# linhthi/BLISS-GNN

Measured on AMD Instinct MI355X. Metric: steps/sec (train step: sample_blocks + gather + SAGE fwd/bwd + Adam + exp3), reddit-like, higher is better.
Workload: dtype bf16

## Files before the change

bliss_gnn_amd/_engine.py:

```python
import contextlib
import ctypes as C
import os

import numpy as np
import torch

from . import _lib
from .graph import Block, Graph

_CHUNK = 1024
_CAP_ERRS = 1 | 2 | 4 | 8 | 64


def _ptr(t):
    return 0 if t is None else t.data_ptr()


def _stream():
    return torch.cuda.current_stream().cuda_stream


def _up8(n):
    return (int(n) + 7) & ~7


class _LayerWs:

    def __init__(self, dev, cap_s, cap_c):
        self.cap_s, self.cap_c = cap_s, cap_c
        self.seg_ptr = torch.empty(cap_s + 1, dtype=torch.int32, device=dev)
        self.seed_acc = torch.empty(60 * cap_s + 64, dtype=torch.uint8, device=dev)
        self.cand_nid = torch.empty(cap_c, dtype=torch.int32, device=dev)
        self.new_id = torch.empty(cap_c, dtype=torch.int32, device=dev)
        self.p = torch.empty(cap_c, dtype=torch.bfloat16, device=dev)
        self.P = torch.empty(cap_c, dtype=torch.bfloat16, device=dev)
        self.uniforms = torch.empty(cap_c, dtype=torch.float32, device=dev)
        self.src_cnt = None


class LayerEngine:

    def __init__(self, g: Graph):
        if g.device.type != "cuda":
            raise RuntimeError("bliss_gnn_amd samples on the GPU only; move the graph with g.to('cuda') "
                               "(the reference's --data-cpu/--use-uva modes are out of scope)")
        self.g = g
        dev = g.device
        V = g.num_nodes()
        self.V, self.Eg = V, g.num_edges()
        if self.Eg >= 2 ** 31:
            raise RuntimeError("int32 edge positions: graphs with >= 2^31 edges are not supported")
        self.scratch_sets = 2
        self._sets = {}
        self.first_pos = torch.full((V,), -1, dtype=torch.int32, device=dev)
        self.acc_p2 = torch.zeros(V, dtype=torch.int64, device=dev)
        self.c_graph = _lib.Graph(g.indptr.data_ptr(), g.indices.data_ptr(), _ptr(g.eid), V, self.Eg)
        self.flags = torch.zeros(16, dtype=torch.int32, device=dev)
        self.fs_ticket = torch.zeros(1, dtype=torch.int32, device=dev)
        self.fuse_scale = os.environ.get("BLISS_FUSE_SCALE", "1") != "0"
        self.flag_err = torch.zeros(1, dtype=torch.int32, device=dev)
        self.n_bins = 0
        for nb in ((int(os.environ["BLISS_NBINS"]),) if os.environ.get("BLISS_NBINS") else (256, 1024)):
            if -(-V // nb) * 12 <= 64 * 1024:
                self.n_bins = nb
                break
        if os.environ.get("BLISS_BINS", "1") == "0" or self.Eg > 2048 * 4096 * 32:
            self.n_bins = 0
        self._bins = None
        self.hist = torch.zeros(32768, dtype=torch.int32, device=dev)
        self.mt_dev = torch.empty(626, dtype=torch.int32, device=dev)
        self.mt_host = torch.empty(626, dtype=torch.int32).pin_memory()
        self.mt_back = torch.empty(626, dtype=torch.int32).pin_memory()
        self._static = {}
        self._slot_bufs, self._slot_counts, self._slot_counts_host = {}, {}, {}
        self.caps = None
        self.ws = None
        self.counts_host = None
        self.retries = 0

    def _set(self, n):
        i = n % self.scratch_sets
        if i not in self._sets:
            dev, V = self.g.device, self.V
            local_id = torch.full((V,), -1, dtype=torch.int32, device=dev)
            self._sets[i] = dict(local_id=local_id, kept_map=torch.full((V,), -1, dtype=torch.int32, device=dev),
                                 span_seg=torch.zeros(self.Eg // 256 + 2, dtype=torch.int32, device=dev),
                                 chunk_cnt=torch.empty(max(self.Eg, V) // _CHUNK + 2, dtype=torch.int32, device=dev),
                                 kept_rec=None, span_cnt=None,
                                 c_maps=_lib.NodeMaps(local_id.data_ptr(), self.first_pos.data_ptr(), self.acc_p2.data_ptr()))
        return self._sets[i]

    def _init_caps(self, S0, fanouts_sampling_order):
        caps, s = [], int(S0)
        for f in fanouts_sampling_order:
            k = min(self.V, int(1.25 * (f + s)) + 64)
            caps.append(dict(S=s, C=self.V, K=k, B=int(min(self.Eg, max(1 << 16, 48 * k)))))
            s = k
        return caps

    def _ensure(self, S0, fan):
        if self.caps is None or len(self.caps) != len(fan):
            self.caps = self._init_caps(S0, fan)
            self.ws = None
        elif self.caps[0]["S"] < S0:
            fresh = self._init_caps(S0, fan)
            self.caps = [{k: max(a[k], b[k]) for k in a} for a, b in zip(self.caps, fresh)]
            self.ws = None
        if self.ws is None:
            dev = self.g.device
            self.ws = [_LayerWs(dev, c["S"], c["C"]) for c in self.caps]
            self.counts_host = torch.empty(len(fan) * 10, dtype=torch.int32).pin_memory()
            self.rng_cap = sum(c["C"] for c in self.caps)
            plan = (C.c_int32 * 4)()
            _lib.check(_lib.lib.bliss_rng_prepare(self.rng_cap, plan), "bliss_rng_prepare")
            self.rng_plan = tuple(plan)
            n_words = 624 * (max(plan[3], self.rng_cap // 624 + 1) + 2)
            self.rng_out = torch.empty(n_words, dtype=torch.float32, device=dev)
            self.rng_raw = torch.empty(n_words, dtype=torch.int32, device=dev)
            self.rng_ctl = torch.zeros(8 + len(fan), dtype=torch.int32, device=dev)

    def _bin_buffers(self):
        if self._bins is None:
            dev, nb = self.g.device, self.n_bins
            cap = int(1.25 * self.Eg / nb) + 8192
            words = (-(-self.Eg // 4096) + 1) * 128 + 4
            self._bins = dict(cap=cap, cursor=torch.zeros(nb + 1, dtype=torch.int32, device=dev),
                              rec=torch.empty(nb * cap, dtype=torch.int64, device=dev),
                              bitmap=torch.zeros(words, dtype=torch.int32, device=dev),
                              prefix=torch.empty(2048 + words, dtype=torch.int32, device=dev),
                              tkey=torch.empty(self.V, dtype=torch.int64, device=dev),
                              tsum=torch.empty(self.V, dtype=torch.int64, device=dev))
        return self._bins

    def _grow(self, errs):
        for n, e in enumerate(errs):
            c = self.caps[n]
            if e & 2 and self.n_bins:
                self.n_bins = 0
            if e & 64:
                c["S"] = min(self.V, 2 * c["S"])
            if e & 4:
                c["K"] = min(self.V, 2 * c["K"])
            if e & 8:
                c["B"] = int(min(self.Eg, 2 * c["B"]))
        for n in range(len(self.caps) - 1):
            self.caps[n + 1]["S"] = max(self.caps[n + 1]["S"], self.caps[n]["K"])
        self.ws = None
        self.retries += 1

    @staticmethod
    def _rng_fields(state_bytes):
        a = state_bytes.numpy()
        return a[8:12].view(np.int32), a[16:24].view(np.int64), a[24:24 + 624 * 8].view(np.uint64)

    def _stage_rng(self, snapshot):
        left, nxt, st = self._rng_fields(snapshot)
        h = self.mt_host.numpy()
        h[:624] = st.astype(np.uint32).view(np.int32)
        h[624], h[625] = int(left[0]), int(nxt[0])

    def _commit_rng(self, snapshot):
        left, nxt, st = self._rng_fields(snapshot)
        h = self.mt_back.numpy()
        st[:] = h[:624].view(np.uint32).astype(np.uint64)
        left[0], nxt[0] = int(h[624]), int(h[625])
        torch.set_rng_state(snapshot)

    def sample_blocks(self, w_rows, seeds, fanouts, mode, eta, eps=0.9999, uniforms=None):
        seeds = seeds.to(torch.int32).contiguous()
        L = len(fanouts)
        self._ensure(int(seeds.numel()), fanouts)
        snapshot = torch.get_rng_state() if uniforms is None else None
        while True:
            out = self._enqueue(w_rows, seeds, fanouts, mode, eta, eps, uniforms, snapshot)
            counts_dev = out[0]
            self.counts_host.copy_(counts_dev, non_blocking=True)
            if snapshot is not None:
                self.mt_back.copy_(self.mt_dev, non_blocking=True)
            torch.cuda.current_stream().synchronize()
            raw = self.counts_host.numpy().tobytes()
            cnts = [_lib.LayerCounts.from_buffer_copy(raw[40 * n: 40 * n + 40]) for n in range(L)]
            errs = [c.err for c in cnts]
            bad = 0
            for e in errs:
                bad |= e
            if bad & ~_CAP_ERRS:
                raise RuntimeError(f"sampler kernel error 0x{bad:x}: {_lib.err_string(bad)}")
            if bad & 1:
                raise RuntimeError("frontier longer than the graph has edges (repeated seeds?) or >= 2^31 positions")
            if bad & 2 and not self.n_bins:
                raise RuntimeError("candidate capacity exceeded / seed id out of range")
            if bad == 0:
                break
            self._grow(errs)
            self._ensure(int(seeds.numel()), fanouts)
        if snapshot is not None:
            self._commit_rng(snapshot)
        return self._finish(out, cnts)

    def sample_blocks_multinomial(self, w_rows, seeds, fanouts, mode, eta, replace=False, fp32_importance=False):
        seeds = seeds.to(torch.int32).contiguous()
        L = len(fanouts)
        self._ensure(int(seeds.numel()), fanouts)
        for n in range(L):
            need = min(self.V, fanouts[n] + self.caps[n]["S"] + 64)
            if self.caps[n]["K"] < need:
                self.caps[n]["K"] = need
            if n + 1 < L and self.caps[n + 1]["S"] < self.caps[n]["K"]:
                self.caps[n + 1]["S"] = self.caps[n]["K"]
                self.ws = None
        self._ensure(int(seeds.numel()), fanouts)
        while True:
            dev, st = self.g.device, _stream()
            counts = torch.empty(L * 10, dtype=torch.int32, device=dev)
            eta_f, ome_f = float(np.float32(eta)), float(np.float32(1.0 - eta))
            layers, state = [], (seeds, int(seeds.numel()), 0)
            for n in range(L):
                cur_seeds, n_seeds, n_seeds_dev = state
                c_ws, c_out, lay, cnt_ptr, kept_nid = self._layer_buffers(n, counts)
                w_pos = w_rows[n]
                _lib.check(_lib.lib.bliss_frontier_prob(C.byref(self.c_graph), C.byref(self._set(n)["c_maps"]), w_pos.data_ptr(),
                                                        cur_seeds.data_ptr(), n_seeds, n_seeds_dev, self.caps[n]["S"], mode,
                                                        eta_f, ome_f, self.Eg, C.byref(c_ws), st), "bliss_frontier_prob")
                self.counts_host.copy_(counts, non_blocking=True)
                torch.cuda.current_stream().synchronize()
                Cn = int(self.counts_host[10 * n + 2])
                prob = self.ws[n].p[:Cn].cpu()
                if fp32_importance:
                    prob = prob.float()
                chosen = torch.multinomial(prob, min(int(fanouts[n]), Cn), replacement=replace)
                chosen_dev = chosen.to(torch.int32).to(dev)
                _lib.check(_lib.lib.bliss_multinomial_select(C.byref(c_ws), chosen_dev.data_ptr(), int(chosen_dev.numel()), st),
                           "bliss_multinomial_select")
                _lib.check(_lib.lib.bliss_build_block(C.byref(self.c_graph), C.byref(self._set(n)["c_maps"]), w_pos.data_ptr(),
                                                      cur_seeds.data_ptr(), self.caps[n]["S"], mode, eta_f, ome_f, self.Eg,
                                                      C.byref(c_ws), C.byref(c_out), st), "bliss_build_block")
                layers.append(lay)
                state = (kept_nid, -1, cnt_ptr + 12)
            self.counts_host.copy_(counts, non_blocking=True)
            torch.cuda.current_stream().synchronize()
            raw = self.counts_host.numpy().tobytes()
            cnts = [_lib.LayerCounts.from_buffer_copy(raw[40 * n: 40 * n + 40]) for n in range(L)]
            bad = 0
            for c in cnts:
                bad |= c.err
            if bad & ~_CAP_ERRS or bad & 2:
                raise RuntimeError(f"sampler kernel error 0x{bad:x}: {_lib.err_string(bad)}")
            if bad == 0:
                return self._finish((counts, layers), cnts)
            self._grow([c.err for c in cnts])
            self._ensure(int(seeds.numel()), fanouts)

    def _layer_buffers(self, n, counts, slot=None):
        dev = self.g.device
        cap, ws = self.caps[n], self.ws[n]
        cs, ck, cb = cap["S"], cap["K"], cap["B"]
        build_t = cs <= 32768
        if ws.src_cnt is None or ws.src_cnt.numel() < ck + 1:
            ws.src_cnt = torch.empty(ck + 1, dtype=torch.int32, device=dev)
        key = (slot, n, cs, ck, cb)
        if slot is not None and key in self._slot_bufs:
            ibuf, hbuf = self._slot_bufs[key]
        else:
            ibuf = torch.empty(_up8(cs + 1) + 4 * _up8(cb) + _up8(ck) + (2 * _up8(cb) + _up8(ck + 1) if build_t else 0),
                               dtype=torch.int32, device=dev)
            hbuf = torch.empty(2 * _up8(cb) + _up8(ck), dtype=torch.bfloat16, device=dev)
            if slot is not None:
                self._slot_bufs[key] = (ibuf, hbuf)
        o = 0
        b_indptr = ibuf[o:o + cs + 1]; o += _up8(cs + 1)
        b_src = ibuf[o:o + cb]; o += _up8(cb)
        b_dst = ibuf[o:o + cb]; o += _up8(cb)
        b_pos = ibuf[o:o + cb]; o += _up8(cb)
        b_eid = ibuf[o:o + cb]; o += _up8(cb)
        kept_nid = ibuf[o:o + ck]; o += _up8(ck)
        t_indptr = t_edge = t_scr = None
        if build_t:
            t_indptr = ibuf[o:o + ck + 1]; o += _up8(ck + 1)
            t_edge = ibuf[o:o + cb]; o += _up8(cb)
            t_scr = ibuf[o:o + cb]
        b_w = hbuf[0:cb]
        b_q = hbuf[_up8(cb):_up8(cb) + cb]
        node_prob = hbuf[2 * _up8(cb):2 * _up8(cb) + ck]
        cnt_ptr = counts.data_ptr() + 40 * n
        sset = self._set(n)
        c_ws = _lib.LayerWs(cnt_ptr, ws.seg_ptr.data_ptr(), ws.seed_acc.data_ptr(), sset["chunk_cnt"].data_ptr(),
                            ws.cand_nid.data_ptr(), ws.p.data_ptr(), ws.P.data_ptr(), ws.new_id.data_ptr(),
                            kept_nid.data_ptr(), node_prob.data_ptr(), self.hist.data_ptr(),
                            ws.src_cnt.data_ptr() if build_t else 0, cap["C"], ck)
        c_ws.kept_map, c_ws.span_seg = sset["kept_map"].data_ptr(), sset["span_seg"].data_ptr()
        e_bound = max(c.get("E", self.Eg) for c in self.caps)
        if e_bound <= (1 << 24):
            pos = -(-e_bound // 1024) * 1024
            if sset["kept_rec"] is None or sset["kept_rec"].numel() < pos * 2:
                sset["kept_rec"] = torch.empty(pos * 2, dtype=torch.int64, device=dev)
                sset["span_cnt"] = torch.zeros(pos // 256 + 4, dtype=torch.int32, device=dev)
            kr, sc = sset["kept_rec"], sset["span_cnt"]
            c_ws.kept_rec, c_ws.span_cnt, c_ws.kept_rec_positions = kr.data_ptr(), sc.data_ptr(), kr.numel() // 2
        if self.n_bins:
            b = self._bin_buffers()
            c_ws.n_bins, c_ws.bin_cap = self.n_bins, b["cap"]
            c_ws.bin_cursor, c_ws.bin_rec = b["cursor"].data_ptr(), b["rec"].data_ptr()
            c_ws.bitmap, c_ws.word_prefix = b["bitmap"].data_ptr(), b["prefix"].data_ptr()
            c_ws.touched_key, c_ws.touched_sum = b["tkey"].data_ptr(), b["tsum"].data_ptr()
        c_out = _lib.BlockOut(b_indptr.data_ptr(), b_src.data_ptr(), b_dst.data_ptr(), b_pos.data_ptr(), b_eid.data_ptr(),
                              b_w.data_ptr(), b_q.data_ptr(), _ptr(t_indptr), _ptr(t_edge), _ptr(t_scr), cb)
        lay = (b_indptr, b_src, b_dst, b_pos, b_eid, b_w, b_q, kept_nid, node_prob, counts[10 * n:10 * n + 10], t_indptr, t_edge)
        return c_ws, c_out, lay, cnt_ptr, kept_nid

    def set_static_caps(self, S0, fanouts, max_sizes, k_margin=1.5, b_margin=3.0):
        caps, s = [], int(S0)
        for n, f in enumerate(fanouts):
            k = min(self.V, int(k_margin * max_sizes[n]["K"]) + 256)
            b = int(min(self.Eg, int(b_margin * max_sizes[n]["B"]) + 4096))
            e = int(min(self.Eg, int(1.5 * max_sizes[n].get("E", self.Eg)) + 65536))
            x = int(min(b, int(1.5 * max_sizes[n]["B"]) + 2048))
            caps.append(dict(S=s, C=self.V, K=k, B=b, E=e, X=x))
            s = k
        self.caps, self.ws = caps, None
        self._ensure(S0, fanouts)

    def stage_rng_from_torch(self):
        self._static_snapshot = torch.get_rng_state()
        self._stage_rng(self._static_snapshot)

    def static_rng_begin(self, chain_rng=False):
        if not chain_rng:
            self.mt_dev.copy_(self.mt_host, non_blocking=True)
        _lib.check(_lib.lib.bliss_rng_stream_begin(self.mt_dev.data_ptr(), self.rng_ctl.data_ptr(), self.rng_out.data_ptr(),
                                                   self.rng_raw.data_ptr(), self.rng_cap, _stream()), "bliss_rng_stream_begin")

    def static_rng_end(self, slot=0):
        _lib.check(_lib.lib.bliss_rng_stream_end(self.mt_dev.data_ptr(), self.rng_ctl.data_ptr(), self.rng_raw.data_ptr(),
                                                 self.rng_cap, self._slot_counts[slot].data_ptr() + 20, _stream()), "bliss_rng_stream_end")
        self.mt_back.copy_(self.mt_dev, non_blocking=True)
        self._slot_counts_host[slot].copy_(self._slot_counts[slot], non_blocking=True)

    def static_rng_chain(self, slot, counts_host):
        cd = self._slot_counts[slot]
        assert counts_host.is_pinned() and counts_host.numel() >= cd.numel() and counts_host.dtype == torch.int32
        _lib.check(_lib.lib.bliss_rng_stream_chain(self.mt_dev.data_ptr(), self.rng_ctl.data_ptr(), self.rng_out.data_ptr(),
                                                   self.rng_raw.data_ptr(), self.rng_cap, cd.data_ptr(), cd.numel(),
                                                   counts_host.data_ptr(), _stream()), "bliss_rng_stream_chain")

    def static_rng_record(self, event):
        if getattr(self, "_gen_stream", None) is None:
            h = int(_lib.lib.bliss_rng_stream_handle())
            if not h:
                raise RuntimeError("bliss_rng_stream_handle failed")
            self._gen_stream = torch.cuda.ExternalStream(h)
        event.record(self._gen_stream)

    def static_rng_ready(self):
        _lib.check(_lib.lib.bliss_rng_stream_ready(_stream()), "bliss_rng_stream_ready")

    def enqueue_static(self, w_rows, seeds, fanouts, mode, eta, eps=0.9999, slot=0, chain_rng=False, external_rng=False, part=None,
                       last_block=True, ready_flag=0):
        if part is not None and (self.scratch_sets < len(fanouts) or not external_rng):
            raise ValueError("split enqueue needs one scratch set per layer and an external generator")
        L = len(fanouts)
        out = self._enqueue(w_rows, seeds, fanouts, mode, eta, eps, None, True, slot=slot, chain_rng=chain_rng,
                            external_rng=external_rng, part=part, last_block=last_block, ready_flag=ready_flag)
        counts_dev, layers = out
        if slot not in self._slot_counts_host:
            self._slot_counts_host[slot] = torch.empty(L * 10, dtype=torch.int32).pin_memory()
        if not external_rng:
            self._slot_counts_host[slot].copy_(counts_dev, non_blocking=True)
            self.mt_back.copy_(self.mt_dev, non_blocking=True)
        blocks = []
        for n, lay in enumerate(layers):
            b_indptr, b_src, b_dst, b_pos, b_eid, b_w, b_q, kept_nid, node_prob, cdev, t_indptr, t_edge = lay
            cap = self.caps[n]
            blk = Block(self.g, cap["K"], cap["S"], b_indptr, b_src, b_dst, b_pos, b_eid, kept_nid)
            blk._edge_weights, blk._q, blk._node_prob = b_w, b_q, node_prob
            blk._counts, blk._counts_dev = None, cdev
            blk._nnz_ptr = counts_dev.data_ptr() + 40 * n + 16
            blk._xcap = int(cap.get("X", cap["B"]))
            if t_indptr is not None:
                blk._transposed = (t_indptr, t_edge)
            blk._trace = {}
            blocks.append(blk)
        self._static[slot] = (blocks, L)
        return blocks

    def finish(self, slot=0, commit=True):
        blocks, L = self._static[slot]
        raw = self._slot_counts_host[slot].numpy().tobytes()
        cnts = [_lib.LayerCounts.from_buffer_copy(raw[40 * n: 40 * n + 40]) for n in range(L)]
        bad = 0
        for c in cnts:
            bad |= c.err
        for b, c in zip(blocks, cnts):
            b._counts = c
        if commit:
            self._commit_rng(self._static_snapshot)
        if bad:
            raise RuntimeError(f"static-shape step exceeded its capacities or hit a kernel error 0x{bad:x} "
                               f"({_lib.err_string(bad)}); the step's results are invalid -- raise the margins")
        return cnts

    def _enqueue(self, w_rows, seeds, fanouts, mode, eta, eps, uniforms, snapshot, slot=None, chain_rng=False, external_rng=False,
                 part=None, last_block=True, ready_flag=0):
        dev, st = self.g.device, _stream()
        L = len(fanouts)
        if snapshot is not None and not chain_rng and not external_rng:
            if snapshot is not True:
                self._stage_rng(snapshot)
            self.mt_dev.copy_(self.mt_host, non_blocking=True)
        if slot is None:
            counts = torch.empty(L * 10, dtype=torch.int32, device=dev)
        else:
            if slot not in self._slot_counts or self._slot_counts[slot].numel() != L * 10:
                self._slot_counts[slot] = torch.empty(L * 10, dtype=torch.int32, device=dev)
            counts = self._slot_counts[slot]
        use_rng = uniforms is None
        if use_rng and not external_rng:
            _lib.check(_lib.lib.bliss_rng_stream_begin(self.mt_dev.data_ptr(), self.rng_ctl.data_ptr(), self.rng_out.data_ptr(),
                                                       self.rng_raw.data_ptr(), self.rng_cap, st), "bliss_rng_stream_begin")
        eta_f = float(np.float32(eta))
        ome_f = float(np.float32(1.0 - eta))
        layers = []
        cur_seeds, n_seeds, n_seeds_dev = seeds, int(seeds.numel()), 0
        for n in range(L):
            cap = self.caps[n]
            cs, ws = cap["S"], self.ws[n]
            c_ws, c_out, lay, cnt_ptr, kept_nid = self._layer_buffers(n, counts, slot)
            w_pos = w_rows[n]
            last = n == L - 1
            if part == "main":
                c_ws.entry_flag = self.flags.data_ptr() + 4 * n
            if part in (None, "main"):
                if self.n_bins and self.fuse_scale:
                    c_ws.fs_ticket = self.fs_ticket.data_ptr()
                    c_ws.fs_fanout, c_ws.fs_eps = int(fanouts[n]), float(eps)
                    if use_rng:
                        c_ws.fs_rng_ctl, c_ws.fs_layer_off = self.rng_ctl.data_ptr(), self.rng_ctl.data_ptr() + 4 * (8 + n)
                        c_ws.fs_is_last, c_ws.fs_rng_cap = int(n == L - 1), self.rng_cap
                _lib.check(_lib.lib.bliss_frontier_prob(C.byref(self.c_graph), C.byref(self._set(n)["c_maps"]), w_pos.data_ptr(),
                                                        cur_seeds.data_ptr(), n_seeds, n_seeds_dev, cs, mode, eta_f, ome_f,
                                                        cap.get("E", self.Eg), C.byref(c_ws), st), "bliss_frontier_prob")
                if use_rng:
                    off_ptr = self.rng_ctl.data_ptr() + 4 * (8 + n)
                    _lib.check(_lib.lib.bliss_poisson_select(C.byref(c_ws), int(fanouts[n]), float(eps), self.rng_out.data_ptr(),
                                                             off_ptr, self.rng_ctl.data_ptr(), int(n == L - 1), self.rng_cap,
                                                             cap["C"], st), "bliss_poisson_select")
                else:
                    u = uniforms[n].to(dev, torch.float32).reshape(-1)
                    m = min(u.numel(), cap["C"])
                    ws.uniforms[:m].copy_(u[:m])
                    _lib.check(_lib.lib.bliss_poisson_select(C.byref(c_ws), int(fanouts[n]), float(eps), ws.uniforms.data_ptr(),
                                                             0, 0, 0, 0, cap["C"], st), "bliss_poisson_select")
            if part is None or (part == "main" and last and last_block) or (part == "early_blocks" and not last) or \
                    (part == "last_block" and last):
                if part == "last_block" and ready_flag:
                    c_ws.block_ready_flag = int(ready_flag)
                if part in ("early_blocks", "last_block"):
                    _lib.check(_lib.lib.bliss_flag_wait(self.flags.data_ptr() + 4 * (n + 1), self.flag_err.data_ptr(), st), "bliss_flag_wait")
                _lib.check(_lib.lib.bliss_build_block(C.byref(self.c_graph), C.byref(self._set(n)["c_maps"]), w_pos.data_ptr(),
                                                      cur_seeds.data_ptr(), cs, mode, eta_f, ome_f, cap.get("E", self.Eg), C.byref(c_ws),
                                                      C.byref(c_out), st), "bliss_build_block")
            layers.append(lay)
            cur_seeds, n_seeds, n_seeds_dev = kept_nid, -1, cnt_ptr + 12
        if part == "main" and not last_block:
            _lib.check(_lib.lib.bliss_flag_raise(self.flags.data_ptr() + 4 * L, st), "bliss_flag_raise")
        if use_rng and not external_rng:
            _lib.check(_lib.lib.bliss_rng_stream_end(self.mt_dev.data_ptr(), self.rng_ctl.data_ptr(), self.rng_raw.data_ptr(),
                                                     self.rng_cap, counts.data_ptr() + 20, _stream()), "bliss_rng_stream_end")
        return counts, layers

    def _finish(self, out, cnts):
        _, layers = out
        blocks = []
        for n, (lay, c) in enumerate(zip(layers, cnts)):
            b_indptr, b_src, b_dst, b_pos, b_eid, b_w, b_q, kept_nid, node_prob, cdev, t_indptr, t_edge = lay
            S, K, B = c.S, c.K, c.B
            blk = Block(self.g, K, S, b_indptr[:S + 1], b_src[:B], b_dst[:B], b_pos[:B], b_eid[:B], kept_nid[:K])
            blk._edge_weights, blk._q, blk._node_prob = b_w[:B], b_q[:B], node_prob[:K]
            blk._counts, blk._counts_dev = c, cdev
            if t_indptr is not None:
                blk._transposed = (t_indptr[:K + 1], t_edge[:max(B, 1)])
            ws = self.ws[n]
            blk._trace = dict(p=ws.p[:c.C], P=ws.P[:c.C], cand_nid=ws.cand_nid[:c.C], new_id=ws.new_id[:c.C])
            blocks.append(blk)
        return blocks
```

bliss_gnn_amd/_lib.py:

```python
import ctypes as C
import os

_HERE = os.path.dirname(os.path.abspath(__file__))
LIB_PATH = os.path.join(_HERE, "libbliss_gnn.so")

EINVAL = -1
MODE_BANDIT, MODE_LADIES, MODE_UNIFORM_NODES, MODE_PARTIALS = 0, 1, 4, 8

ERR_BITS = {
    1: "frontier larger than 2^31-1 edges",
    2: "candidate capacity exceeded / seed id out of range",
    4: "kept-node capacity exceeded",
    8: "block-edge capacity exceeded",
    16: "non-finite or negative weight reached an exact reduction",
    32: "exact sum left its fixed-point range",
    64: "seed capacity exceeded",
    128: "random stream ran short / generator made no progress",
    256: "a cross-stream flag never came (bliss_flag_wait timed out)",
}


class Graph(C.Structure):
    _fields_ = [("indptr", C.c_void_p), ("indices", C.c_void_p), ("eid", C.c_void_p),
                ("num_nodes", C.c_int32), ("num_edges", C.c_int64)]


class NodeMaps(C.Structure):
    _fields_ = [("local_id", C.c_void_p), ("first_pos", C.c_void_p), ("acc_p2", C.c_void_p)]


class LayerCounts(C.Structure):
    _fields_ = [("S", C.c_int32), ("E", C.c_int32), ("C", C.c_int32), ("K", C.c_int32), ("B", C.c_int32),
                ("err", C.c_int32), ("iters", C.c_int32), ("all_one", C.c_int32), ("c", C.c_double)]


class LayerWs(C.Structure):
    _fields_ = [("counts", C.c_void_p), ("seg_ptr", C.c_void_p), ("seed_acc", C.c_void_p), ("chunk_cnt", C.c_void_p),
                ("cand_nid", C.c_void_p), ("p", C.c_void_p), ("P", C.c_void_p), ("new_id", C.c_void_p),
                ("kept_nid", C.c_void_p), ("node_prob", C.c_void_p), ("hist", C.c_void_p), ("src_cnt", C.c_void_p), ("cap_c", C.c_int32), ("cap_k", C.c_int32),
                ("n_bins", C.c_int32), ("bin_cap", C.c_int64), ("bin_cursor", C.c_void_p), ("bin_rec", C.c_void_p),
                ("bitmap", C.c_void_p), ("word_prefix", C.c_void_p), ("touched_key", C.c_void_p), ("touched_sum", C.c_void_p),
                ("span_seg", C.c_void_p), ("kept_rec", C.c_void_p), ("span_cnt", C.c_void_p), ("kept_rec_positions", C.c_int64),
                ("kept_map", C.c_void_p), ("entry_flag", C.c_void_p),
                ("fs_ticket", C.c_void_p), ("fs_fanout", C.c_int32), ("fs_is_last", C.c_int32), ("fs_rng_cap", C.c_int32),
                ("fs_reserved", C.c_int32), ("fs_eps", C.c_double), ("fs_rng_ctl", C.c_void_p), ("fs_layer_off", C.c_void_p),
                ("block_ready_flag", C.c_void_p)]


class Exp3Block(C.Structure):
    _fields_ = [("w_pos", C.c_void_p), ("row_sum", C.c_void_p), ("scratch", C.c_void_p), ("norm_out", C.c_void_p),
                ("blk_indptr", C.c_void_p), ("blk_src", C.c_void_p), ("blk_dst", C.c_void_p), ("blk_pos", C.c_void_p),
                ("q_ij", C.c_void_p), ("node_prob", C.c_void_p), ("embed_norm", C.c_void_p), ("alpha_or_null", C.c_void_p),
                ("dst_nid", C.c_void_p), ("n_edges_dev", C.c_void_p), ("rewards_out", C.c_void_p), ("edges_bound", C.c_int32)]


EXP3_MAX_BLOCKS = 8


class Exp3RankLists(C.Structure):
    _fields_ = [("w_pos", C.c_void_p * EXP3_MAX_BLOCKS), ("row_sum", C.c_void_p * EXP3_MAX_BLOCKS),
                ("pos_off_words", C.c_int32 * EXP3_MAX_BLOCKS), ("factor_off_bf16", C.c_int32 * EXP3_MAX_BLOCKS),
                ("count_off_words", C.c_int32 * EXP3_MAX_BLOCKS), ("bound", C.c_int32 * EXP3_MAX_BLOCKS),
                ("n_blocks", C.c_int32), ("n_ranks", C.c_int32), ("rank_stride_words", C.c_int64)]


class PackLists(C.Structure):
    _fields_ = [("pos", C.c_void_p * EXP3_MAX_BLOCKS), ("n_dev", C.c_void_p * EXP3_MAX_BLOCKS),
                ("pos_off_words", C.c_int32 * EXP3_MAX_BLOCKS), ("count_off_words", C.c_int32 * EXP3_MAX_BLOCKS),
                ("bound", C.c_int32 * EXP3_MAX_BLOCKS), ("n_blocks", C.c_int32)]


class TileGemm(C.Structure):
    _fields_ = [("a1", C.c_void_p), ("a1_stride", C.c_int64), ("ids", C.c_void_p),
                ("w1", C.c_void_p), ("w1_stride", C.c_int64), ("k1", C.c_int32),
                ("a2", C.c_void_p), ("a2_stride", C.c_int64), ("w2", C.c_void_p), ("w2_stride", C.c_int64), ("k2", C.c_int32),
                ("bias", C.c_void_p), ("m_bound", C.c_int32), ("m_dev", C.c_void_p), ("n", C.c_int32),
                ("out", C.c_void_p), ("out_stride", C.c_int64), ("a_copy", C.c_void_p), ("copy_stride", C.c_int64),
                ("in_norm", C.c_void_p), ("out_norm", C.c_void_p),
                ("relu", C.c_int32), ("drop_p", C.c_float), ("drop_seed", C.c_uint32), ("drop_ctr", C.c_void_p)]


class DGrad(C.Structure):
    _fields_ = [("a1", C.c_void_p), ("a1_stride", C.c_int64), ("w1", C.c_void_p), ("w1_stride", C.c_int64), ("k1", C.c_int32),
                ("a2", C.c_void_p), ("a2_stride", C.c_int64), ("w2", C.c_void_p), ("w2_stride", C.c_int64), ("k2", C.c_int32),
                ("m2_bound", C.c_int32), ("m2_dev", C.c_void_p),
                ("m_bound", C.c_int32), ("m_dev", C.c_void_p), ("n", C.c_int32), ("out", C.c_void_p), ("out_stride", C.c_int64)]


class WGrad(C.Structure):
    _fields_ = [("d", C.c_void_p), ("d_stride", C.c_int64), ("n_out", C.c_int32),
                ("x", C.c_void_p), ("x_stride", C.c_int64), ("k_in", C.c_int32),
                ("rows_bound", C.c_int32), ("rows_dev", C.c_void_p),
                ("dw", C.c_void_p), ("dw_stride", C.c_int64), ("db", C.c_void_p)]


class GatFused(C.Structure):
    _fields_ = [("indptr", C.c_void_p), ("src", C.c_void_p), ("n_dst", C.c_int32), ("n_dst_dev", C.c_void_p),
                ("feat", C.c_void_p), ("feat_stride", C.c_int64), ("attn", C.c_void_p), ("heads", C.c_int32), ("head_dim", C.c_int32),
                ("negative_slope", C.c_float), ("e", C.c_void_p), ("a", C.c_void_p), ("a_drop", C.c_void_p),
                ("rst", C.c_void_p), ("rst_stride", C.c_int64),
                ("drop_p", C.c_float), ("drop_seed", C.c_uint32), ("drop_ctr", C.c_void_p), ("drop_ctr_used", C.c_void_p),
                ("g", C.c_void_p), ("g_stride", C.c_int64), ("de", C.c_void_p), ("d_er", C.c_void_p), ("d_er_stride", C.c_int64),
                ("dattn_part", C.c_void_p),
                ("wg_row", C.c_void_p), ("n_wg_dev", C.c_void_p), ("cap_wg", C.c_int32), ("row_ws", C.c_void_p), ("seg_part", C.c_void_p),
                ("err", C.c_void_p)]


ADAM_MAX_TENSORS = 32


class AdamTensors(C.Structure):
    _fields_ = [("param", C.c_void_p * ADAM_MAX_TENSORS), ("grad", C.c_void_p * ADAM_MAX_TENSORS),
                ("exp_avg", C.c_void_p * ADAM_MAX_TENSORS), ("exp_avg_sq", C.c_void_p * ADAM_MAX_TENSORS),
                ("numel", C.c_int64 * ADAM_MAX_TENSORS), ("count", C.c_int32)]


class BlockOut(C.Structure):
    _fields_ = [("indptr", C.c_void_p), ("src", C.c_void_p), ("dst", C.c_void_p), ("pos", C.c_void_p),
                ("eid", C.c_void_p), ("edge_weights", C.c_void_p), ("q_ij", C.c_void_p), ("t_indptr", C.c_void_p),
                ("t_edge", C.c_void_p), ("t_scratch", C.c_void_p), ("cap_b", C.c_int32)]


_P, _I32, _I64, _F, _D = C.c_void_p, C.c_int32, C.c_int64, C.c_float, C.c_double

SIGNATURES = {
    "bliss_layer_counts_bytes": [],
    "bliss_frontier_prob": [C.POINTER(Graph), C.POINTER(NodeMaps), _P, _P, _I32, _P, _I32, C.c_int, _F, _F, _I64, C.POINTER(LayerWs), _P],
    "bliss_rng_stream_begin": [_P, _P, _P, _P, _I32, _P],
    "bliss_rng_stream_wait": [_P, _P, _P, C.c_int, _I32, _P],
    "bliss_rng_stream_end": [_P, _P, _P, _I32, _P, _P],
    "bliss_rng_stream_chain": [_P, _P, _P, _P, _I32, _P, _I32, _P, _P],
    "bliss_rng_stream_ready": [_P],
    "bliss_rng_prepare": [_I32, _P],
    "bliss_mt_jump_poly": [_I64, _P],
    "bliss_flag_wait": [_P, _P, _P],
    "bliss_flag_set_spin_bound": [C.c_int64],
    "bliss_flag_raise": [_P, _P],
    "bliss_gather_rows": [_P, _I64, _P, _I32, _I32, _P, _I64, _P, _P],
    "bliss_exp3_apply_ranks": [C.POINTER(Exp3RankLists), _P, _P, _P, _P],
    "bliss_pack_lists": [C.POINTER(PackLists), _P, _P],
    "bliss_mt19937_uniform": [_P, _P, _I32, _P, _I32, _P],
    "bliss_poisson_select": [C.POINTER(LayerWs), _I32, _D, _P, _P, _P, C.c_int, _I32, _I64, _P],
    "bliss_multinomial_select": [C.POINTER(LayerWs), _P, _I32, _P],
    "bliss_tile_gemm": [C.POINTER(TileGemm), C.POINTER(TileGemm), _P],
    "bliss_cross_entropy": [_P, _I64, _P, _I32, _I32, _P, _P, _I64, _P, _P, _P, _P],
    "bliss_cross_entropy_sum": [_P, _I64, _P, _I64, _P, _P, _I32, _I32, _P, _P, _I64, _P, _P, _P, _P],
    "bliss_cross_entropy_masked": [_P, _I64, _P, _I64, _P, _I32, _P, _I32, _I32, _P, _F, _I32, _P, _P, _I64, _P, _P, _P, _P],
    "bliss_adam_step": [C.POINTER(AdamTensors), _P, _F, _F, _F, _F, _P],
    "bliss_cand_importance": [_P, _I32, C.c_int, _P, _P, _P],
    "bliss_poisson_scale": [_P, _P, _I32, _D, _P, _P],
    "bliss_keyed_select": [_P, _P, _P, _I32, _P, C.c_uint64, C.c_uint64, _I32, _P, _P, _P],
    "bliss_exp3_normalize_global": [_P, _I64, _P, _P, _P, _P, _P],
    "bliss_build_block": [C.POINTER(Graph), C.POINTER(NodeMaps), _P, _P, _I32, C.c_int, _F, _F, _I64, C.POINTER(LayerWs), C.POINTER(BlockOut), _P],
    "bliss_normalized_edata": [C.POINTER(Graph), _P, _P],
    "bliss_embed_norm": [_P, _I32, _I32, _I64, _P, _P],
    "bliss_spmm_fwd": [_P, _P, _P, _P, _P, _I64, _I32, _P, _I32, _I32, C.c_int, _P, _I64, C.c_int, _P, _P],
    "bliss_spmm_bwd": [_P, _P, _P, _P, _P, _P, _P, _I64, _I32, _P, _I32, _I32, C.c_int, _P, _I64, C.c_int, _P, _P],
    "bliss_block_transpose": [_P, _P, _I32, _I32, _I32, _P, _P, _P, _I64, _P],
    "bliss_spmm_chunk_edges": [_I32],
    "bliss_sage_epilogue_fwd": [_P, _I64, _P, _I64, _I32, _I32, _F, C.c_uint32, _P, _P, _I64, _P, _P],
    "bliss_sage_epilogue_bwd": [_P, _I64, _P, _I64, _I32, _I32, _F, _P, _I64, _P],
    "bliss_gat_chunk_edges": [],
    "bliss_graph_prepare": [_P, _P, _I64, _I32, C.c_int, _P, _P, _P, _P, _P, _P, _I64, _P],
    "bliss_exp3_update": [C.POINTER(Graph), _P, _P, _P, _P, _P, _P, _P, _P, _P, _P, _P, _P, _I32, _P, _I32, _F, _P, _P, C.c_int, _P, _P],
    "bliss_exp3_step": [C.POINTER(Graph), _P, C.POINTER(Exp3Block), _I32, _F, _P, _P],
    "bliss_exp3_normalize_global_rows": [C.POINTER(Exp3Block), _I32, _I64, _P, _I64, _P],
    "bliss_exp3_update_blocks": [C.POINTER(Graph), _P, C.POINTER(Exp3Block), _I32, _F, _P, _P],
    "bliss_exp3_apply": [_P, _P, _P, _P, _P, _I32, _P, _P],
    "bliss_exp3_normalize": [_P, _I64, _P, _P, _P, _P],
    "bliss_row_sum": [_P, _I64, _P, _P],
    "bliss_gat_logits": [_P, _P, _P, _I32, _P, _I64, _P, _I32, _I32, _F, _P, _P],
    "bliss_sage_dgrad": [C.POINTER(DGrad), _P],
    "bliss_sage_wgrad": [C.POINTER(WGrad), _I32, _P, _I64, _P],
    "bliss_shard_local_seeds": [_P, _I32, _P, _I32, _I32, _I32, _P, _P, _P, _P, _P, _P],
    "bliss_shard_scatter_partials": [_P, _P, _P, _P, _P, _P, _P, _I32, _P, _P],
    "bliss_shard_zero_dense": [_P, _I32, _P],
    "bliss_shard_pack_rows": [_P, _P, _I32, _I32, _I32, _P, _I64, _I32, _P, _I64, _P],
    "bliss_shard_place_rows": [_P, _I64, _P, _P, _I32, _P, _I64, _I32, _I32, _P],
    "bliss_shard_take_rows": [_P, _I32, _I64, _I32, _P, _P, _I32, _P, _I64, _I32, _P],
    "bliss_shard_candidates": [_P, _I32, _I32, _P, _P, _P, _P, _P, _I32, _P, _P, _P],
    "bliss_shard_select_kept": [_P, _P, _P, _P, C.c_uint64, _P, _I32, _P, _I32, _P, _P, _P, _P, _P, _I32, _I32, _I32, _P, _P, _P, _I32, _P, _P, _P],
    "bliss_gat_fused_supported": [_I32, _I32],
    "bliss_gat_segment_edges": [],
    "bliss_gat_fused_stamps": [_P, _P],
    "bliss_gat_segments": [_P, _I32, _I32, _P, _P, _P, _P],
    "bliss_gat_fused_fwd": [C.POINTER(GatFused), _P],
    "bliss_gat_fused_bwd_dst": [C.POINTER(GatFused), _P, _P, _P, _P],
    "bliss_gat_rows_src_fused": [_P, _I32, _P, _P, _P, _P, _I32, _P, _P, _P, _I64, _P, _I64, _P, _I32, _I32, _F, _P, _I64, _P, _P],
    "bliss_gat_logits_f32": [_P, _P, _P, _I32, _P, _I64, _P, _I32, _I32, _F, _P, _P],
    "bliss_gat_edge_dot": [_P, _P, _P, _I32, _P, _I64, _P, _I64, _I32, _I32, _P, _P],
    "bliss_gat_edge_softmax": [_P, _I32, _P, _P, _I32, C.c_int, _P, _P],
    "bliss_gat_rows": [C.c_int, _P, _I32, _P, _P, _P, _P, _I32, _P, _P, _I64, _P, _I32, _I32, _F, _P, _I64, _P, _P, _P],
    "bliss_gat_alpha": [_P, _I32, _P, _P, _P, _P, _P],
    "bliss_prof_enable": [C.c_int],
    "bliss_prof_reset": [],
    "bliss_prof_read": [C.c_int, C.POINTER(C.c_double), C.POINTER(C.c_int64)],
    "bliss_prof_kernel_count": [],
}


SPECIAL_SIGNATURES = ("bliss_prof_kernel_name", "bliss_block_transpose_temp_bytes", "bliss_graph_prepare_capacity",
                      "bliss_graph_prepare_temp_bytes", "bliss_rng_stream_handle", "bliss_sage_wgrad_workspace")


def _load():
    if not os.path.exists(LIB_PATH):
        raise ImportError(
            f"{LIB_PATH} not found: build it with `python -c 'import __graft_entry__ as g; g.build()'` "
            "or `make -C bliss_gnn_amd/csrc`.  bliss_gnn_amd has no CPU or PyTorch fallback.")
    lib = C.CDLL(LIB_PATH)
    for name, argtypes in SIGNATURES.items():
        fn = getattr(lib, name)
        fn.argtypes = argtypes
        fn.restype = C.c_int
    lib.bliss_block_transpose_temp_bytes.argtypes = [_I32, _I32]
    lib.bliss_block_transpose_temp_bytes.restype = C.c_int64
    lib.bliss_sage_wgrad_workspace.argtypes = [C.POINTER(WGrad), _I32]
    lib.bliss_sage_wgrad_workspace.restype = C.c_int64
    for name in ("bliss_graph_prepare_capacity", "bliss_graph_prepare_temp_bytes"):
        getattr(lib, name).argtypes = [_I64, _I32, C.c_int]
        getattr(lib, name).restype = C.c_int64
    lib.bliss_rng_stream_handle.argtypes = []
    lib.bliss_rng_stream_handle.restype = C.c_int64
    lib.bliss_prof_kernel_name.argtypes = [C.c_int]
    lib.bliss_prof_kernel_name.restype = C.c_char_p
    assert lib.bliss_layer_counts_bytes() == C.sizeof(LayerCounts), "LayerCounts layout mismatch"
    return lib


lib = _load()


def check(rc, what):
    if rc != 0:
        raise RuntimeError(f"{what} failed with code {rc}" + (" (invalid argument)" if rc == EINVAL else " (hipError_t)"))


def err_string(bits):
    return "; ".join(msg for b, msg in ERR_BITS.items() if bits & b) or "unknown"
```

bliss_gnn_amd/csrc/prof.h:

```cpp
#pragma once
#include <hip/hip_runtime.h>

enum BlissKernelId {
  BK_SEG_SCAN = 0, BK_PASS1, BK_PASS2, BK_CHUNK_SCAN, BK_PASS3, BK_CAND_FINALIZE, BK_POISSON_SCALE, BK_SELECT1, BK_SELECT2,
  BK_BLOCK1, BK_INDPTR_SCAN, BK_BLOCK2, BK_CLEANUP, BK_MT19937, BK_SPMM_FWD, BK_SPMM_BWD, BK_EMBED_NORM, BK_EXP3_UPDATE,
  BK_EXP3_APPLY, BK_NORMALIZE, BK_ROW_SUM, BK_NORM_EDATA, BK_TRANSPOSE, BK_SPMM_FIXUP, BK_COL_SUMS, BK_BIN_SCATTER, BK_BIN_REDUCE,
  BK_BITMAP_SCAN, BK_CAND_NUMBER, BK_COUNT
};

extern int g_bliss_prof_sel;
void bliss_prof_begin(int id, hipStream_t st);
void bliss_prof_end(int id, hipStream_t st);

#define PROF_LAUNCH(id, st, ...)                                              \
  do {                                                                        \
    const bool p_ = (g_bliss_prof_sel == -1 || g_bliss_prof_sel == (id));    \
    if (p_) bliss_prof_begin((id), (st));                                     \
    __VA_ARGS__;                                                              \
    if (p_) bliss_prof_end((id), (st));                                       \
  } while (0)
```

bliss_gnn_amd/csrc/prof.hip:

```cpp
#include "prof.h"
#include "bliss_gnn.h"
#include <mutex>
#include <vector>

int g_bliss_prof_sel = -2;

namespace {
struct Pair { hipEvent_t a, b; int id; };
std::mutex g_mu;
std::vector<Pair> g_open, g_free;
double g_ms[BK_COUNT];
long long g_n[BK_COUNT];
const char* kNames[BK_COUNT] = {
  "k_seg_scan", "k_frontier_pass1", "k_frontier_pass2", "k_chunk_scan", "k_frontier_pass3", "k_cand_finalize", "k_poisson_scale",
  "k_select_pass1", "k_select_pass2", "k_block_pass1", "k_indptr_scan", "k_block_pass2", "k_cleanup", "k_mt19937_uniform",
  "k_spmm_fwd", "k_spmm_bwd", "k_embed_norm", "k_exp3_update", "k_exp3_apply", "k_normalize_row", "k_row_sum",
  "k_normalized_edata", "k_block_transpose", "k_spmm_fixup", "k_col_sums", "k_bin_scatter", "k_bin_reduce", "k_bitmap_scan",
  "k_cand_number"};
thread_local Pair t_cur;

void drain_locked() {
  for (auto& p : g_open) {
    (void)hipEventSynchronize(p.b);
    float ms = 0.f;
    if (hipEventElapsedTime(&ms, p.a, p.b) == hipSuccess) { g_ms[p.id] += ms; g_n[p.id] += 1; }
    g_free.push_back(p);
  }
  g_open.clear();
}
}

void bliss_prof_begin(int id, hipStream_t st) {
  std::lock_guard<std::mutex> lk(g_mu);
  if (g_open.size() >= 8192) drain_locked();
  Pair p;
  if (!g_free.empty()) { p = g_free.back(); g_free.pop_back(); }
  else { (void)hipEventCreate(&p.a); (void)hipEventCreate(&p.b); }
  p.id = id;
  (void)hipEventRecord(p.a, st);
  t_cur = p;
}

void bliss_prof_end(int id, hipStream_t st) {
  (void)id;
  (void)hipEventRecord(t_cur.b, st);
  std::lock_guard<std::mutex> lk(g_mu);
  g_open.push_back(t_cur);
}

extern "C" {

int bliss_prof_enable(int kernel_id) {
  if (kernel_id < -2 || kernel_id >= BK_COUNT) return BLISS_EINVAL;
  g_bliss_prof_sel = kernel_id;
  return 0;
}

int bliss_prof_reset(void) {
  std::lock_guard<std::mutex> lk(g_mu);
  drain_locked();
  for (int i = 0; i < BK_COUNT; ++i) { g_ms[i] = 0; g_n[i] = 0; }
  return 0;
}

int bliss_prof_read(int kernel_id, double* total_ms, int64_t* launches) {
  if (kernel_id < 0 || kernel_id >= BK_COUNT || !total_ms || !launches) return BLISS_EINVAL;
  std::lock_guard<std::mutex> lk(g_mu);
  drain_locked();
  *total_ms = g_ms[kernel_id];
  *launches = g_n[kernel_id];
  return 0;
}

int bliss_prof_kernel_count(void) { return BK_COUNT; }

const char* bliss_prof_kernel_name(int kernel_id) { return (kernel_id >= 0 && kernel_id < BK_COUNT) ? kNames[kernel_id] : ""; }

}
```

bliss_gnn_amd/csrc/sampler.hip:

```cpp
#include "common.cuh"
#include "bliss_gnn.h"
#include "prof.h"
#include <cstdlib>

#ifndef TPB
#define TPB 256
#endif
#define ITEMS 4
#define CHUNK (TPB * ITEMS)

namespace {

#define SPAN (64 * ITEMS)
#define SEG_ZERO_WGS 8
#define LONG_COL 1024

struct EdgeAt {
  int k;
  int64_t pos;
  int src;
};

__device__ __forceinline__ EdgeAt decode(int base, int E, int S, const int* __restrict__ seg_ptr,
                                         const long long* __restrict__ col_base, const int* __restrict__ indices, int* k_hint) {
  EdgeAt r;
  const int e = base + lane_id();
  r.k = wave_segment(seg_ptr, S, base, k_hint);
  r.pos = 0; r.src = 0;
  if (e < E) {
    r.pos = col_base[r.k] + e;
    r.src = indices[r.pos];
  } else r.k = -1;
  return r;
}

__device__ __forceinline__ int chunk_wave_offset(int wave_total, int* sh4, int* chunk_total) {
  const int wave = threadIdx.x >> 6;
  __syncthreads();
  if (lane_id() == 0) sh4[wave] = wave_total;
  __syncthreads();
  int off = 0, tot = 0;
#pragma unroll
  for (int w = 0; w < TPB / 64; ++w) { const int v = sh4[w]; tot += v; if (w < wave) off += v; }
  *chunk_total = tot;
  return off;
}

__device__ __forceinline__ bf16_t edge_q(bf16_t w, bf16_t wsum, int n, float eta_f, float ome_f) {
  float wd = rbf(bf2f(w) / bf2f(wsum));
  float a = rbf((1.0f / (float)n) * eta_f);
  float b = rbf(ome_f * wd);
  return f2bf(a + b);
}

__device__ __forceinline__ bf16_t edge_q_pre(bf16_t w, bf16_t wsum, float a, float ome_f) {
  float wd = rbf(bf2f(w) / bf2f(wsum));
  float b = rbf(ome_f * wd);
  return f2bf(a + b);
}

__device__ __forceinline__ void seg_scan_body(const int64_t* __restrict__ indptr, const int* __restrict__ seeds,
                                              LayerCounts* cnt, int S_host, const int* __restrict__ S_dev, int cap_s,
                                              unsigned long long* __restrict__ seed_acc, int* __restrict__ seg_ptr,
                                              int* __restrict__ local_id, int num_nodes, int* __restrict__ src_cnt, int cap_k,
                                              int* __restrict__ bin_cursor, int n_bins, long long* __restrict__ col_base,
                                              int* __restrict__ span_seg, long long frontier_cap, int* entry_flag,
                                              int wg, int n_wgs, bool keep_sums, int* sh, int* st_sh, int* hub_count = nullptr) {
  if (entry_flag && wg == 0 && threadIdx.x == 0) __hip_atomic_store(entry_flag, 1, __ATOMIC_RELEASE, __HIP_MEMORY_SCOPE_AGENT);
  __shared__ int sh_long;
  if (hub_count && threadIdx.x == 0) sh_long = 0;
  int S = S_host >= 0 ? S_host : *S_dev;
  int bad = 0;
  if (S > cap_s) { S = cap_s; bad |= BLISS_ERR_CAP_SEEDS; }
  if (wg > 0 || n_wgs == 1) {
    const int nz = n_wgs > 1 ? n_wgs - 1 : 1, bz = n_wgs > 1 ? wg - 1 : 0;
    const int t0 = bz * blockDim.x + threadIdx.x, step = nz * blockDim.x;
    for (int i = (keep_sums ? 2 * cap_s : 0) + t0; i < cap_s * 5; i += step) seed_acc[i] = 0ull;
    if (src_cnt) for (int i = t0; i <= cap_k; i += step) src_cnt[i] = 0;
    if (bin_cursor) for (int i = t0; i <= n_bins; i += step) bin_cursor[i] = 0;
    for (int k = t0; k < S; k += step) { const int s = seeds[k]; if (s >= 0 && s < num_nodes) local_id[s] = k; }
    if (n_wgs > 1) return;
  }
  long long run = 0;
  constexpr int G = 4;
  for (int base0 = 0; base0 < S; base0 += G * (int)blockDim.x) {
    int degs[G];
    long long cols[G];
#pragma unroll
    for (int i = 0; i < G; ++i) {
      const int k = base0 + i * (int)blockDim.x + threadIdx.x;
      degs[i] = 0; cols[i] = 0;
      if (k < S) {
        const int s = seeds[k];
        if (s < 0 || s >= num_nodes) { bad |= BLISS_ERR_CAP_CAND; }
        else {
          cols[i] = indptr[s];
          degs[i] = (int)(indptr[s + 1] - cols[i]);
        }
      }
    }
#pragma unroll
    for (int i = 0; i < G; ++i) {
      const int k = base0 + i * (int)blockDim.x + threadIdx.x;
      if (base0 + i * (int)blockDim.x >= S) break;
      const int deg = degs[i];
      int tot, ex = block_excl_scan(deg, sh, &tot);
      const long long start = run + ex;
      if (k < S) {
        seg_ptr[k] = (int)start;
        col_base[k] = deg > 0 ? cols[i] - start : 0;
      }
      if (hub_count) {
        const bool is_long = k < S && deg > LONG_COL;
        const unsigned long long mask = __ballot(is_long);
        if (mask) {
          int base_l = 0;
          if (lane_id() == 0) base_l = atomicAdd(&sh_long, __popcll(mask));
          base_l = __shfl(base_l, 0);
          if (is_long) hub_count[base_l + __popcll(mask & ((1ull << lane_id()) - 1ull))] = k;
        }
      }
      if (run + tot <= frontier_cap) {
        st_sh[threadIdx.x] = (int)(k < S ? start : run + tot);
        __syncthreads();
        const long long sp_end = (run + tot + SPAN - 1) / SPAN;
        for (long long sp = (run + SPAN - 1) / SPAN + threadIdx.x; sp < sp_end; sp += blockDim.x) {
          const int p = (int)(sp * SPAN);
          int t = 0;
#pragma unroll
          for (int step = 512; step >= 1; step >>= 1) if (st_sh[t + step] <= p) t += step;
          span_seg[sp] = base0 + i * (int)blockDim.x + t;
        }
      }
      run += tot;
      if (run > frontier_cap) bad |= BLISS_ERR_CAP_FRONTIER;
    }
  }
  int any_bad = __syncthreads_or(bad);
  if (threadIdx.x == 0) {
    if (hub_count) hub_count[cap_s] = sh_long;
    seg_ptr[S] = (int)run;
    cnt->S = S; cnt->E = (any_bad & BLISS_ERR_CAP_FRONTIER) ? 0 : (int)run;
    cnt->C = 0; cnt->K = 0; cnt->B = 0; cnt->iters = 0; cnt->all_one = 0; cnt->c = 1.0;
    cnt->err = any_bad;
  }
}

__global__ void __launch_bounds__(1024) k_seg_scan(const int64_t* __restrict__ indptr, const int* __restrict__ seeds,
                                                   LayerCounts* cnt, int S_host, const int* __restrict__ S_dev, int cap_s,
                                                   unsigned long long* __restrict__ seed_acc, int* __restrict__ seg_ptr,
                                                   int* __restrict__ local_id, int num_nodes, int* __restrict__ src_cnt, int cap_k,
                                                   int* __restrict__ bin_cursor, int n_bins, long long* __restrict__ col_base,
                                                   int* __restrict__ span_seg, long long frontier_cap, int* entry_flag,
                                                   int keep_sums, int* hub_count) {
  __shared__ int sh[17];
  __shared__ int st_sh[1024];
  seg_scan_body(indptr, seeds, cnt, S_host, S_dev, cap_s, seed_acc, seg_ptr, local_id, num_nodes, src_cnt, cap_k, bin_cursor, n_bins,
                col_base, span_seg, frontier_cap, entry_flag, blockIdx.x, gridDim.x, keep_sums != 0, sh, st_sh, hub_count);
}

template <bool BANDIT>
__global__ void __launch_bounds__(TPB) k_frontier_pass1(const int64_t* __restrict__ indptr, const int* __restrict__ indices,
                                                        const bf16_t* __restrict__ w, const int* __restrict__ seeds,
                                                        const int* __restrict__ seg_ptr, const long long* __restrict__ col_base,
    const int* __restrict__ span_seg, LayerCounts* cnt,
                                                        const int* __restrict__ local_id, unsigned* first_pos,
                                                        unsigned long long* acc_w) {
  const int S = cnt->S, E = cnt->E;
  const int nspans = (E + SPAN - 1) / SPAN;
  int bad = 0;
  for (int sp = blockIdx.x * (TPB / 64) + (threadIdx.x >> 6); sp < nspans; sp += gridDim.x * (TPB / 64)) {
    int hint = span_seg[sp];
#pragma unroll
    for (int i = 0; i < ITEMS; ++i) {
      const int base = sp * SPAN + i * 64;
      if (base >= E) break;
      const int e = base + lane_id();
      EdgeAt a = decode(base, E, S, seg_ptr, col_base, indices, &hint);
      int64_t term = 0;
      if (a.k >= 0) {
        if (local_id[a.src] < 0) {
          if (__hip_atomic_load(first_pos + a.src, __ATOMIC_RELAXED, __HIP_MEMORY_SCOPE_AGENT) > (unsigned)e)
            atomicMin(first_pos + a.src, (unsigned)e);
        }
        if (BANDIT) term = bf_to_fixed(w[a.pos], FRAC_DST, &bad);
      }
      if (BANDIT) wave_segsum_atomic_i64(a.k, term, acc_w);
    }
  }
  if (bad) atomicOr(&cnt->err, bad);
}

template <bool BANDIT>
__global__ void __launch_bounds__(TPB) k_frontier_pass2(const int64_t* __restrict__ indptr, const int* __restrict__ indices,
                                                        const bf16_t* __restrict__ w, const int* __restrict__ seeds,
                                                        const int* __restrict__ seg_ptr, const long long* __restrict__ col_base,
    const int* __restrict__ span_seg, LayerCounts* cnt,
                                                        const unsigned* __restrict__ first_pos,
                                                        const unsigned long long* __restrict__ acc_w,
                                                        unsigned long long* acc_q, int* __restrict__ chunk_cnt,
                                                        float eta_f, float ome_f) {
  __shared__ int sh4[TPB / 64];
  const int S = cnt->S, E = cnt->E;
  const int nchunks = (E + CHUNK - 1) / CHUNK;
  int bad = 0;
  for (int chunk = blockIdx.x; chunk < nchunks; chunk += gridDim.x) {
    int nfirst = 0, hint = span_seg[chunk * ITEMS + (threadIdx.x >> 6)];
#pragma unroll
    for (int i = 0; i < ITEMS; ++i) {
      const int base = chunk * CHUNK + (threadIdx.x >> 6) * SPAN + i * 64;
      if (base >= E) break;
      const int e = base + lane_id();
      EdgeAt a = decode(base, E, S, seg_ptr, col_base, indices, &hint);
      int64_t term = 0;
      bool first = false;
      if (a.k >= 0) {
        first = first_pos[a.src] == (unsigned)e;
        if (BANDIT) {
          bf16_t wsum = fixed_to_bf((int64_t)acc_w[a.k], FRAC_DST, &bad);
          bf16_t q = edge_q(w[a.pos], wsum, seg_ptr[a.k + 1] - seg_ptr[a.k], eta_f, ome_f);
          term = bf_to_fixed(q, FRAC_DST, &bad);
        }
      }
      nfirst += __popcll(__ballot(first));
      if (BANDIT) wave_segsum_atomic_i64(a.k, term, acc_q);
    }
    int tot;
    chunk_wave_offset(nfirst, sh4, &tot);
    if (threadIdx.x == 0) chunk_cnt[chunk] = tot;
  }
  if (bad) atomicOr(&cnt->err, bad);
}

__global__ void __launch_bounds__(1024) k_chunk_scan(int* __restrict__ chunk_cnt, LayerCounts* cnt, int which, int cap) {
  __shared__ int sh[17];
  int n_items = which == 1 ? cnt->C : cnt->E;
  const int n = (n_items + CHUNK - 1) / CHUNK;
  int run = 0;
  for (int base = 0; base < n; base += blockDim.x) {
    int i = base + threadIdx.x;
    int v = i < n ? chunk_cnt[i] : 0;
    int tot, ex = block_excl_scan(v, sh, &tot);
    if (i < n) chunk_cnt[i] = run + ex;
    run += tot;
  }
  if (threadIdx.x == 0) {
    int total = which == 0 ? cnt->S + run : run;
    int errbit = which == 0 ? BLISS_ERR_CAP_CAND : (which == 1 ? BLISS_ERR_CAP_KEPT : BLISS_ERR_CAP_EDGES);
    if (total > cap) { atomicOr(&cnt->err, errbit); total = cap; }
    if (which == 0) cnt->C = total; else if (which == 1) cnt->K = total; else cnt->B = total;
  }
}

template <bool BANDIT>
__global__ void __launch_bounds__(TPB) k_frontier_pass3(const int64_t* __restrict__ indptr, const int* __restrict__ indices,
                                                        const bf16_t* __restrict__ w, const int* __restrict__ seeds,
                                                        const int* __restrict__ seg_ptr, const long long* __restrict__ col_base,
    const int* __restrict__ span_seg, LayerCounts* cnt,
                                                        const unsigned* __restrict__ first_pos,
                                                        const unsigned long long* __restrict__ acc_w,
                                                        const unsigned long long* __restrict__ acc_q,
                                                        const int* __restrict__ chunk_off, int* local_id,
                                                        int* __restrict__ cand_nid, unsigned long long* acc_p2,
                                                        float eta_f, float ome_f, int cap_c, int uniform_nodes) {
  __shared__ int sh4[TPB / 64];
  const int S = cnt->S, E = cnt->E;
  const int nchunks = (E + CHUNK - 1) / CHUNK;
  int bad = 0;
  for (int chunk = blockIdx.x; chunk < nchunks; chunk += gridDim.x) {
    int hint = span_seg[chunk * ITEMS + (threadIdx.x >> 6)], wave_total = 0;
    unsigned long long mask[ITEMS];
    int srcs[ITEMS];
#pragma unroll
    for (int i = 0; i < ITEMS; ++i) {
      mask[i] = 0; srcs[i] = 0;
      const int base = chunk * CHUNK + (threadIdx.x >> 6) * SPAN + i * 64;
      if (base >= E) continue;
      const int e = base + lane_id();
      EdgeAt a = decode(base, E, S, seg_ptr, col_base, indices, &hint);
      bool first = false;
      if (a.k >= 0) {
        srcs[i] = a.src;
        first = first_pos[a.src] == (unsigned)e;
        bf16_t t = 0;
        if (uniform_nodes) {
          acc_p2[a.src] = 1ull;
        } else if (BANDIT) {
          bf16_t wsum = fixed_to_bf((int64_t)acc_w[a.k], FRAC_DST, &bad);
          bf16_t q = edge_q(w[a.pos], wsum, seg_ptr[a.k + 1] - seg_ptr[a.k], eta_f, ome_f);
          bf16_t qsum = fixed_to_bf((int64_t)acc_q[a.k], FRAC_DST, &bad);
          float r = rbf(bf2f(q) / bf2f(qsum));
          t = f2bf(r * r);
        } else {
          float x = bf2f(w[a.pos]);
          t = f2bf(x * x);
        }
        int64_t fx = uniform_nodes ? 0 : bf_to_fixed(t, FRAC_SRC, &bad);
        if (fx) atomicAdd(acc_p2 + a.src, (unsigned long long)fx);
      }
      mask[i] = __ballot(first);
      wave_total += __popcll(mask[i]);
    }
    int tot;
    int run = S + chunk_off[chunk] + chunk_wave_offset(wave_total, sh4, &tot);
#pragma unroll
    for (int i = 0; i < ITEMS; ++i) {
      if ((mask[i] >> lane_id()) & 1ull) {
        const int id = run + __popcll(mask[i] & ((1ull << lane_id()) - 1ull));
        if (id < cap_c) { local_id[srcs[i]] = id; cand_nid[id] = srcs[i]; }
      }
      run += __popcll(mask[i]);
    }
  }
  if (bad) atomicOr(&cnt->err, bad);
}

#define HIST_BINS 32768
#define HWIN_LO 0x3000
#define HWIN_N 4096
#ifndef FIN_TPB
#define FIN_TPB 1024
#endif
__global__ void __launch_bounds__(FIN_TPB) k_cand_finalize(const int* __restrict__ seeds, LayerCounts* cnt, int* __restrict__ cand_nid,
                                                           unsigned long long* acc_p2, unsigned* first_pos,
                                                           bf16_t* __restrict__ p, int* hist, int cap_c, int uniform_nodes) {
  __shared__ int lh[HIST_BINS];
  const int S = cnt->S;
  const int C = min(cnt->C, cap_c);
  if ((int)blockIdx.x * FIN_TPB >= C) return;
  {
    int4* lh4 = reinterpret_cast<int4*>(lh);
    for (int b = threadIdx.x; b < HIST_BINS / 4; b += FIN_TPB) lh4[b] = make_int4(0, 0, 0, 0);
  }
  __syncthreads();
  int bad = 0;
  for (int id = blockIdx.x * FIN_TPB + threadIdx.x; id < C; id += gridDim.x * FIN_TPB) {
    int g;
    if (id < S) { g = seeds[id]; cand_nid[id] = g; } else g = cand_nid[id];
    const unsigned long long raw = acc_p2[g];
    acc_p2[g] = 0;
    first_pos[g] = 0xffffffffu;
    bf16_t pj;
    if (uniform_nodes) pj = raw ? (bf16_t)0x3f80 : (bf16_t)0;
    else pj = f2bf(sqrtf(bf2f(fixed_to_bf((int64_t)raw, FRAC_SRC, &bad))));
    p[id] = pj;
    if (pj < HIST_BINS) atomicAdd(&lh[pj], 1); else bad |= BLISS_ERR_NONFINITE;
  }
  __syncthreads();
  {
    const int4* lh4 = reinterpret_cast<const int4*>(lh);
    for (int b = threadIdx.x; b < HIST_BINS / 4; b += FIN_TPB) {
      const int4 v = lh4[b];
      if (v.x | v.y | v.z | v.w) {
        if (v.x) atomicAdd(hist + 4 * b, v.x);
        if (v.y) atomicAdd(hist + 4 * b + 1, v.y);
        if (v.z) atomicAdd(hist + 4 * b + 2, v.z);
        if (v.w) atomicAdd(hist + 4 * b + 3, v.w);
      }
    }
  }
  if (bad) atomicOr(&cnt->err, bad);
}

#define BIN_TPB 1024
#ifndef BIN_ITEMS
#define BIN_ITEMS 4
#endif
#define BIN_BATCH (BIN_TPB * BIN_ITEMS)
#define MAX_BINS 1024
#ifndef COL_TPB
#define COL_TPB 1024
#endif
#ifndef COL_R
#define COL_R 16
#endif
#ifndef COL_RB
#define COL_RB 8
#endif
#define COL_BIG (COL_R * 64)
static_assert(LONG_COL == COL_BIG, "k_seg_scan lists the columns k_col_sums treats as long");
#ifndef BINRED_TPB
#define BINRED_TPB 1024
#endif

template <int NT>
__device__ __forceinline__ int block_max_u31(int v, long long* sh) {
  v = wave_max_u31(v);
  __syncthreads();
  if (lane_id() == 0) sh[threadIdx.x >> 6] = v;
  __syncthreads();
  int t = 0;
#pragma unroll
  for (int w = 0; w < NT / 64; ++w) t = max(t, (int)sh[w]);
  return t;
}

template <int NT>
__device__ __forceinline__ long long block_sum2_i64(long long a, long long b, long long* sh2, long long* b_out) {
  a = wave_total_i64(a);
  b = wave_total_i64(b);
  __syncthreads();
  if (lane_id() == 0) { sh2[threadIdx.x >> 6] = a; sh2[NT / 64 + (threadIdx.x >> 6)] = b; }
  __syncthreads();
  long long ta = 0, tb = 0;
#pragma unroll
  for (int w = 0; w < NT / 64; ++w) { ta += sh2[w]; tb += sh2[NT / 64 + w]; }
  *b_out = tb;
  return ta;
}

template <int NT>
__device__ __forceinline__ long long block_sum_i64(long long v, long long* sh) {
  v = wave_total_i64(v);
  __syncthreads();
  if (lane_id() == 0) sh[threadIdx.x >> 6] = v;
  __syncthreads();
  long long t = 0;
#pragma unroll
  for (int w = 0; w < NT / 64; ++w) t += sh[w];
  return t;
}

__device__ __forceinline__ void col_store(int k, long long ws_fixed, long long qs_fixed, bf16_t wsum, int n, float eta_f,
                                          unsigned long long* acc_w, unsigned long long* acc_q, uint2* seed_coef, int* bad) {
  acc_w[k] = (unsigned long long)ws_fixed; acc_q[k] = (unsigned long long)qs_fixed;
  const bf16_t qsum = fixed_to_bf(qs_fixed, FRAC_DST, bad);
  seed_coef[k] = make_uint2((unsigned)wsum | ((unsigned)qsum << 16), __float_as_uint(rbf((1.0f / (float)n) * eta_f)));
}

__global__ void __launch_bounds__(COL_TPB) k_col_sums(const int64_t* __restrict__ indptr, const bf16_t* __restrict__ w,
                                                      const int* __restrict__ seeds, const int* __restrict__ seg_ptr,
                                                      const long long* __restrict__ col_base, const int* __restrict__ span_seg,
                                                      LayerCounts* cnt, unsigned long long* __restrict__ acc_w,
                                                      unsigned long long* __restrict__ acc_q, float eta_f, float ome_f,
                                                      uint2* __restrict__ seed_coef, int n_wave_wgs,
                                                      const int* __restrict__ long_list, int cap_s) {
  __shared__ long long sh[COL_TPB / 64];
  __shared__ long long sh2[2 * COL_TPB / 64];
  const int S = cnt->S, tid = threadIdx.x, lane = lane_id();
  if (cnt->E == 0) return;
  int bad = 0;
  const int n_block_wgs = (int)gridDim.x - n_wave_wgs;
  if ((int)blockIdx.x < n_wave_wgs)
  for (int k = blockIdx.x * (COL_TPB / 64) + (tid >> 6); k < S; k += n_wave_wgs * (COL_TPB / 64)) {
    const int s0 = seg_ptr[k], n = seg_ptr[k + 1] - s0;
    if (n == 0 || n > COL_BIG) continue;
    const long long p0 = col_base[k] + s0;
    bf16_t wr[COL_R];
    long long part = 0;
    int emax = 1;
#pragma unroll
    for (int r = 0; r < COL_R; ++r) {
      const int i = lane + r * 64;
      wr[r] = 0;
      if (i < n) wr[r] = w[p0 + i];
    }
#pragma unroll
    for (int r = 0; r < COL_R; ++r)
      if (lane + r * 64 < n) emax = max(emax, bf_exp_field(wr[r]));
    const int wfrac = rel_frac(FRAC_DST, wave_max_u31(emax));
    long long part_lo = 0;
    int sticky = 0;
#pragma unroll
    for (int r = 0; r < COL_R; ++r)
      if (lane + r * 64 < n) part += bf_to_fixed_wide(wr[r], wfrac, &part_lo, &sticky, &bad);
    const long long ws_fixed = wave_total_i64(part);
    bf16_t wsum;
    if (__ballot(part_lo != 0 || sticky) == 0ull) wsum = fixed_to_bf(ws_fixed, wfrac, &bad);
    else wsum = fixed_wide_to_bf(ws_fixed, wave_total_i64(part_lo), __ballot(sticky) != 0ull, wfrac, &bad);
    const float a = rbf((1.0f / (float)n) * eta_f);
    part = 0;
#pragma unroll
    for (int r = 0; r < COL_R; ++r) {
      const int i = lane + r * 64;
      if (i < n) part += bf_to_fixed(edge_q_pre(wr[r], wsum, a, ome_f), FRAC_DST, &bad);
    }
    const long long qs_fixed = wave_total_i64(part);
    if (lane == 0) col_store(k, ws_fixed, qs_fixed, wsum, n, eta_f, acc_w, acc_q, seed_coef, &bad);
  }
  if ((int)blockIdx.x >= n_wave_wgs)
  for (int li = (int)blockIdx.x - n_wave_wgs, n_long = long_list[cap_s]; li < n_long; li += n_block_wgs) {
    const int k = long_list[li];
    const int s0 = seg_ptr[k], n = seg_ptr[k + 1] - s0;
    if (n <= COL_BIG) continue;
    const long long p0 = col_base[k] + s0;
    bf16_t wr[COL_RB];
    long long part = 0;
    int emax = 1;
#pragma unroll
    for (int r = 0; r < COL_RB; ++r) {
      const int i = tid + r * COL_TPB;
      wr[r] = 0;
      if (i < n) wr[r] = w[p0 + i];
    }
#pragma unroll
    for (int r = 0; r < COL_RB; ++r)
      if (tid + r * COL_TPB < n) emax = max(emax, bf_exp_field(wr[r]));
#pragma unroll 8
    for (int i = tid + COL_RB * COL_TPB; i < n; i += COL_TPB) emax = max(emax, bf_exp_field(w[p0 + i]));
    const int wfrac = rel_frac(FRAC_DST, block_max_u31<COL_TPB>(emax, sh));
    long long part_lo = 0;
    int sticky = 0;
#pragma unroll
    for (int r = 0; r < COL_RB; ++r)
      if (tid + r * COL_TPB < n) part += bf_to_fixed_wide(wr[r], wfrac, &part_lo, &sticky, &bad);
#pragma unroll 8
    for (int i = tid + COL_RB * COL_TPB; i < n; i += COL_TPB)
      part += bf_to_fixed_wide(w[p0 + i], wfrac, &part_lo, &sticky, &bad);
    long long lost;
    const long long ws_fixed = block_sum2_i64<COL_TPB>(part, (part_lo != 0 || sticky) ? 1 : 0, sh2, &lost);
    bf16_t wsum;
    if (lost == 0) wsum = fixed_to_bf(ws_fixed, wfrac, &bad);
    else {
      const long long lo_tot = block_sum_i64<COL_TPB>(part_lo, sh);
      const long long st_tot = block_sum_i64<COL_TPB>(sticky, sh);
      wsum = fixed_wide_to_bf(ws_fixed, lo_tot, st_tot != 0, wfrac, &bad);
    }
    const float a = rbf((1.0f / (float)n) * eta_f);
    part = 0;
#pragma unroll
    for (int r = 0; r < COL_RB; ++r) {
      const int i = tid + r * COL_TPB;
      if (i < n) part += bf_to_fixed(edge_q_pre(wr[r], wsum, a, ome_f), FRAC_DST, &bad);
    }
#pragma unroll 8
    for (int i = tid + COL_RB * COL_TPB; i < n; i += COL_TPB) part += bf_to_fixed(edge_q_pre(w[p0 + i], wsum, a, ome_f), FRAC_DST, &bad);
    const long long qs_fixed = block_sum_i64<COL_TPB>(part, sh);
    if (tid == 0) col_store(k, ws_fixed, qs_fixed, wsum, n, eta_f, acc_w, acc_q, seed_coef, &bad);
  }
  if (bad) atomicOr(&cnt->err, bad);
}

template <bool BANDIT>
__global__ void __launch_bounds__(BIN_TPB) k_bin_scatter(const int64_t* __restrict__ indptr, const int* __restrict__ indices,
                                                     const bf16_t* __restrict__ w, const int* __restrict__ seeds,
                                                     const int* __restrict__ seg_ptr, const long long* __restrict__ col_base,
    const int* __restrict__ span_seg, LayerCounts* cnt,
                                                     const unsigned long long* __restrict__ acc_w,
                                                     const unsigned long long* __restrict__ acc_q, float eta_f, float ome_f,
                                                     int uniform_nodes, int n_bins, int log2_bins, long long bin_cap, int* bin_cursor,
                                                     unsigned long long* __restrict__ bin_rec, unsigned* __restrict__ bitmap,
                                                     const uint2* __restrict__ seed_coef) {
  __shared__ int hist[MAX_BINS];
  __shared__ int gbase[MAX_BINS];
  const int S = cnt->S, E = cnt->E, tid = threadIdx.x;
  const int nb = (E + BIN_BATCH - 1) / BIN_BATCH;
  const int bmask = n_bins - 1;
  int bad = 0;
  for (int batch = blockIdx.x; batch < nb; batch += gridDim.x) {
    for (int b = tid; b < n_bins; b += BIN_TPB) hist[b] = 0;
    if (tid < BIN_BATCH / 32) bitmap[batch * (BIN_BATCH / 32) + tid] = 0u;
    __syncthreads();
    int srcs[BIN_ITEMS], ranks[BIN_ITEMS];
    bf16_t ts[BIN_ITEMS];
    const int wbase = batch * BIN_BATCH + (tid >> 6) * (64 * BIN_ITEMS);
    int hint = span_seg[wbase >> 8];
#pragma unroll
    for (int j = 0; j < BIN_ITEMS; ++j) {
      ranks[j] = -1; srcs[j] = 0; ts[j] = 0;
      const int base = wbase + j * 64;
      if (base >= E) continue;
      EdgeAt a = decode(base, E, S, seg_ptr, col_base, indices, &hint);
      if (a.k >= 0) {
        bf16_t t;
        if (uniform_nodes) {
          t = (bf16_t)0x3f80;
        } else if (BANDIT) {
          const uint2 cf = seed_coef[a.k];
          bf16_t q = edge_q_pre(w[a.pos], (bf16_t)(cf.x & 0xffffu), __uint_as_float(cf.y), ome_f);
          float r = rbf(bf2f(q) / bf2f((bf16_t)(cf.x >> 16)));
          t = f2bf(r * r);
        } else {
          float x = bf2f(w[a.pos]);
          t = f2bf(x * x);
        }
        srcs[j] = a.src; ts[j] = t;
        ranks[j] = atomicAdd(&hist[a.src & bmask], 1);
      }
    }
    __syncthreads();
    for (int b = tid; b < n_bins; b += BIN_TPB) {
      const int h = hist[b];
      int g0 = 0;
      if (h) {
        g0 = atomicAdd(bin_cursor + b, h);
        if ((long long)g0 + h > bin_cap) bad |= BLISS_ERR_CAP_CAND;
      }
      gbase[b] = g0;
    }
    __syncthreads();
#pragma unroll
    for (int j = 0; j < BIN_ITEMS; ++j) {
      if (ranks[j] >= 0) {
        const int b = srcs[j] & bmask;
        const long long idx = (long long)gbase[b] + ranks[j];
        if (idx < bin_cap) {
          const size_t o = (size_t)b * (size_t)bin_cap + (size_t)idx;
          const unsigned e = (unsigned)(wbase + j * 64 + lane_id());
          bin_rec[o] = ((unsigned long long)e << 32) | ((unsigned long long)((unsigned)srcs[j] >> log2_bins) << 15) | (ts[j] & 0x7fffu);
        }
      }
    }
    __syncthreads();
  }
  if (bad) atomicOr(&cnt->err, bad);
}

__global__ void __launch_bounds__(BINRED_TPB) k_bin_reduce(LayerCounts* cnt, int n_bins, int log2_bins, long long bin_cap,
                                                           int* bin_cursor, const unsigned long long* __restrict__ bin_rec,
                                                           int num_nodes, int slots,
                                                           const int* __restrict__ local_id, unsigned long long* __restrict__ seed_p2,
                                                           unsigned long long* __restrict__ touched_key,
                                                           unsigned long long* __restrict__ touched_sum, unsigned* bitmap, int cap_c) {
  extern __shared__ unsigned long long dyn_lds[];
  unsigned long long* sm = dyn_lds;
  unsigned* mn = (unsigned*)(dyn_lds + slots);
  const int b = blockIdx.x, tid = threadIdx.x;
  if (cnt->E == 0) return;
  const int ne = b < num_nodes ? ((num_nodes - 1 - b) >> log2_bins) + 1 : 0;
  for (int i = tid; i < ne; i += BINRED_TPB) { sm[i] = 0ull; mn[i] = 0xffffffffu; }
  __syncthreads();
  long long n = bin_cursor[b];
  if (n > bin_cap) n = bin_cap;
  const unsigned long long* rec = bin_rec + (size_t)b * (size_t)bin_cap;
  int bad = 0;
  for (long long i = tid; i < n; i += BINRED_TPB) {
    const unsigned long long r = rec[i];
    const int li = (int)(((unsigned)r) >> 15);
    atomicMin(&mn[li], (unsigned)(r >> 32));
    const int64_t fx = bf_to_fixed((bf16_t)(r & 0x7fffu), FRAC_SRC, &bad);
    if (fx) atomicAdd(&sm[li], (unsigned long long)fx);
  }
  __syncthreads();
  __shared__ int wg_cnt, wg_base;
  if (tid == 0) wg_cnt = 0;
  __syncthreads();
  for (int li = tid; li < ne; li += BINRED_TPB) {
    bool is_cand = false;
    if (mn[li] != 0xffffffffu) {
      const int lid = local_id[((unsigned)li << log2_bins) | (unsigned)b];
      if (lid >= 0) { seed_p2[lid] = sm[li]; mn[li] = 0xffffffffu; }
      else is_cand = true;
    }
    const unsigned long long mask = __ballot(is_cand);
    if (mask && lane_id() == 0) atomicAdd(&wg_cnt, __popcll(mask));
  }
  __syncthreads();
  if (tid == 0) { wg_base = wg_cnt ? atomicAdd(bin_cursor + n_bins, wg_cnt) : 0; wg_cnt = 0; }
  __syncthreads();
  for (int li = tid; li < ne; li += BINRED_TPB) {
    const unsigned fp = mn[li];
    if (fp != 0xffffffffu) {
      const int j = wg_base + atomicAdd(&wg_cnt, 1);
      if (j < cap_c) { touched_key[j] = ((unsigned long long)fp << 32) | (((unsigned)li << log2_bins) | (unsigned)b); touched_sum[j] = sm[li]; }
      atomicOr(bitmap + (fp >> 5), 1u << (fp & 31u));
    }
  }
  if (bad) atomicOr(&cnt->err, bad);
}

#define BTILE_W 4
#define BTILE (1024 * BTILE_W)
#define MAX_TILES 2048
__global__ void __launch_bounds__(1024) k_bitmap_tiles(const unsigned* __restrict__ bitmap, int* __restrict__ word_prefix,
                                                       int* __restrict__ tile_sum, LayerCounts* cnt) {
  __shared__ int sh[17];
  const int nw = (cnt->E + 31) >> 5;
  const int ntiles = (nw + BTILE - 1) / BTILE;
  for (int tile = blockIdx.x; tile < ntiles; tile += gridDim.x) {
    const int i = tile * BTILE + threadIdx.x * BTILE_W;
    uint4 v = make_uint4(0, 0, 0, 0);
    if (i < nw) v = *reinterpret_cast<const uint4*>(bitmap + i);
    const int c0 = __popc(v.x), c1 = __popc(v.y), c2 = __popc(v.z), c3 = __popc(v.w);
    int total, ex = block_excl_scan(c0 + c1 + c2 + c3, sh, &total);
    if (i < nw) *reinterpret_cast<int4*>(word_prefix + i) = make_int4(ex, ex + c0, ex + c0 + c1, ex + c0 + c1 + c2);
    if (threadIdx.x == 0) tile_sum[tile] = total;
  }
}

__device__ __forceinline__ double block_sum_f64(double v, double* shd) {
  for (int d = 32; d >= 1; d >>= 1) {
    long long b = __double_as_longlong(v);
    int lo = __shfl_down((int)(b & 0xffffffffll), d), hi = __shfl_down((int)(b >> 32), d);
    v += __longlong_as_double(((long long)hi << 32) | (unsigned)lo);
  }
  __syncthreads();
  if (lane_id() == 0) shd[threadIdx.x >> 6] = v;
  __syncthreads();
  double t = 0;
  for (int i = 0; i < (int)(blockDim.x >> 6); ++i) t += shd[i];
  return t;
}

template <bool COHERENT>
__device__ __forceinline__ void poisson_scale_body(int* hist, LayerCounts* cnt, int C, int num, double eps, int* rng_ctl,
                                                   int* layer_off, int is_last, int rng_cap_total, int* __restrict__ sel_state,
                                                   double* shd) {
  for (int i = threadIdx.x; i < (C + CHUNK - 1) / CHUNK + 2; i += 1024) sel_state[i] = 0;
  if (rng_ctl && threadIdx.x == 1023) rng_stream_acquire(rng_ctl, C, layer_off, is_last, rng_cap_total);
  int n[HIST_BINS / 1024];
  bool any = false;
#pragma unroll
  for (int i = 0; i < HIST_BINS / 1024; ++i) {
    const int b = i * 1024 + threadIdx.x;
    n[i] = COHERENT ? __hip_atomic_load(hist + b, __ATOMIC_RELAXED, __HIP_MEMORY_SCOPE_AGENT) : hist[b];
  }
#pragma unroll
  for (int i = 0; i < HIST_BINS / 1024; ++i) {
    const int b = i * 1024 + threadIdx.x;
    if (n[i]) {
      if (COHERENT) __hip_atomic_store(hist + b, 0, __ATOMIC_RELAXED, __HIP_MEMORY_SCOPE_AGENT); else hist[b] = 0;
      any = true;
    }
  }
  if (C <= num) {
    if (threadIdx.x == 0) { cnt->c = 1.0; cnt->all_one = 1; cnt->iters = 0; }
    return;
  }
  double c = 1.0;
  int it = 0;
  for (; it < 50; ++it) {
    const float c32 = (float)c;
    double loc = 0;
    if (any) {
#pragma unroll
      for (int i = 0; i < HIST_BINS / 1024; ++i) {
        if (n[i]) {
          float v = rbf(bf2f((bf16_t)(i * 1024 + threadIdx.x)) * c32);
          v = v < 1.0f ? v : (v != v ? v : 1.0f);
          loc += (double)n[i] * (double)v;
        }
      }
    }
    double Ssum = block_sum_f64(loc, shd);
    double lo = Ssum < (double)num ? Ssum : (double)num, hi = Ssum < (double)num ? (double)num : Ssum;
    if (lo / hi >= eps) { ++it; break; }
    c *= (double)num / Ssum;
  }
  if (threadIdx.x == 0) { cnt->c = c; cnt->all_one = 0; cnt->iters = it > 50 ? 50 : it; }
}

__global__ void __launch_bounds__(1024) k_poisson_scale(int* hist, LayerCounts* cnt, int num, double eps, int* rng_ctl,
                                                        int* layer_off, int is_last, int rng_cap_total, int* __restrict__ sel_state) {
  __shared__ double shd[16];
  poisson_scale_body<false>(hist, cnt, cnt->C, num, eps, rng_ctl, layer_off, is_last, rng_cap_total, sel_state, shd);
}

struct FusedScale { int* ticket; int num; double eps; int* rng_ctl; int* layer_off; int is_last; int rng_cap_total; int* sel_state; };
__global__ void __launch_bounds__(FIN_TPB) k_cand_number(const int* __restrict__ seeds, LayerCounts* cnt, int* __restrict__ cand_nid,
                                                         int* local_id, const unsigned long long* __restrict__ seed_p2,
                                                         const unsigned long long* __restrict__ touched_key,
                                                         const unsigned long long* __restrict__ touched_sum,
                                                         const unsigned* __restrict__ bitmap, const int* __restrict__ word_prefix,
                                                         const int* __restrict__ tile_sum, bf16_t* __restrict__ p, int* hist,
                                                         int cap_c, int uniform_nodes, const FusedScale fs) {
  __shared__ int lh[HWIN_N + 4];
  __shared__ int tile_off[MAX_TILES];
  __shared__ int sh[17];
  const int S = cnt->S;
  const int ntiles = (((cnt->E + 31) >> 5) + BTILE - 1) / BTILE;
  int run = 0;
  for (int base = 0; base < ntiles; base += FIN_TPB) {
    const int t = base + threadIdx.x;
    int total, ex = block_excl_scan(t < ntiles ? tile_sum[t] : 0, sh, &total);
    if (t < ntiles) tile_off[t] = run + ex;
    run += total;
  }
  int C = S + run;
  if (C > cap_c) { C = cap_c; if (blockIdx.x == 0 && threadIdx.x == 0) atomicOr(&cnt->err, BLISS_ERR_CAP_CAND); }
  if (blockIdx.x == 0 && threadIdx.x == 0) cnt->C = C;
  if (blockIdx.x != 0 && (int)blockIdx.x * FIN_TPB >= C) return;
  {
    int4* lh4 = reinterpret_cast<int4*>(lh);
    for (int b = threadIdx.x; b < (HWIN_N + 4) / 4; b += FIN_TPB) lh4[b] = make_int4(0, 0, 0, 0);
  }
  __syncthreads();
  int bad = 0;
  for (int i = blockIdx.x * FIN_TPB + threadIdx.x; i < C; i += gridDim.x * FIN_TPB) {
    int id;
    unsigned long long raw;
    if (i < S) {
      id = i; raw = seed_p2[i];
      cand_nid[i] = seeds[i];
    } else {
      const unsigned long long key = touched_key[i - S];
      raw = touched_sum[i - S];
      const unsigned fp = (unsigned)(key >> 32), g = (unsigned)key;
      id = S + tile_off[(fp >> 5) / BTILE] + word_prefix[fp >> 5] + __popc(bitmap[fp >> 5] & ((1u << (fp & 31u)) - 1u));
      if (id >= cap_c) continue;
      local_id[g] = id; cand_nid[id] = (int)g;
    }
    bf16_t pj;
    if (uniform_nodes) pj = raw ? (bf16_t)0x3f80 : (bf16_t)0;
    else pj = f2bf(sqrtf(bf2f(fixed_to_bf((int64_t)raw, FRAC_SRC, &bad))));
    p[id] = pj;
    if (pj >= HIST_BINS) bad |= BLISS_ERR_NONFINITE;
    else if ((unsigned)(pj - HWIN_LO) < (unsigned)HWIN_N) atomicAdd(&lh[pj - HWIN_LO], 1);
    else if (pj == 0) atomicAdd(&lh[HWIN_N], 1);
    else atomicAdd(hist + pj, 1);
  }
  __syncthreads();
  {
    const int4* lh4 = reinterpret_cast<const int4*>(lh);
    for (int b = threadIdx.x; b < HWIN_N / 4; b += FIN_TPB) {
      const int4 v = lh4[b];
      if (v.x | v.y | v.z | v.w) {
        if (v.x) atomicAdd(hist + HWIN_LO + 4 * b, v.x);
        if (v.y) atomicAdd(hist + HWIN_LO + 4 * b + 1, v.y);
        if (v.z) atomicAdd(hist + HWIN_LO + 4 * b + 2, v.z);
        if (v.w) atomicAdd(hist + HWIN_LO + 4 * b + 3, v.w);
      }
    }
    if (threadIdx.x == 0 && lh[HWIN_N]) atomicAdd(hist, lh[HWIN_N]);
  }
  if (bad) atomicOr(&cnt->err, bad);
  if (fs.ticket) {
    static_assert(FIN_TPB == 1024, "the fused Poisson scale runs in a 1024-thread workgroup");
    __shared__ int sh_is_last;
    __shared__ double shd[16];
    int active = (C + FIN_TPB - 1) / FIN_TPB;
    if (active > (int)gridDim.x) active = (int)gridDim.x;
    if (active < 1) active = 1;
    asm volatile("s_waitcnt vmcnt(0)" ::: "memory");
    __syncthreads();
    if (threadIdx.x == 0) {
      sh_is_last = atomicAdd(fs.ticket, 1) == active - 1;
      if (sh_is_last) __hip_atomic_store(fs.ticket, 0, __ATOMIC_RELAXED, __HIP_MEMORY_SCOPE_AGENT);
    }
    __syncthreads();
    if (sh_is_last)
      poisson_scale_body<true>(hist, cnt, C, fs.num, fs.eps, fs.rng_ctl, fs.layer_off, fs.is_last, fs.rng_cap_total, fs.sel_state, shd);
  }
}

__device__ __forceinline__ bf16_t incl_prob(const bf16_t* __restrict__ p, int j, int S, int all_one, float c32) {
  if (all_one || j < S) return 0x3f80;
  float v = rbf(bf2f(p[j]) * c32);
  return (v < 1.0f || v != v) ? f2bf(v) : (bf16_t)0x3f80;
}

#define SEL_AGG 1
#define SEL_PFX 2
__global__ void __launch_bounds__(TPB) k_select_fused(const bf16_t* __restrict__ p, const float* __restrict__ uniforms_base,
                                                      const int* __restrict__ u_off, LayerCounts* cnt, bf16_t* __restrict__ P,
                                                      int* state, const int* __restrict__ cand_nid, int* __restrict__ new_id,
                                                      int* __restrict__ kept_nid, bf16_t* __restrict__ node_prob, int cap_c, int cap_k,
                                                      int* __restrict__ kept_map) {
  __shared__ int sh4[TPB / 64];
  __shared__ int sh_chunk, sh_base, sh_K;
  const float* __restrict__ uniforms = uniforms_base + (u_off ? *u_off : 0);
  const int S = cnt->S, C = min(cnt->C, cap_c), all_one = cnt->all_one;
  const float c32 = (float)cnt->c;
  const int nchunks = (C + CHUNK - 1) / CHUNK;
  if (threadIdx.x == 0) sh_chunk = atomicAdd(state, 1);
  __syncthreads();
  const int chunk = sh_chunk;
  if (chunk >= nchunks) return;
  unsigned long long mask[ITEMS];
  bf16_t Pv[ITEMS];
  int wave_total = 0;
#pragma unroll
  for (int i = 0; i < ITEMS; ++i) {
    const int j = chunk * CHUNK + (threadIdx.x >> 6) * SPAN + i * 64 + lane_id();
    bool keep = false;
    Pv[i] = 0;
    if (j < C) {
      Pv[i] = incl_prob(p, j, S, all_one, c32);
      P[j] = Pv[i];
      keep = __hip_atomic_load(uniforms + j, __ATOMIC_RELAXED, __HIP_MEMORY_SCOPE_AGENT) < bf2f(Pv[i]);
    }
    mask[i] = __ballot(keep);
    wave_total += __popcll(mask[i]);
  }
  int tot;
  const int woff = chunk_wave_offset(wave_total, sh4, &tot);
  if (threadIdx.x < 64) {
    const int lane = lane_id();
    int excl = 0, bad = 0;
    if (chunk > 0) {
      if (lane == 0) __hip_atomic_store(state + 1 + chunk, (tot << 2) | SEL_AGG, __ATOMIC_RELAXED, __HIP_MEMORY_SCOPE_AGENT);
      long long spins = 0;
      for (int top = chunk - 1; top >= 0;) {
        const int j = top - lane;
        const int v = j >= 0 ? __hip_atomic_load(state + 1 + j, __ATOMIC_RELAXED, __HIP_MEMORY_SCOPE_AGENT) : SEL_PFX;
        const unsigned long long ready = __ballot((v & 3) != 0), pfx = __ballot((v & 3) == SEL_PFX);
        const int stop = pfx ? __ffsll((long long)pfx) - 1 : 63;
        const unsigned long long need = stop == 63 ? ~0ull : ((1ull << (stop + 1)) - 1ull);
        if ((ready & need) != need) {
          __builtin_amdgcn_s_sleep(1);
          if (++spins > (1ll << 22)) { bad = BLISS_ERR_CAP_KEPT; break; }
          continue;
        }
        excl += wave_total_i32(lane <= stop && j >= 0 ? (v >> 2) : 0);
        if (pfx) break;
        top -= 64;
      }
    }
    if (lane == 0) {
      __hip_atomic_store(state + 1 + chunk, ((excl + tot) << 2) | SEL_PFX, __ATOMIC_RELAXED, __HIP_MEMORY_SCOPE_AGENT);
      sh_base = excl;
      if (chunk == nchunks - 1) {
        int K = excl + tot;
        if (K > cap_k) { bad |= BLISS_ERR_CAP_KEPT; K = cap_k; }
        cnt->K = K;
        sh_K = K;
      }
      if (bad) atomicOr(&cnt->err, bad);
    }
  }
  __syncthreads();
  int run = sh_base + woff;
#pragma unroll
  for (int i = 0; i < ITEMS; ++i) {
    const int j = chunk * CHUNK + (threadIdx.x >> 6) * SPAN + i * 64 + lane_id();
    if (j < C) {
      const bool keep = (mask[i] >> lane_id()) & 1ull;
      const int r = run + __popcll(mask[i] & ((1ull << lane_id()) - 1ull));
      if (keep && r < cap_k) {
        const int g = cand_nid[j];
        kept_nid[r] = g; node_prob[r] = Pv[i]; new_id[j] = r;
        if (kept_map) kept_map[g] = r;
      } else new_id[j] = -1;
    }
    run += __popcll(mask[i]);
  }
  if (chunk == nchunks - 1)
    for (int r = sh_K + threadIdx.x; r < cap_k; r += TPB) { kept_nid[r] = 0; node_prob[r] = 0x3f80; }
}

__global__ void __launch_bounds__(TPB) k_mn_prepare(LayerCounts* cnt, const bf16_t* __restrict__ p, bf16_t* __restrict__ P,
                                                    int* __restrict__ new_id, int cap_c) {
  const int C = min(cnt->C, cap_c);
  for (int j = blockIdx.x * TPB + threadIdx.x; j < C; j += gridDim.x * TPB) { P[j] = p[j]; new_id[j] = 0; }
}
__global__ void __launch_bounds__(TPB) k_mn_mark(LayerCounts* cnt, const int* __restrict__ chosen, int n_chosen, int* __restrict__ new_id, int cap_c) {
  const int C = min(cnt->C, cap_c);
  for (int i = blockIdx.x * TPB + threadIdx.x; i < n_chosen; i += gridDim.x * TPB) {
    const int j = chosen[i];
    if (j >= 0 && j < C) new_id[j] = 1; else atomicOr(&cnt->err, BLISS_ERR_CAP_CAND);
  }
}
template <bool EMIT>
__global__ void __launch_bounds__(TPB) k_mn_select(LayerCounts* cnt, const bf16_t* __restrict__ P, int* __restrict__ chunk_io,
                                                   const int* __restrict__ cand_nid, int* __restrict__ new_id,
                                                   int* __restrict__ kept_nid, bf16_t* __restrict__ node_prob, int cap_c, int cap_k,
                                                   int* __restrict__ kept_map) {
  __shared__ int sh4[TPB / 64];
  const int S = cnt->S, C = min(cnt->C, cap_c);
  const int nchunks = (C + CHUNK - 1) / CHUNK;
  for (int chunk = blockIdx.x; chunk < nchunks; chunk += gridDim.x) {
    unsigned long long mask[ITEMS];
    int drawn[ITEMS];
    int wave_total = 0;
#pragma unroll
    for (int i = 0; i < ITEMS; ++i) {
      const int j = chunk * CHUNK + (threadIdx.x >> 6) * SPAN + i * 64 + lane_id();
      drawn[i] = j < C ? (EMIT ? new_id[j] : new_id[j] == 1) : 0;
      mask[i] = __ballot(j < C && (drawn[i] == 1 || j < S));
      wave_total += __popcll(mask[i]);
    }
    int tot;
    const int woff = chunk_wave_offset(wave_total, sh4, &tot);
    if (!EMIT) { if (threadIdx.x == 0) chunk_io[chunk] = tot; continue; }
    int run = chunk_io[chunk] + woff;
#pragma unroll
    for (int i = 0; i < ITEMS; ++i) {
      const int j = chunk * CHUNK + (threadIdx.x >> 6) * SPAN + i * 64 + lane_id();
      if (j < C) {
        const bool in_u = (mask[i] >> lane_id()) & 1ull;
        const int r = run + __popcll(mask[i] & ((1ull << lane_id()) - 1ull));
        if (in_u && r < cap_k) {
          const int g = cand_nid[j];
          kept_nid[r] = g; node_prob[r] = P[j]; new_id[j] = drawn[i] == 1 ? r : -2 - r;
          if (kept_map && drawn[i] == 1) kept_map[g] = r;
        } else new_id[j] = -1;
      }
      run += __popcll(mask[i]);
    }
  }
  if (EMIT) {
    const int K = min(cnt->K, cap_k);
    for (int r = K + blockIdx.x * TPB + threadIdx.x; r < cap_k; r += gridDim.x * TPB) { kept_nid[r] = 0; node_prob[r] = 0x3f80; }
  }
}

struct KeptRec { int k, pos, nid, lid; };
__device__ __forceinline__ int span_collect(int chunk, int E, int S, const int* __restrict__ seg_ptr,
                                            const long long* __restrict__ col_base, const int* __restrict__ span_seg,
                                            const int* __restrict__ indices, const int* __restrict__ kept_map,
                                            const int* __restrict__ local_id, const int* __restrict__ new_id, KeptRec* buf) {
  int n = 0, hint = span_seg[chunk * ITEMS + (threadIdx.x >> 6)];
#pragma unroll
  for (int i = 0; i < ITEMS; ++i) {
    const int base = chunk * CHUNK + (threadIdx.x >> 6) * SPAN + i * 64;
    if (base >= E) break;
    EdgeAt a = decode(base, E, S, seg_ptr, col_base, indices, &hint);
    int lid = 0, nid = -1;
    if (a.k >= 0) {
      if (kept_map) nid = kept_map[a.src];
      else { lid = local_id[a.src]; nid = new_id[lid]; }
    }
    const unsigned long long mask = __ballot(nid >= 0);
    if (nid >= 0) {
      KeptRec r; r.k = a.k; r.pos = (int)a.pos; r.nid = nid; r.lid = lid;
      buf[n + __popcll(mask & ((1ull << lane_id()) - 1ull))] = r;
    }
    n += __popcll(mask);
  }
  __builtin_amdgcn_fence(__ATOMIC_SEQ_CST, "wavefront"); __builtin_amdgcn_wave_barrier();
  return n;
}

template <bool BANDIT>
__global__ void __launch_bounds__(TPB) k_block_pass1(const int64_t* __restrict__ indptr, const int* __restrict__ indices,
                                                     const bf16_t* __restrict__ w, const int* __restrict__ seeds,
                                                     const int* __restrict__ seg_ptr, const long long* __restrict__ col_base,
    const int* __restrict__ span_seg, LayerCounts* cnt,
                                                     const unsigned long long* __restrict__ acc_w,
                                                     const int* __restrict__ local_id, const int* __restrict__ new_id,
                                                     const bf16_t* __restrict__ P, int* deg_blk, unsigned long long* acc_wt,
                                                     int* __restrict__ chunk_cnt, int* src_cnt, float eta_f, float ome_f,
                                                     const int* __restrict__ kept_map, const bf16_t* __restrict__ node_prob,
                                                     const uint2* __restrict__ seed_coef, KeptRec* __restrict__ kept_rec,
                                                     int* __restrict__ span_cnt, long long kept_rec_positions) {
  __shared__ int sh4[TPB / 64];
  __shared__ KeptRec sh_kept[TPB / 64][SPAN];
  const int S = cnt->S, E = cnt->E;
  if (E > kept_rec_positions) kept_rec = nullptr;
  const int nchunks = (E + CHUNK - 1) / CHUNK;
  KeptRec* buf = sh_kept[threadIdx.x >> 6];
  int bad = 0;
  for (int chunk = blockIdx.x; chunk < nchunks; chunk += gridDim.x) {
    const int n = span_collect(chunk, E, S, seg_ptr, col_base, span_seg, indices, kept_map, local_id, new_id, buf);
    if (kept_rec) {
      const int span = chunk * ITEMS + (threadIdx.x >> 6);
      if (lane_id() == 0) span_cnt[span] = n;
      for (int j = lane_id(); j < n; j += 64) kept_rec[(size_t)span * SPAN + j] = buf[j];
    }
    for (int j0 = 0; j0 < n; j0 += 64) {
      const int j = j0 + lane_id();
      int key = -1;
      int64_t term = 0;
      if (j < n) {
        const KeptRec r = buf[j];
        key = r.k;
        if (src_cnt) atomicAdd(src_cnt + r.nid, 1);
        if (BANDIT) {
          bf16_t q;
          const bf16_t wv = w[r.pos];
          if (seed_coef) { const uint2 cf = seed_coef[r.k]; q = edge_q_pre(wv, (bf16_t)(cf.x & 0xffffu), __uint_as_float(cf.y), ome_f); }
          else q = edge_q(wv, fixed_to_bf((int64_t)acc_w[r.k], FRAC_DST, &bad), seg_ptr[r.k + 1] - seg_ptr[r.k], eta_f, ome_f);
          bf16_t wt = f2bf(bf2f(q) / bf2f(kept_map ? node_prob[r.nid] : P[r.lid]));
          term = bf_to_fixed(wt, FRAC_BLK, &bad);
        }
      }
      wave_segsum_atomic_i32(key, key >= 0, deg_blk);
      if (BANDIT) wave_segsum_atomic_i64(key, term, acc_wt);
    }
    int tot;
    chunk_wave_offset(n, sh4, &tot);
    if (threadIdx.x == 0) chunk_cnt[chunk] = tot;
  }
  if (bad) atomicOr(&cnt->err, bad);
}

__global__ void __launch_bounds__(1024) k_block_scans(int* __restrict__ chunk_cnt, const int* __restrict__ deg_blk, LayerCounts* cnt,
                                                      int* __restrict__ blk_indptr, int cap_s, int cap_b,
                                                      int* __restrict__ src_cnt, int* __restrict__ t_indptr, int cap_k) {
  __shared__ int sh[17];
  if (blockIdx.x == 2) {
    int run = 0;
    for (int base = 0; base <= cap_k; base += blockDim.x) {
      int j = base + threadIdx.x;
      int v = j < cap_k ? src_cnt[j] : 0;
      int tot, ex = block_excl_scan(v, sh, &tot);
      if (j <= cap_k) { t_indptr[j] = run + ex; if (j < cap_k) src_cnt[j] = run + ex; }
      run += tot;
    }
    return;
  }
  if (blockIdx.x == 0) {
    const int n = (cnt->E + CHUNK - 1) / CHUNK;
    int run = 0;
    for (int base = 0; base < n; base += blockDim.x) {
      int i = base + threadIdx.x;
      int v = i < n ? chunk_cnt[i] : 0;
      int tot, ex = block_excl_scan(v, sh, &tot);
      if (i < n) chunk_cnt[i] = run + ex;
      run += tot;
    }
    if (threadIdx.x == 0) {
      if (run > cap_b) { atomicOr(&cnt->err, BLISS_ERR_CAP_EDGES); run = cap_b; }
      cnt->B = run;
    }
    return;
  }
  const int S = cnt->S;
  int run = 0;
  for (int base = 0; base < S; base += blockDim.x) {
    int k = base + threadIdx.x;
    int v = k < S ? deg_blk[k] : 0;
    int tot, ex = block_excl_scan(v, sh, &tot);
    if (k < S) blk_indptr[k] = run + ex;
    run += tot;
  }
  for (int k = S + threadIdx.x; k <= cap_s; k += blockDim.x) blk_indptr[k] = run;
}

template <bool BANDIT>
__global__ void __launch_bounds__(TPB) k_block_pass2(const int64_t* __restrict__ indptr, const int* __restrict__ indices,
                                                     const int* __restrict__ eid_map, const bf16_t* __restrict__ w,
                                                     const int* __restrict__ seeds, const int* __restrict__ seg_ptr, const long long* __restrict__ col_base,
    const int* __restrict__ span_seg, LayerCounts* cnt, const unsigned long long* __restrict__ acc_w,
                                                     const int* __restrict__ local_id, const int* __restrict__ new_id,
                                                     const bf16_t* __restrict__ P, const int* __restrict__ deg_blk,
                                                     const unsigned long long* __restrict__ acc_wt,
                                                     const int* __restrict__ chunk_off, int* __restrict__ out_src,
                                                     int* __restrict__ out_dst, int* __restrict__ out_pos,
                                                     int* __restrict__ out_eid, bf16_t* __restrict__ out_w,
                                                     bf16_t* __restrict__ out_q, int* src_cursor, int* __restrict__ t_unsorted,
                                                     float eta_f, float ome_f, int cap_b, const int* __restrict__ kept_map,
                                                     const bf16_t* __restrict__ node_prob, const uint2* __restrict__ seed_coef,
                                                     const KeptRec* __restrict__ kept_rec, const int* __restrict__ span_cnt,
                                                     long long kept_rec_positions) {
  __shared__ int sh4[TPB / 64];
  __shared__ KeptRec sh_kept[TPB / 64][SPAN];
  const int S = cnt->S, E = cnt->E;
  if (E > kept_rec_positions) kept_rec = nullptr;
  const int nchunks = (E + CHUNK - 1) / CHUNK;
  KeptRec* buf = sh_kept[threadIdx.x >> 6];
  int bad = 0;
  for (int chunk = blockIdx.x; chunk < nchunks; chunk += gridDim.x) {
    const int span = chunk * ITEMS + (threadIdx.x >> 6);
    int n;
    const KeptRec* list = buf;
    if (kept_rec) {
      n = (span * SPAN < E) ? span_cnt[span] : 0;
      list = kept_rec + (size_t)span * SPAN;
    } else n = span_collect(chunk, E, S, seg_ptr, col_base, span_seg, indices, kept_map, local_id, new_id, buf);
    int tot;
    const int run = chunk_off[chunk] + chunk_wave_offset(n, sh4, &tot);
    for (int j = lane_id(); j < n; j += 64) {
      const int idx = run + j;
      if (idx >= cap_b) break;
      const KeptRec r = list[j];
      const int k = r.k;
      bf16_t q;
      const bf16_t wv = w[r.pos];
      if (BANDIT) {
        if (seed_coef) { const uint2 cf = seed_coef[k]; q = edge_q_pre(wv, (bf16_t)(cf.x & 0xffffu), __uint_as_float(cf.y), ome_f); }
        else q = edge_q(wv, fixed_to_bf((int64_t)acc_w[k], FRAC_DST, &bad), seg_ptr[k + 1] - seg_ptr[k], eta_f, ome_f);
      } else q = wv;
      float wt = rbf(bf2f(q) / bf2f(kept_map ? node_prob[r.nid] : P[r.lid]));
      float d = rbf((float)deg_blk[k]);
      float out;
      if (BANDIT) {
        bf16_t wts = fixed_to_bf((int64_t)acc_wt[k], FRAC_BLK, &bad);
        float ratio = rbf(d / bf2f(wts));
        out = wt * ratio;
      } else {
        out = wt * d;
      }
      out_src[idx] = r.nid;
      if (src_cursor) t_unsorted[atomicAdd(src_cursor + r.nid, 1)] = idx;
      out_dst[idx] = k;
      out_pos[idx] = r.pos;
      out_eid[idx] = eid_map ? eid_map[r.pos] : r.pos;
      out_w[idx] = f2bf(out);
      out_q[idx] = q;
    }
    __builtin_amdgcn_fence(__ATOMIC_SEQ_CST, "wavefront"); __builtin_amdgcn_wave_barrier();
  }
  if (bad) atomicOr(&cnt->err, bad);
}

__device__ __forceinline__ void maps_cleanup(LayerCounts* cnt, const int* __restrict__ cand_nid, int* local_id, int cap_c,
                                             const int* __restrict__ kept_nid, int* kept_map, int cap_k) {
  const int C = min(cnt->C, cap_c), K = min(cnt->K, cap_k);
  const int t0 = blockIdx.x * blockDim.x + threadIdx.x, step = gridDim.x * blockDim.x;
  for (int id = t0; id < C; id += step) local_id[cand_nid[id]] = -1;
  if (kept_map) for (int r = t0; r < K; r += step) kept_map[kept_nid[r]] = -1;
}

#define TSORT_MAX_S 32768
__global__ void __launch_bounds__(TPB) k_tr_sort_lists(const int* __restrict__ t_indptr, const int* __restrict__ t_unsorted,
                                                       const int* __restrict__ dst, LayerCounts* cnt, int cap_k, int cap_s,
                                                       int* __restrict__ t_edge, const int* __restrict__ cand_nid, int* local_id,
                                                       int cap_c, const int* __restrict__ kept_nid, int* kept_map, int do_cleanup) {
  extern __shared__ unsigned bm_all[];
  if (do_cleanup) maps_cleanup(cnt, cand_nid, local_id, cap_c, kept_nid, kept_map, cap_k);
  const int lane = lane_id(), wave = threadIdx.x >> 6;
  const int words = (cap_s + 31) / 32;
  unsigned* bm = bm_all + (size_t)wave * (words + 1);
  const int K = min(cnt->K, cap_k);
  for (int j = blockIdx.x * (TPB / 64) + wave; j < K; j += gridDim.x * (TPB / 64)) {
    const int beg = t_indptr[j], len = t_indptr[j + 1] - beg;
    if (len <= 0) continue;
    if (len <= 64) {
      const int v = lane < len ? t_unsorted[beg + lane] : 0x7fffffff;
      int rank = 0;
      for (int k = 0; k < len; ++k) rank += (__shfl(v, k) < v);
      if (lane < len) t_edge[beg + rank] = v;
      continue;
    }
    for (int w = lane; w <= words; w += 64) bm[w] = 0;
    __builtin_amdgcn_fence(__ATOMIC_SEQ_CST, "wavefront"); __builtin_amdgcn_wave_barrier();
    for (int i = lane; i < len; i += 64) { const int d = dst[t_unsorted[beg + i]]; atomicOr(bm + (d >> 5), 1u << (d & 31)); }
    __builtin_amdgcn_fence(__ATOMIC_SEQ_CST, "wavefront"); __builtin_amdgcn_wave_barrier();
    int carry = 0;
    for (int base = 0; base < words; base += 64) {
      const int w = base + lane;
      const unsigned bits = w < words ? bm[w] : 0u;
      int c = __popc(bits), inc = c;
#pragma unroll
      for (int d = 1; d < 64; d <<= 1) { int t = __shfl_up(inc, d); if (lane >= d) inc += t; }
      const int excl = carry + inc - c;
      carry += __shfl(inc, 63);
      for (int i = 0; i < len; i += 64) {
        const int idx = i + lane;
        int e = 0, d = -1;
        if (idx < len) { e = t_unsorted[beg + idx]; d = dst[e]; }
        const int dw = d >> 5;
        const bool mine = idx < len && dw >= base && dw < base + 64;
        const int src_lane = mine ? dw - base : 0;
        const int ex_w = __shfl(excl, src_lane);
        const unsigned bits_w = __shfl((int)bits, src_lane);
        if (mine) t_edge[beg + ex_w + __popc(bits_w & ((1u << (d & 31)) - 1u))] = e;
      }
    }
    __builtin_amdgcn_fence(__ATOMIC_SEQ_CST, "wavefront"); __builtin_amdgcn_wave_barrier();
  }
}

__global__ void __launch_bounds__(TPB) k_cleanup(LayerCounts* cnt, const int* __restrict__ cand_nid, int* local_id, int cap_c,
                                                 const int* __restrict__ kept_nid, int* kept_map, int cap_k) {
  maps_cleanup(cnt, cand_nid, local_id, cap_c, kept_nid, kept_map, cap_k);
}

inline int grid_for(int64_t n, int per_block, int max_blocks = 8192) {
  int64_t g = (n + per_block - 1) / per_block;
  if (g < 1) g = 1;
  if (g > max_blocks) g = max_blocks;
  return (int)g;
}

}

#define CK(x) do { hipError_t e_ = (x); if (e_ != hipSuccess) return (int)e_; } while (0)

static long long g_flag_spin_bound = 1ll << 22;
__global__ void __launch_bounds__(64) k_flag_wait(int* flag, int* err, long long bound) {
  if (threadIdx.x != 0) return;
  long long spins = 0;
  while (__hip_atomic_load(flag, __ATOMIC_RELAXED, __HIP_MEMORY_SCOPE_AGENT) == 0) {
    __builtin_amdgcn_s_sleep(8);
    if (++spins > bound) { if (err) atomicOr(err, BLISS_ERR_FLAG_TIMEOUT); break; }
  }
  __builtin_amdgcn_fence(__ATOMIC_ACQUIRE, "agent");
  __hip_atomic_store(flag, 0, __ATOMIC_RELAXED, __HIP_MEMORY_SCOPE_AGENT);
}

__global__ void k_flag_raise(int* flag) {
  if (threadIdx.x == 0) __hip_atomic_store(flag, 1, __ATOMIC_RELEASE, __HIP_MEMORY_SCOPE_AGENT);
}

extern "C" {

int bliss_layer_counts_bytes(void) { return (int)sizeof(LayerCounts); }

int bliss_flag_raise(int32_t* flag, void* stream) {
  if (!flag) return BLISS_EINVAL;
  k_flag_raise<<<1, 64, 0, (hipStream_t)stream>>>(flag);
  return (int)hipGetLastError();
}

int bliss_flag_wait(int32_t* flag, int32_t* err_word, void* stream) {
  if (!flag) return BLISS_EINVAL;
  k_flag_wait<<<1, 64, 0, (hipStream_t)stream>>>(flag, err_word, g_flag_spin_bound);
  return (int)hipGetLastError();
}

int bliss_flag_set_spin_bound(int64_t spins) {
  if (spins < 1) return BLISS_EINVAL;
  g_flag_spin_bound = spins;
  return 0;
}

int bliss_frontier_prob(const bliss_graph_t* g, const bliss_node_maps_t* m, const void* w_pos, const int32_t* seeds,
                        int32_t n_seeds, const int32_t* n_seeds_dev, int32_t cap_s, int mode, float eta_f,
                        float one_minus_eta_f, int64_t frontier_bound, const bliss_layer_ws_t* ws, void* stream_) {
  if (!g || !m || !seeds || !ws || !w_pos || cap_s <= 0 || !ws->hist || !ws->span_seg) return BLISS_EINVAL;
  if (n_seeds < 0 && !n_seeds_dev) return BLISS_EINVAL;
  if (n_seeds > cap_s) return BLISS_EINVAL;
  const int uniform_nodes = (mode & BLISS_MODE_UNIFORM_NODES) ? 1 : 0;
  const bool partials_only = (mode & BLISS_MODE_PARTIALS) != 0;
  mode &= ~(BLISS_MODE_UNIFORM_NODES | BLISS_MODE_PARTIALS);
  if (mode != BLISS_MODE_BANDIT && mode != BLISS_MODE_LADIES) return BLISS_EINVAL;
  if (partials_only && ws->n_bins <= 0) return BLISS_EINVAL;
  hipStream_t st = (hipStream_t)stream_;
  LayerCounts* cnt = (LayerCounts*)ws->counts;
  const bf16_t* w = (const bf16_t*)w_pos;
  unsigned long long* acc_w = (unsigned long long*)ws->seed_acc;
  unsigned long long* acc_q = acc_w + cap_s;
  const long long* col_base = (const long long*)(acc_w + 5 * (size_t)cap_s);
  if (frontier_bound < 1) frontier_bound = 1;
  const int ge = grid_for(frontier_bound, TPB), gc = grid_for(frontier_bound, CHUNK);
  const bool binned = ws->n_bins > 0;
  int log2_bins = 0, slots = 0;
  if (binned) {
    while ((1 << log2_bins) < ws->n_bins) ++log2_bins;
    slots = (g->num_nodes + ws->n_bins - 1) >> log2_bins;
    if ((1 << log2_bins) != ws->n_bins || ws->n_bins > MAX_BINS || (size_t)slots * 12 > 64 * 1024 || ws->bin_cap <= 0 ||
        g->num_edges > (long long)MAX_TILES * BTILE * 32 || !ws->bin_cursor || !ws->bin_rec || !ws->bitmap || !ws->word_prefix || !ws->touched_key || !ws->touched_sum)
      return BLISS_EINVAL;
  }
  const long long fcap = (long long)(g->num_edges < 0x7fffffffll ? g->num_edges : 0x7fffffffll);
  const bool col_sums = binned && mode == BLISS_MODE_BANDIT;
  int* long_list = (int*)(acc_w + 7 * (size_t)cap_s);
  PROF_LAUNCH(BK_SEG_SCAN, st, k_seg_scan<<<1 + SEG_ZERO_WGS, 1024, 0, st>>>(g->indptr, seeds, cnt, n_seeds, n_seeds_dev, cap_s, acc_w, ws->seg_ptr,
                                                            m->local_id, g->num_nodes, ws->src_cnt, ws->cap_k,
                                                            binned ? ws->bin_cursor : nullptr, ws->n_bins, (long long*)col_base, ws->span_seg,
                                                            fcap, ws->entry_flag, col_sums ? 1 : 0, col_sums ? long_list : nullptr));
  if (binned) {
    unsigned long long* seed_p2 = acc_w + 4 * (size_t)cap_s;
    uint2* seed_coef = (uint2*)(acc_w + 6 * (size_t)cap_s);
    unsigned long long* bin_rec = (unsigned long long*)ws->bin_rec;
    const int gb = grid_for(frontier_bound, BIN_BATCH);
    const int n_wave_wgs = grid_for(cap_s, COL_TPB / 64, 2048);
    if (col_sums)
      PROF_LAUNCH(BK_COL_SUMS, st, k_col_sums<<<n_wave_wgs + (cap_s < 2048 ? cap_s : 2048), COL_TPB, 0, st>>>(g->indptr, w, seeds, ws->seg_ptr, col_base, ws->span_seg, cnt, acc_w, acc_q, eta_f, one_minus_eta_f, seed_coef, n_wave_wgs, long_list, cap_s));
    if (mode == BLISS_MODE_BANDIT)
      PROF_LAUNCH(BK_BIN_SCATTER, st, k_bin_scatter<true><<<gb, BIN_TPB, 0, st>>>(g->indptr, g->indices, w, seeds, ws->seg_ptr, col_base, ws->span_seg, cnt, acc_w, acc_q, eta_f, one_minus_eta_f, uniform_nodes, ws->n_bins, log2_bins, ws->bin_cap, ws->bin_cursor, bin_rec, ws->bitmap, seed_coef));
    else
      PROF_LAUNCH(BK_BIN_SCATTER, st, k_bin_scatter<false><<<gb, BIN_TPB, 0, st>>>(g->indptr, g->indices, w, seeds, ws->seg_ptr, col_base, ws->span_seg, cnt, acc_w, acc_q, eta_f, one_minus_eta_f, uniform_nodes, ws->n_bins, log2_bins, ws->bin_cap, ws->bin_cursor, bin_rec, ws->bitmap, seed_coef));
    PROF_LAUNCH(BK_BIN_REDUCE, st, k_bin_reduce<<<ws->n_bins, BINRED_TPB, (size_t)slots * 12, st>>>(
        cnt, ws->n_bins, log2_bins, ws->bin_cap, ws->bin_cursor, bin_rec, g->num_nodes, slots, m->local_id, seed_p2,
        (unsigned long long*)ws->touched_key, (unsigned long long*)ws->touched_sum, ws->bitmap, ws->cap_c));
    if (partials_only) return (int)hipGetLastError();
    int* tile_sum = ws->word_prefix;
    int* word_prefix = ws->word_prefix + MAX_TILES;
    PROF_LAUNCH(BK_BITMAP_SCAN, st, k_bitmap_tiles<<<grid_for(frontier_bound, (int64_t)BTILE * 32, MAX_TILES), 1024, 0, st>>>(ws->bitmap, word_prefix, tile_sum, cnt));
    int gf = (ws->cap_c + FIN_TPB - 1) / FIN_TPB;
    if (gf < 1) gf = 1;
    if (gf > 512) gf = 512;
    PROF_LAUNCH(BK_CAND_NUMBER, st, k_cand_number<<<gf, FIN_TPB, 0, st>>>(
        seeds, cnt, ws->cand_nid, m->local_id, seed_p2, (const unsigned long long*)ws->touched_key,
        (const unsigned long long*)ws->touched_sum, ws->bitmap, word_prefix, tile_sum, (bf16_t*)ws->p, ws->hist, ws->cap_c, uniform_nodes,
        FusedScale{ws->fs_ticket, ws->fs_fanout, ws->fs_eps, ws->fs_rng_ctl, ws->fs_layer_off, ws->fs_is_last, ws->fs_rng_cap, ws->chunk_cnt}));
    return (int)hipGetLastError();
  }
  if (mode == BLISS_MODE_BANDIT) {
    PROF_LAUNCH(BK_PASS1, st, k_frontier_pass1<true><<<ge, TPB, 0, st>>>(g->indptr, g->indices, w, seeds, ws->seg_ptr, col_base, ws->span_seg, cnt, m->local_id, m->first_pos, acc_w));
    PROF_LAUNCH(BK_PASS2, st, k_frontier_pass2<true><<<gc, TPB, 0, st>>>(g->indptr, g->indices, w, seeds, ws->seg_ptr, col_base, ws->span_seg, cnt, m->first_pos, acc_w, acc_q, ws->chunk_cnt, eta_f, one_minus_eta_f));
  } else {
    PROF_LAUNCH(BK_PASS1, st, k_frontier_pass1<false><<<ge, TPB, 0, st>>>(g->indptr, g->indices, w, seeds, ws->seg_ptr, col_base, ws->span_seg, cnt, m->local_id, m->first_pos, acc_w));
    PROF_LAUNCH(BK_PASS2, st, k_frontier_pass2<false><<<gc, TPB, 0, st>>>(g->indptr, g->indices, w, seeds, ws->seg_ptr, col_base, ws->span_seg, cnt, m->first_pos, acc_w, acc_q, ws->chunk_cnt, eta_f, one_minus_eta_f));
  }
  PROF_LAUNCH(BK_CHUNK_SCAN, st, k_chunk_scan<<<1, 1024, 0, st>>>(ws->chunk_cnt, cnt, 0, ws->cap_c));
  if (mode == BLISS_MODE_BANDIT)
    PROF_LAUNCH(BK_PASS3, st, k_frontier_pass3<true><<<gc, TPB, 0, st>>>(g->indptr, g->indices, w, seeds, ws->seg_ptr, col_base, ws->span_seg, cnt, m->first_pos, acc_w, acc_q, ws->chunk_cnt, m->local_id, ws->cand_nid, (unsigned long long*)m->acc_p2, eta_f, one_minus_eta_f, ws->cap_c, uniform_nodes));
  else
    PROF_LAUNCH(BK_PASS3, st, k_frontier_pass3<false><<<gc, TPB, 0, st>>>(g->indptr, g->indices, w, seeds, ws->seg_ptr, col_base, ws->span_seg, cnt, m->first_pos, acc_w, acc_q, ws->chunk_cnt, m->local_id, ws->cand_nid, (unsigned long long*)m->acc_p2, eta_f, one_minus_eta_f, ws->cap_c, uniform_nodes));
  {
    int gf = (ws->cap_c + FIN_TPB * 8 - 1) / (FIN_TPB * 8);
    if (gf < 1) gf = 1;
    if (gf > 256) gf = 256;
    PROF_LAUNCH(BK_CAND_FINALIZE, st, k_cand_finalize<<<gf, FIN_TPB, 0, st>>>(
        seeds, cnt, ws->cand_nid, (unsigned long long*)m->acc_p2, m->first_pos, (bf16_t*)ws->p, ws->hist, ws->cap_c, uniform_nodes));
  }
  return (int)hipGetLastError();
}

int bliss_poisson_select(const bliss_layer_ws_t* ws, int32_t fanout, double eps, const float* uniforms,
                         int32_t* uniforms_offset_dev, int32_t* rng_ctl, int is_last, int32_t rng_cap_total,
                         int64_t cand_bound, void* stream_) {
  if (!ws || !uniforms || fanout < 0 || (rng_ctl && !uniforms_offset_dev)) return BLISS_EINVAL;
  hipStream_t st = (hipStream_t)stream_;
  LayerCounts* cnt = (LayerCounts*)ws->counts;
  if (cand_bound < 1) cand_bound = 1;
  if (cand_bound > ws->cap_c) cand_bound = ws->cap_c;
  if (!ws->fs_ticket)
    PROF_LAUNCH(BK_POISSON_SCALE, st, k_poisson_scale<<<1, 1024, 0, st>>>(ws->hist, cnt, fanout, eps, rng_ctl, uniforms_offset_dev, is_last, rng_cap_total, ws->chunk_cnt));
  PROF_LAUNCH(BK_SELECT2, st, k_select_fused<<<grid_for(cand_bound, CHUNK, 1 << 20), TPB, 0, st>>>(
      (const bf16_t*)ws->p, uniforms, uniforms_offset_dev, cnt, (bf16_t*)ws->P, ws->chunk_cnt, ws->cand_nid, ws->new_id, ws->kept_nid,
      (bf16_t*)ws->node_prob, ws->cap_c, ws->cap_k, ws->kept_map));
  return (int)hipGetLastError();
}

int bliss_poisson_scale(int32_t* hist, void* counts, int32_t fanout, double eps, int32_t* scratch, void* stream_) {
  if (!hist || !counts || !scratch || fanout < 0) return BLISS_EINVAL;
  hipStream_t st = (hipStream_t)stream_;
  PROF_LAUNCH(BK_POISSON_SCALE, st, k_poisson_scale<<<1, 1024, 0, st>>>(hist, (LayerCounts*)counts, fanout, eps, nullptr, nullptr, 0, 0, scratch));
  return (int)hipGetLastError();
}

int bliss_multinomial_select(const bliss_layer_ws_t* ws, const int32_t* chosen, int32_t n_chosen, void* stream_) {
  if (!ws || n_chosen < 0 || (n_chosen > 0 && !chosen)) return BLISS_EINVAL;
  hipStream_t st = (hipStream_t)stream_;
  LayerCounts* cnt = (LayerCounts*)ws->counts;
  const int gc = grid_for(ws->cap_c, CHUNK), ge = grid_for(ws->cap_c, TPB);
  k_mn_prepare<<<ge, TPB, 0, st>>>(cnt, (const bf16_t*)ws->p, (bf16_t*)ws->P, ws->new_id, ws->cap_c);
  if (n_chosen > 0) k_mn_mark<<<grid_for(n_chosen, TPB), TPB, 0, st>>>(cnt, chosen, n_chosen, ws->new_id, ws->cap_c);
  k_mn_select<false><<<gc, TPB, 0, st>>>(cnt, (const bf16_t*)ws->P, ws->chunk_cnt, ws->cand_nid, ws->new_id, ws->kept_nid, (bf16_t*)ws->node_prob, ws->cap_c, ws->cap_k, ws->kept_map);
  k_chunk_scan<<<1, 1024, 0, st>>>(ws->chunk_cnt, cnt, 1, ws->cap_k);
  k_mn_select<true><<<gc, TPB, 0, st>>>(cnt, (const bf16_t*)ws->P, ws->chunk_cnt, ws->cand_nid, ws->new_id, ws->kept_nid, (bf16_t*)ws->node_prob, ws->cap_c, ws->cap_k, ws->kept_map);
  return (int)hipGetLastError();
}

int bliss_build_block(const bliss_graph_t* g, const bliss_node_maps_t* m, const void* w_pos, const int32_t* seeds,
                      int32_t cap_s, int mode, float eta_f, float one_minus_eta_f, int64_t frontier_bound,
                      const bliss_layer_ws_t* ws, const bliss_block_out_t* out, void* stream_) {
  if (!g || !m || !seeds || !ws || !out || !w_pos || cap_s <= 0 || !ws->span_seg) return BLISS_EINVAL;
  mode &= ~BLISS_MODE_UNIFORM_NODES;
  if (mode != BLISS_MODE_BANDIT && mode != BLISS_MODE_LADIES) return BLISS_EINVAL;
  hipStream_t st = (hipStream_t)stream_;
  LayerCounts* cnt = (LayerCounts*)ws->counts;
  const bf16_t* w = (const bf16_t*)w_pos;
  unsigned long long* acc_w = (unsigned long long*)ws->seed_acc;
  unsigned long long* acc_wt = acc_w + 2 * (size_t)cap_s;
  int* deg_blk = (int*)(acc_w + 3 * (size_t)cap_s);
  const long long* col_base = (const long long*)(acc_w + 5 * (size_t)cap_s);
  const uint2* seed_coef = (ws->n_bins > 0 && mode == BLISS_MODE_BANDIT) ? (const uint2*)(acc_w + 6 * (size_t)cap_s) : nullptr;
  if (frontier_bound < 1) frontier_bound = 1;
  const int gc = grid_for(frontier_bound, CHUNK);
  KeptRec* kept_rec = (ws->kept_rec && ws->span_cnt && frontier_bound <= ws->kept_rec_positions) ? (KeptRec*)ws->kept_rec : nullptr;
  int* src_cnt = ws->src_cnt;
  const bool want_t = src_cnt && out->t_indptr && out->t_edge && out->t_scratch;
  if (want_t && cap_s > TSORT_MAX_S) return BLISS_EINVAL;
  int* sc = want_t ? src_cnt : nullptr;
  if (mode == BLISS_MODE_BANDIT)
    PROF_LAUNCH(BK_BLOCK1, st, k_block_pass1<true><<<gc, TPB, 0, st>>>(g->indptr, g->indices, w, seeds, ws->seg_ptr, col_base, ws->span_seg, cnt, acc_w, m->local_id, ws->new_id, (const bf16_t*)ws->P, deg_blk, acc_wt, ws->chunk_cnt, sc, eta_f, one_minus_eta_f, ws->kept_map, (const bf16_t*)ws->node_prob, seed_coef, kept_rec, ws->span_cnt, (long long)ws->kept_rec_positions));
  else
    PROF_LAUNCH(BK_BLOCK1, st, k_block_pass1<false><<<gc, TPB, 0, st>>>(g->indptr, g->indices, w, seeds, ws->seg_ptr, col_base, ws->span_seg, cnt, acc_w, m->local_id, ws->new_id, (const bf16_t*)ws->P, deg_blk, acc_wt, ws->chunk_cnt, sc, eta_f, one_minus_eta_f, ws->kept_map, (const bf16_t*)ws->node_prob, seed_coef, kept_rec, ws->span_cnt, (long long)ws->kept_rec_positions));
  PROF_LAUNCH(BK_INDPTR_SCAN, st, k_block_scans<<<want_t ? 3 : 2, 1024, 0, st>>>(ws->chunk_cnt, deg_blk, cnt, out->indptr, cap_s, out->cap_b, src_cnt, out->t_indptr, ws->cap_k));
  if (mode == BLISS_MODE_BANDIT)
    PROF_LAUNCH(BK_BLOCK2, st, k_block_pass2<true><<<gc, TPB, 0, st>>>(g->indptr, g->indices, g->eid, w, seeds, ws->seg_ptr, col_base, ws->span_seg, cnt, acc_w, m->local_id, ws->new_id, (const bf16_t*)ws->P, deg_blk, acc_wt, ws->chunk_cnt, out->src, out->dst, out->pos, out->eid, (bf16_t*)out->edge_weights, (bf16_t*)out->q_ij, sc, out->t_scratch, eta_f, one_minus_eta_f, out->cap_b, ws->kept_map, (const bf16_t*)ws->node_prob, seed_coef, kept_rec, ws->span_cnt, (long long)ws->kept_rec_positions));
  else
    PROF_LAUNCH(BK_BLOCK2, st, k_block_pass2<false><<<gc, TPB, 0, st>>>(g->indptr, g->indices, g->eid, w, seeds, ws->seg_ptr, col_base, ws->span_seg, cnt, acc_w, m->local_id, ws->new_id, (const bf16_t*)ws->P, deg_blk, acc_wt, ws->chunk_cnt, out->src, out->dst, out->pos, out->eid, (bf16_t*)out->edge_weights, (bf16_t*)out->q_ij, sc, out->t_scratch, eta_f, one_minus_eta_f, out->cap_b, ws->kept_map, (const bf16_t*)ws->node_prob, seed_coef, kept_rec, ws->span_cnt, (long long)ws->kept_rec_positions));
  if (want_t && ws->block_ready_flag) {
    PROF_LAUNCH(BK_CLEANUP, st, k_cleanup<<<grid_for(ws->cap_c, TPB), TPB, 0, st>>>(cnt, ws->cand_nid, m->local_id, ws->cap_c, ws->kept_nid, ws->kept_map, ws->cap_k));
    k_flag_raise<<<1, 64, 0, st>>>(ws->block_ready_flag);
    const size_t lds = (size_t)(TPB / 64) * ((cap_s + 31) / 32 + 1) * sizeof(unsigned);
    PROF_LAUNCH(BK_TRANSPOSE, st, k_tr_sort_lists<<<grid_for(ws->cap_k, TPB / 64), TPB, lds, st>>>(out->t_indptr, out->t_scratch, out->dst, cnt, ws->cap_k, cap_s, out->t_edge, ws->cand_nid, m->local_id, ws->cap_c, ws->kept_nid, ws->kept_map, 0));
  } else if (want_t) {
    const size_t lds = (size_t)(TPB / 64) * ((cap_s + 31) / 32 + 1) * sizeof(unsigned);
    PROF_LAUNCH(BK_TRANSPOSE, st, k_tr_sort_lists<<<grid_for(ws->cap_k, TPB / 64), TPB, lds, st>>>(out->t_indptr, out->t_scratch, out->dst, cnt, ws->cap_k, cap_s, out->t_edge, ws->cand_nid, m->local_id, ws->cap_c, ws->kept_nid, ws->kept_map, 1));
    if (ws->block_ready_flag) k_flag_raise<<<1, 64, 0, st>>>(ws->block_ready_flag);
  } else {
    PROF_LAUNCH(BK_CLEANUP, st, k_cleanup<<<grid_for(ws->cap_c, TPB), TPB, 0, st>>>(cnt, ws->cand_nid, m->local_id, ws->cap_c, ws->kept_nid, ws->kept_map, ws->cap_k));
    if (ws->block_ready_flag) k_flag_raise<<<1, 64, 0, st>>>(ws->block_ready_flag);
  }
  return (int)hipGetLastError();
}

}
```

bliss_gnn_amd/roofline.py:

```python
import ctypes as C

from . import _lib

HBM_PEAK_GBPS = 8000.0


def kernel_names():
    n = _lib.lib.bliss_prof_kernel_count()
    return [_lib.lib.bliss_prof_kernel_name(i).decode() for i in range(n)]


def algorithmic_bytes(kernel, s, dims=None, layer=None):
    S, E, Cn, K, B = s["S"], s["E"], s["C"], s["K"], s["B"]
    D = dims[layer] if dims is not None and layer is not None else 0
    table = {
        "k_frontier_pass1": 6 * E + 8 * S,
        "k_frontier_pass2": 6 * E + 16 * S,
        "k_frontier_pass3": 6 * E + 16 * S + 12 * Cn,
        "k_col_sums": 2 * E + 24 * S,
        "k_bin_scatter": 6 * E + 16 * S,
        "k_bin_reduce": 12 * Cn,
        "k_cand_number": 14 * Cn,
        "k_block_pass1": 6 * E + 16 * S + 6 * Cn,
        "k_block_pass2": 6 * E + 16 * S + 6 * Cn + 20 * B,
        "k_cand_finalize": 14 * Cn,
        "k_poisson_scale": 2 * Cn,
        "k_select_pass1": 8 * Cn, "k_select_pass2": 12 * Cn + 6 * K,
        "k_mt19937_uniform": 4 * Cn,
        "k_spmm_fwd": 4 * (S + 1) + 6 * B + 2 * K * D + 2 * S * D,
        "k_spmm_bwd": 4 * (K + 1) + 10 * B + 2 * S * D + 2 * K * D,
        "k_exp3_update": 12 * B + 4 * K + 4 * S,
        "k_embed_norm": 2 * K * D + 2 * K,
    }
    return table.get(kernel)


class KernelTimer:
    def __init__(self):
        self.names = kernel_names()

    def enable(self, which):
        idx = {"all": -1, "off": -2}.get(which)
        if idx is None:
            idx = self.names.index(which)
        _lib.check(_lib.lib.bliss_prof_enable(idx), "bliss_prof_enable")
        _lib.check(_lib.lib.bliss_prof_reset(), "bliss_prof_reset")

    def read(self):
        out = {}
        for i, n in enumerate(self.names):
            ms, cnt = C.c_double(), C.c_int64()
            _lib.check(_lib.lib.bliss_prof_read(i, C.byref(ms), C.byref(cnt)), "bliss_prof_read")
            if cnt.value:
                out[n] = dict(total_ms=ms.value, launches=cnt.value, avg_us=1e3 * ms.value / cnt.value)
        return out
```

include/bliss_gnn.h:

```cpp
#ifndef BLISS_GNN_H
#define BLISS_GNN_H
#include <stdint.h>

#ifdef __cplusplus
extern "C" {
#endif

#define BLISS_EINVAL (-1)

#define BLISS_MODE_BANDIT 0
#define BLISS_MODE_LADIES 1
#define BLISS_ROWSUM_SLOTS 32
#define BLISS_NORM_SCRATCH (2 + 3 * BLISS_ROWSUM_SLOTS)
#define BLISS_MODE_UNIFORM_NODES 4
#define BLISS_MODE_PARTIALS 8

typedef struct {
  const int64_t* indptr;
  const int32_t* indices;
  const int32_t* eid;
  int32_t num_nodes;
  int64_t num_edges;
} bliss_graph_t;

typedef struct {
  int32_t* local_id;
  uint32_t* first_pos;
  uint64_t* acc_p2;
} bliss_node_maps_t;

typedef struct {
  int32_t S, E, C, K, B;
  int32_t err;
  int32_t iters;
  int32_t all_one;
  double c;
} bliss_layer_counts_t;

typedef struct {
  void* counts;
  int32_t* seg_ptr;
  void* seed_acc;
  int32_t* chunk_cnt;
  int32_t* cand_nid;
  void* p;
  void* P;
  int32_t* new_id;
  int32_t* kept_nid;
  void* node_prob;
  int32_t* hist;
  int32_t* src_cnt;
  int32_t cap_c, cap_k;
  int32_t n_bins;
  int64_t bin_cap;
  int32_t* bin_cursor;
  uint64_t* bin_rec;
  uint32_t* bitmap;
  int32_t* word_prefix;
  uint64_t* touched_key;
  uint64_t* touched_sum;
  int32_t* span_seg;
  void* kept_rec;
  int32_t* span_cnt;
  int64_t kept_rec_positions;
  int32_t* kept_map;
  int32_t* entry_flag;
  int32_t* fs_ticket; int32_t fs_fanout, fs_is_last, fs_rng_cap, fs_reserved; double fs_eps; int32_t* fs_rng_ctl; int32_t* fs_layer_off;
  int32_t* block_ready_flag;
} bliss_layer_ws_t;

typedef struct {
  int32_t* indptr;
  int32_t* src;
  int32_t* dst;
  int32_t* pos;
  int32_t* eid;
  void* edge_weights;
  void* q_ij;
  int32_t* t_indptr;
  int32_t* t_edge;
  int32_t* t_scratch;
  int32_t cap_b;
} bliss_block_out_t;

int bliss_layer_counts_bytes(void);

int bliss_flag_wait(int32_t* flag, int32_t* err_word, void* stream);
int bliss_flag_set_spin_bound(int64_t spins);
int bliss_flag_raise(int32_t* flag, void* stream);

int bliss_frontier_prob(const bliss_graph_t* g, const bliss_node_maps_t* maps, const void* w_pos,
                        const int32_t* seeds, int32_t n_seeds, const int32_t* n_seeds_dev, int32_t cap_s, int mode,
                        float eta_f, float one_minus_eta_f, int64_t frontier_bound, const bliss_layer_ws_t* ws,
                        void* stream);

int bliss_poisson_select(const bliss_layer_ws_t* ws, int32_t fanout, double eps, const float* uniforms,
                         int32_t* uniforms_offset_dev, int32_t* rng_ctl, int is_last, int32_t rng_cap_total,
                         int64_t cand_bound, void* stream);

int bliss_multinomial_select(const bliss_layer_ws_t* ws, const int32_t* chosen, int32_t n_chosen, void* stream);

int bliss_build_block(const bliss_graph_t* g, const bliss_node_maps_t* maps, const void* w_pos,
                      const int32_t* seeds, int32_t cap_s, int mode, float eta_f, float one_minus_eta_f,
                      int64_t frontier_bound, const bliss_layer_ws_t* ws, const bliss_block_out_t* out, void* stream);

int bliss_mt19937_uniform(void* state, const int32_t* n_dev, int32_t n_word_offset, float* out, int32_t cap, void* stream);

int bliss_rng_stream_begin(const void* state, int32_t* ctl, float* out, uint32_t* raw, int32_t cap_total, void* stream);
int bliss_rng_prepare(int32_t cap_total, int32_t* plan4);
int bliss_mt_jump_poly(int64_t n_words, uint32_t* poly_words);
int bliss_rng_stream_wait(int32_t* ctl, const void* counts, int32_t* layer_off, int is_last, int32_t cap_total, void* stream);
int bliss_rng_stream_end(void* state, const int32_t* ctl, const uint32_t* raw, int32_t cap_total, int32_t* err_word,
                         void* stream);
int bliss_rng_stream_chain(void* state, int32_t* ctl, float* out, uint32_t* raw, int32_t cap_total, int32_t* counts_dev,
                           int32_t n_count_words, int32_t* counts_host, void* stream);
int bliss_rng_stream_ready(void* stream);
int64_t bliss_rng_stream_handle(void);

int bliss_cand_importance(const int64_t* sums, int32_t n, int uniform_nodes, void* p_bf16, int32_t* err, void* stream);
int bliss_poisson_scale(int32_t* hist, void* counts, int32_t fanout, double eps, int32_t* scratch, void* stream);
int bliss_keyed_select(const int32_t* nid, const void* p_bf16, const uint8_t* is_seed, int32_t n, const void* counts,
                       uint64_t seed, uint64_t step, int32_t layer, void* P_bf16, uint8_t* keep, void* stream);
int bliss_shard_local_seeds(const int32_t* seeds_g, int32_t n_seeds, const int32_t* n_seeds_dev, int32_t lo, int32_t hi, int32_t cap_s,
                            int32_t* seeds_l, int32_t* seeds_l_copy, int32_t* seed_pos, int32_t* n_local_dev, int32_t* err, void* stream);
int bliss_shard_scatter_partials(const int32_t* seeds_l, const int64_t* seed_p2, const int32_t* n_local_dev, const int64_t* touched_key,
                                 const int64_t* touched_sum, const int32_t* n_touched_dev, int64_t* dense, int32_t num_nodes,
                                 int32_t* err, void* stream);
int bliss_shard_pack_rows(const int32_t* nid, const int32_t* n_rows_dev, int32_t cap_rows, int32_t lo, int32_t hi, const void* table_bf16,
                          int64_t table_stride, int32_t row_len, void* out_bf16, int64_t out_stride, void* stream);
int bliss_shard_place_rows(const void* src_bf16, int64_t src_stride, const int32_t* pos, const int32_t* n_dev, int32_t cap_s, void* out_bf16,
                           int64_t out_stride, int32_t n_rows, int32_t row_len, void* stream);
int bliss_shard_take_rows(const void* src, int32_t src_is_f32, int64_t src_stride, int32_t n_src_rows, const int32_t* pos, const int32_t* n_dev,
                          int32_t cap_s, void* out_bf16, int64_t out_stride, int32_t row_len, void* stream);
int bliss_shard_zero_dense(int64_t* dense, int32_t num_nodes, void* stream);
int bliss_shard_candidates(int64_t* dense, int32_t num_nodes, int32_t uniform_nodes, int32_t* cand_nid, void* p_bf16, uint8_t* is_seed,
                           int32_t* hist, void* counts, int32_t cap_c, int32_t* scratch, int32_t* err, void* stream);
int bliss_shard_select_kept(const int32_t* cand_nid, const void* p_bf16, const uint8_t* is_seed, const void* counts, uint64_t seed,
                            int64_t* step_dev, int32_t layer, const int32_t* seeds_g, int32_t n_seeds, const int32_t* n_seeds_dev,
                            void* P_bf16, int32_t* kept_nid, void* node_prob_bf16, int32_t* kept_map, int32_t cap_k, int32_t cap_c,
                            int32_t num_nodes, void* layer_counts, const int32_t* n_local_dev, int32_t* scratch, int32_t bump_step,
                            int32_t* done_flag, int32_t* err, void* stream);
int bliss_exp3_normalize_global(void* w_pos, int64_t num_edges, int64_t* row_sum, const int64_t* norm_limbs, int64_t* scratch,
                                void* norm_out_bf16, void* stream);

typedef struct {
  const void* a1; int64_t a1_stride; const int32_t* ids;
  const void* w1; int64_t w1_stride; int32_t k1;
  const void* a2; int64_t a2_stride; const void* w2; int64_t w2_stride; int32_t k2;
  const void* bias;
  int32_t m_bound; const int32_t* m_dev; int32_t n;
  void* out; int64_t out_stride;
  void* a_copy; int64_t copy_stride;
  void* in_norm; void* out_norm;
  int32_t relu; float drop_p; uint32_t drop_seed; void* drop_ctr;
} bliss_tile_gemm_t;
int bliss_tile_gemm(const bliss_tile_gemm_t* first, const bliss_tile_gemm_t* second_or_null, void* stream);

typedef struct {
  const void* a1; int64_t a1_stride; const void* w1; int64_t w1_stride; int32_t k1;
  const void* a2; int64_t a2_stride; const void* w2; int64_t w2_stride; int32_t k2; int32_t m2_bound; const int32_t* m2_dev;
  int32_t m_bound; const int32_t* m_dev; int32_t n;
  void* out; int64_t out_stride;
} bliss_dgrad_t;
int bliss_sage_dgrad(const bliss_dgrad_t* args, void* stream);
typedef struct {
  const void* d; int64_t d_stride; int32_t n_out;
  const void* x; int64_t x_stride; int32_t k_in;
  int32_t rows_bound; const int32_t* rows_dev;
  void* dw; int64_t dw_stride; void* db;
} bliss_wgrad_t;
int64_t bliss_sage_wgrad_workspace(const bliss_wgrad_t* probs, int32_t n_probs);
int bliss_sage_wgrad(const bliss_wgrad_t* probs, int32_t n_probs, float* partials, int64_t partial_floats, void* stream);

int bliss_cross_entropy(const void* logits, int64_t stride, const int64_t* labels, int32_t n_rows, int32_t n_cls,
                        float* row_loss, void* dlogits, int64_t d_stride, float* loss_out, uint32_t* ticket, int32_t* err,
                        void* stream);
int bliss_cross_entropy_sum(const void* logits, int64_t stride, const void* logits2, int64_t stride2, const int64_t* label_table,
                            const int32_t* label_ids, int32_t n_rows, int32_t n_cls, float* row_loss, void* dlogits, int64_t d_stride,
                            float* loss_out, uint32_t* ticket, int32_t* err, void* stream);
int bliss_cross_entropy_masked(const void* logits, int64_t stride, const void* logits2, int64_t stride2, const int64_t* label_table,
                               int32_t n_table, const int32_t* label_ids, int32_t id_off, int32_t n_rows, const int32_t* n_rows_dev,
                               float denom, int32_t n_cls, float* row_loss, void* dlogits, int64_t d_stride, float* loss_out,
                               uint32_t* ticket, int32_t* err, void* stream);

#define BLISS_ADAM_MAX_TENSORS 32
typedef struct {
  void* param[BLISS_ADAM_MAX_TENSORS];
  const void* grad[BLISS_ADAM_MAX_TENSORS];
  void* exp_avg[BLISS_ADAM_MAX_TENSORS];
  void* exp_avg_sq[BLISS_ADAM_MAX_TENSORS];
  int64_t numel[BLISS_ADAM_MAX_TENSORS];
  int32_t count;
} bliss_adam_t;
int bliss_adam_step(const bliss_adam_t* tensors, float* state, float beta1, float beta2, float eps, float weight_decay, void* stream);

int bliss_normalized_edata(const bliss_graph_t* g, void* w_pos, void* stream);

int bliss_gather_rows(const void* feat, int64_t feat_stride, const int32_t* ids, int32_t n_rows, int32_t dim, void* out,
                      int64_t out_stride, void* norm_out, void* stream);

int bliss_embed_norm(const void* h, int32_t n_rows, int32_t dim, int64_t row_stride, void* out, void* stream);

int bliss_spmm_chunk_edges(int32_t nnz_bound);
int bliss_spmm_fwd(const int32_t* indptr, const int32_t* src, const int32_t* dst, const void* w, const void* h,
                   int64_t h_stride, int32_t n_dst, const int32_t* nnz_dev, int32_t nnz, int32_t dim, int mean, void* out,
                   int64_t out_stride, int out_fp32, float* partials, void* stream);

int bliss_spmm_bwd(const int32_t* t_indptr, const int32_t* t_edge, const int32_t* src, const int32_t* dst,
                   const int32_t* indptr, const void* w, const void* gout, int64_t gout_stride, int32_t n_src,
                   const int32_t* nnz_dev, int32_t nnz, int32_t dim, int mean, void* gh, int64_t gh_stride, int out_fp32,
                   float* partials, void* stream);

int bliss_sage_epilogue_fwd(const void* a, int64_t a_stride, const void* b, int64_t b_stride, int32_t n_rows, int32_t dim,
                            float p_drop, uint32_t seed, uint64_t* ctr, void* out, int64_t out_stride, void* norm_out, void* stream);
int bliss_sage_epilogue_bwd(const void* dout, int64_t dout_stride, const void* out, int64_t out_stride, int32_t n_rows, int32_t dim,
                            float p_drop, void* din, int64_t din_stride, void* stream);

int64_t bliss_block_transpose_temp_bytes(int32_t cap_b, int32_t n_src_cap);
int bliss_block_transpose(const int32_t* src, const int32_t* nnz_dev, int32_t nnz, int32_t cap_b, int32_t n_src_cap,
                          int32_t* t_indptr, int32_t* t_edge, void* temp, int64_t temp_bytes, void* stream);

int64_t bliss_graph_prepare_capacity(int64_t n_edges, int32_t num_nodes, int undirected);
int64_t bliss_graph_prepare_temp_bytes(int64_t n_edges, int32_t num_nodes, int undirected);
int bliss_graph_prepare(const int32_t* coo_src, const int32_t* coo_dst, int64_t n_edges, int32_t num_nodes, int undirected,
                        int64_t* indptr, int32_t* indices, int32_t* eid, int64_t* n_out, int32_t* err, void* temp,
                        int64_t temp_bytes, void* stream);

int bliss_exp3_update(const bliss_graph_t* g, const void* edge_w_pos, void* w_pos, int64_t* row_sum,
                      const int32_t* blk_indptr, const int32_t* blk_src, const int32_t* blk_dst,
                      const int32_t* blk_pos, const void* q_ij, const void* node_prob, const void* embed_norm,
                      const void* alpha_or_null, const int32_t* dst_nid, int32_t n_dst, const int32_t* n_edges_dev,
                      int32_t edges_bound, float delta_f, void* rewards_out, void* factor_out, int apply,
                      int32_t* err, void* stream);

#define BLISS_EXP3_MAX_BLOCKS 8
typedef struct {
  void* w_pos; int64_t* row_sum; int64_t* scratch; void* norm_out;
  const int32_t *blk_indptr, *blk_src, *blk_dst, *blk_pos;
  const void *q_ij, *node_prob, *embed_norm, *alpha_or_null;
  const int32_t* dst_nid; const int32_t* n_edges_dev;
  void* rewards_out;
  int32_t edges_bound;
} bliss_exp3_block_t;
int bliss_exp3_step(const bliss_graph_t* g, const void* edge_w_pos, const bliss_exp3_block_t* blocks, int32_t n_blocks,
                    float delta_f, int32_t* err, void* stream);
int bliss_exp3_update_blocks(const bliss_graph_t* g, const void* edge_w_pos, const bliss_exp3_block_t* blocks, int32_t n_blocks,
                             float delta_f, int32_t* err, void* stream);
int bliss_exp3_normalize_global_rows(const bliss_exp3_block_t* rows, int32_t n_rows, int64_t num_edges, const int64_t* norm_limbs,
                                     int64_t limb_stride, void* stream);

int bliss_exp3_apply(void* w_pos, int64_t* row_sum, const int32_t* pos, const void* factor, const int32_t* n_dev,
                     int32_t n_bound, int32_t* err, void* stream);

typedef struct {
  void* w_pos[BLISS_EXP3_MAX_BLOCKS];
  int64_t* row_sum[BLISS_EXP3_MAX_BLOCKS];
  int32_t pos_off_words[BLISS_EXP3_MAX_BLOCKS], factor_off_bf16[BLISS_EXP3_MAX_BLOCKS], count_off_words[BLISS_EXP3_MAX_BLOCKS],
      bound[BLISS_EXP3_MAX_BLOCKS];
  int32_t n_blocks, n_ranks;
  int64_t rank_stride_words;
} bliss_exp3_rank_lists_t;
int bliss_exp3_apply_ranks(const bliss_exp3_rank_lists_t* lists, const int32_t* gathered, int32_t* barrier, int32_t* err, void* stream);

typedef struct {
  const int32_t* pos[BLISS_EXP3_MAX_BLOCKS];
  const int32_t* n_dev[BLISS_EXP3_MAX_BLOCKS];
  int32_t pos_off_words[BLISS_EXP3_MAX_BLOCKS], count_off_words[BLISS_EXP3_MAX_BLOCKS], bound[BLISS_EXP3_MAX_BLOCKS];
  int32_t n_blocks;
} bliss_pack_lists_t;
int bliss_pack_lists(const bliss_pack_lists_t* lists, int32_t* buf, void* stream);

int bliss_exp3_normalize(void* w_pos, int64_t num_edges, int64_t* row_sum, int64_t* scratch, void* norm_out_bf16,
                         void* stream);

int bliss_row_sum(const void* w_pos, int64_t num_edges, int64_t* row_sum, void* stream);

int bliss_gat_chunk_edges(void);
int bliss_gat_logits(const int32_t* src, const int32_t* dst, const int32_t* nnz_dev, int32_t nnz, const void* feat,
                     int64_t feat_stride, const void* attn, int32_t heads, int32_t head_dim, float negative_slope, void* e_out,
                     void* stream);
typedef struct {
  const int32_t* indptr; const int32_t* src; int32_t n_dst; const int32_t* n_dst_dev;
  const void* feat; int64_t feat_stride; const void* attn; int32_t heads; int32_t head_dim; float negative_slope;
  void* e; void* a; void* a_drop;
  void* rst; int64_t rst_stride;
  float drop_p; uint32_t drop_seed; void* drop_ctr; void* drop_ctr_used;
  const void* g; int64_t g_stride; void* de; void* d_er; int64_t d_er_stride; float* dattn_part;
  const int32_t* wg_row; const int32_t* n_wg_dev; int32_t cap_wg; void* row_ws; float* seg_part; int32_t* err;
} bliss_gat_fused_t;
int bliss_gat_segment_edges(void);
int bliss_gat_fused_stamps(long long* stamps, long long* stamps_bwd);
int bliss_gat_segments(const int32_t* indptr, int32_t n_dst, int32_t cap_wg, int32_t* wg_row, int32_t* n_wg_dev, int32_t* err, void* stream);
int bliss_gat_fused_supported(int32_t heads, int32_t head_dim);
int bliss_gat_rows_src_fused(const int32_t* t_indptr, int32_t n_src, const int32_t* t_edge, const int32_t* src, const int32_t* dst,
                             const int32_t* nnz_dev, int32_t nnz, const void* de, const void* a_drop, const void* feat, int64_t feat_stride,
                             const void* g, int64_t g_stride, const void* attn, int32_t heads, int32_t head_dim, float negative_slope,
                             void* out, int64_t out_stride, float* partials, void* stream);
int bliss_gat_fused_fwd(const bliss_gat_fused_t* args, void* stream);
int bliss_gat_fused_bwd_dst(const bliss_gat_fused_t* args, float* block_sums, float* d_attn, uint32_t* ticket, void* stream);
int bliss_gat_logits_f32(const int32_t* src, const int32_t* dst, const int32_t* nnz_dev, int32_t nnz, const void* feat,
                         int64_t feat_stride, const void* attn, int32_t heads, int32_t head_dim, float negative_slope, float* e_out,
                         void* stream);
int bliss_gat_edge_dot(const int32_t* src, const int32_t* dst, const int32_t* nnz_dev, int32_t nnz, const void* feat,
                       int64_t feat_stride, const void* g, int64_t g_stride, int32_t heads, int32_t head_dim, void* out, void* stream);
int bliss_gat_edge_softmax(const int32_t* indptr, int32_t n_dst, const void* x, const void* a_or_null, int32_t heads, int backward,
                           void* out, void* stream);
int bliss_gat_rows(int which, const int32_t* row_ptr, int32_t n_rows, const int32_t* t_edge, const int32_t* src, const int32_t* dst,
                   const int32_t* nnz_dev, int32_t nnz, const void* coef, const void* feat, int64_t feat_stride, const void* attn,
                   int32_t heads, int32_t head_dim, float negative_slope, void* out, int64_t out_stride, float* partials,
                   float* d_attn, void* stream);
int bliss_gat_alpha(const int32_t* indptr, int32_t n_dst, const void* q_ij, const void* a_ij, void* alpha_out, int32_t* err, void* stream);

int bliss_prof_enable(int kernel_id);
int bliss_prof_reset(void);
int bliss_prof_read(int kernel_id, double* total_ms, int64_t* launches);
int bliss_prof_kernel_count(void);
const char* bliss_prof_kernel_name(int kernel_id);

#ifdef __cplusplus
}
#endif
#endif
```

Before: 1463.

## Fuse candidate importance into bin reduce and merge numbering with selection

In the binned sampling path, the bin-reduce kernel now computes each candidate's importance, writes a packed candidate record indexed by first-position, and builds the histogram directly. This removes the separate touched-key/sum buffers and the k_cand_number kernel. The Poisson scale runs as an extra workgroup inside the bitmap-tile scan kernel. A new k_cand_select kernel numbers candidates from the bitmap prefix and performs the keep/drop selection in one pass. The intent is fewer launches and fewer global round-trips per layer, at the cost of a larger per-word candidate record buffer and a more complex scan kernel.

```diff
diff --git a/bliss_gnn_amd/_engine.py b/bliss_gnn_amd/_engine.py
--- a/bliss_gnn_amd/_engine.py
+++ b/bliss_gnn_amd/_engine.py
@@ -57,7 +57,6 @@
         self.c_graph = _lib.Graph(g.indptr.data_ptr(), g.indices.data_ptr(), _ptr(g.eid), V, self.Eg)
         self.flags = torch.zeros(16, dtype=torch.int32, device=dev)
         self.fs_ticket = torch.zeros(1, dtype=torch.int32, device=dev)
-        self.fuse_scale = os.environ.get("BLISS_FUSE_SCALE", "1") != "0"
         self.flag_err = torch.zeros(1, dtype=torch.int32, device=dev)
         self.n_bins = 0
         for nb in ((int(os.environ["BLISS_NBINS"]),) if os.environ.get("BLISS_NBINS") else (256, 1024)):
@@ -128,6 +127,7 @@
                               rec=torch.empty(nb * cap, dtype=torch.int64, device=dev),
                               bitmap=torch.zeros(words, dtype=torch.int32, device=dev),
                               prefix=torch.empty(2048 + words, dtype=torch.int32, device=dev),
+                              crec=torch.empty(words * 32, dtype=torch.int64, device=dev),
                               tkey=torch.empty(self.V, dtype=torch.int64, device=dev),
                               tsum=torch.empty(self.V, dtype=torch.int64, device=dev))
         return self._bins
@@ -303,6 +303,7 @@
             c_ws.bin_cursor, c_ws.bin_rec = b["cursor"].data_ptr(), b["rec"].data_ptr()
             c_ws.bitmap, c_ws.word_prefix = b["bitmap"].data_ptr(), b["prefix"].data_ptr()
             c_ws.touched_key, c_ws.touched_sum = b["tkey"].data_ptr(), b["tsum"].data_ptr()
+            c_ws.cand_rec, c_ws.fs_local_id = b["crec"].data_ptr(), sset["local_id"].data_ptr()
         c_out = _lib.BlockOut(b_indptr.data_ptr(), b_src.data_ptr(), b_dst.data_ptr(), b_pos.data_ptr(), b_eid.data_ptr(),
                               b_w.data_ptr(), b_q.data_ptr(), _ptr(t_indptr), _ptr(t_edge), _ptr(t_scr), cb)
         lay = (b_indptr, b_src, b_dst, b_pos, b_eid, b_w, b_q, kept_nid, node_prob, counts[10 * n:10 * n + 10], t_indptr, t_edge)
@@ -430,7 +431,7 @@
             if part == "main":
                 c_ws.entry_flag = self.flags.data_ptr() + 4 * n
             if part in (None, "main"):
-                if self.n_bins and self.fuse_scale:
+                if self.n_bins:
                     c_ws.fs_ticket = self.fs_ticket.data_ptr()
                     c_ws.fs_fanout, c_ws.fs_eps = int(fanouts[n]), float(eps)
                     if use_rng:
diff --git a/bliss_gnn_amd/_lib.py b/bliss_gnn_amd/_lib.py
--- a/bliss_gnn_amd/_lib.py
+++ b/bliss_gnn_amd/_lib.py
@@ -44,6 +44,7 @@
                 ("kept_map", C.c_void_p), ("entry_flag", C.c_void_p),
                 ("fs_ticket", C.c_void_p), ("fs_fanout", C.c_int32), ("fs_is_last", C.c_int32), ("fs_rng_cap", C.c_int32),
                 ("fs_reserved", C.c_int32), ("fs_eps", C.c_double), ("fs_rng_ctl", C.c_void_p), ("fs_layer_off", C.c_void_p),
+                ("cand_rec", C.c_void_p), ("fs_local_id", C.c_void_p),
                 ("block_ready_flag", C.c_void_p)]
 
 
diff --git a/bliss_gnn_amd/csrc/prof.h b/bliss_gnn_amd/csrc/prof.h
--- a/bliss_gnn_amd/csrc/prof.h
+++ b/bliss_gnn_amd/csrc/prof.h
@@ -5,7 +5,7 @@
   BK_SEG_SCAN = 0, BK_PASS1, BK_PASS2, BK_CHUNK_SCAN, BK_PASS3, BK_CAND_FINALIZE, BK_POISSON_SCALE, BK_SELECT1, BK_SELECT2,
   BK_BLOCK1, BK_INDPTR_SCAN, BK_BLOCK2, BK_CLEANUP, BK_MT19937, BK_SPMM_FWD, BK_SPMM_BWD, BK_EMBED_NORM, BK_EXP3_UPDATE,
   BK_EXP3_APPLY, BK_NORMALIZE, BK_ROW_SUM, BK_NORM_EDATA, BK_TRANSPOSE, BK_SPMM_FIXUP, BK_COL_SUMS, BK_BIN_SCATTER, BK_BIN_REDUCE,
-  BK_BITMAP_SCAN, BK_CAND_NUMBER, BK_COUNT
+  BK_BITMAP_SCAN, BK_CAND_NUMBER, BK_CAND_SELECT, BK_COUNT
 };
 
 extern int g_bliss_prof_sel;
diff --git a/bliss_gnn_amd/csrc/prof.hip b/bliss_gnn_amd/csrc/prof.hip
--- a/bliss_gnn_amd/csrc/prof.hip
+++ b/bliss_gnn_amd/csrc/prof.hip
@@ -16,7 +16,7 @@
   "k_select_pass1", "k_select_pass2", "k_block_pass1", "k_indptr_scan", "k_block_pass2", "k_cleanup", "k_mt19937_uniform",
   "k_spmm_fwd", "k_spmm_bwd", "k_embed_norm", "k_exp3_update", "k_exp3_apply", "k_normalize_row", "k_row_sum",
   "k_normalized_edata", "k_block_transpose", "k_spmm_fixup", "k_col_sums", "k_bin_scatter", "k_bin_reduce", "k_bitmap_scan",
-  "k_cand_number"};
+  "k_cand_number", "k_cand_select"};
 thread_local Pair t_cur;
 
 void drain_locked() {
diff --git a/bliss_gnn_amd/csrc/sampler.hip b/bliss_gnn_amd/csrc/sampler.hip
--- a/bliss_gnn_amd/csrc/sampler.hip
+++ b/bliss_gnn_amd/csrc/sampler.hip
@@ -321,6 +321,29 @@
 #ifndef FIN_TPB
 #define FIN_TPB 1024
 #endif
+__device__ __forceinline__ bf16_t cand_importance(unsigned long long raw, int uniform_nodes, int* bad) {
+  if (uniform_nodes) return raw ? (bf16_t)0x3f80 : (bf16_t)0;
+  return f2bf(sqrtf(bf2f(fixed_to_bf((int64_t)raw, FRAC_SRC, bad))));
+}
+__device__ __forceinline__ void hist_count(bf16_t pj, int* lh, int* hist, int* bad) {
+  if (pj >= HIST_BINS) *bad |= BLISS_ERR_NONFINITE;
+  else if ((unsigned)(pj - HWIN_LO) < (unsigned)HWIN_N) atomicAdd(&lh[pj - HWIN_LO], 1);
+  else if (pj == 0) atomicAdd(&lh[HWIN_N], 1);
+  else atomicAdd(hist + pj, 1);
+}
+__device__ __forceinline__ void hist_flush(const int* lh, int* hist) {
+  const int4* lh4 = reinterpret_cast<const int4*>(lh);
+  for (int b = threadIdx.x; b < HWIN_N / 4; b += blockDim.x) {
+    const int4 v = lh4[b];
+    if (v.x | v.y | v.z | v.w) {
+      if (v.x) atomicAdd(hist + HWIN_LO + 4 * b, v.x);
+      if (v.y) atomicAdd(hist + HWIN_LO + 4 * b + 1, v.y);
+      if (v.z) atomicAdd(hist + HWIN_LO + 4 * b + 2, v.z);
+      if (v.w) atomicAdd(hist + HWIN_LO + 4 * b + 3, v.w);
+    }
+  }
+  if (threadIdx.x == 0 && lh[HWIN_N]) atomicAdd(hist, lh[HWIN_N]);
+}
 __global__ void __launch_bounds__(FIN_TPB) k_cand_finalize(const int* __restrict__ seeds, LayerCounts* cnt, int* __restrict__ cand_nid,
                                                            unsigned long long* acc_p2, unsigned* first_pos,
                                                            bf16_t* __restrict__ p, int* hist, int cap_c, int uniform_nodes) {
@@ -606,19 +629,23 @@
   if (bad) atomicOr(&cnt->err, bad);
 }
 
+template <bool FUSED>
 __global__ void __launch_bounds__(BINRED_TPB) k_bin_reduce(LayerCounts* cnt, int n_bins, int log2_bins, long long bin_cap,
                                                            int* bin_cursor, const unsigned long long* __restrict__ bin_rec,
                                                            int num_nodes, int slots,
                                                            const int* __restrict__ local_id, unsigned long long* __restrict__ seed_p2,
                                                            unsigned long long* __restrict__ touched_key,
-                                                           unsigned long long* __restrict__ touched_sum, unsigned* bitmap, int cap_c) {
+                                                           unsigned long long* __restrict__ touched_sum, unsigned* bitmap, int cap_c,
+                                                           unsigned long long* __restrict__ cand_rec, int* hist, int uniform_nodes) {
   extern __shared__ unsigned long long dyn_lds[];
+  __shared__ int lh[FUSED ? HWIN_N + 4 : 4];
   unsigned long long* sm = dyn_lds;
   unsigned* mn = (unsigned*)(dyn_lds + slots);
   const int b = blockIdx.x, tid = threadIdx.x;
   if (cnt->E == 0) return;
   const int ne = b < num_nodes ? ((num_nodes - 1 - b) >> log2_bins) + 1 : 0;
   for (int i = tid; i < ne; i += BINRED_TPB) { sm[i] = 0ull; mn[i] = 0xffffffffu; }
+  if (FUSED) for (int i = tid; i < HWIN_N + 4; i += BINRED_TPB) lh[i] = 0;
   __syncthreads();
   long long n = bin_cursor[b];
   if (n > bin_cap) n = bin_cap;
@@ -637,37 +664,165 @@
   __syncthreads();
   for (int li = tid; li < ne; li += BINRED_TPB) {
     bool is_cand = false;
-    if (mn[li] != 0xffffffffu) {
-      const int lid = local_id[((unsigned)li << log2_bins) | (unsigned)b];
+    const unsigned fp = mn[li];
+    if (fp != 0xffffffffu) {
+      const unsigned g = ((unsigned)li << log2_bins) | (unsigned)b;
+      const int lid = local_id[g];
       if (lid >= 0) { seed_p2[lid] = sm[li]; mn[li] = 0xffffffffu; }
-      else is_cand = true;
+      else {
+        is_cand = true;
+        if (FUSED) {
+          const bf16_t pj = cand_importance(sm[li], uniform_nodes, &bad);
+          cand_rec[fp] = ((unsigned long long)pj << 32) | g;
+          atomicOr(bitmap + (fp >> 5), 1u << (fp & 31u));
+          hist_count(pj, lh, hist, &bad);
+        }
+      }
     }
     const unsigned long long mask = __ballot(is_cand);
     if (mask && lane_id() == 0) atomicAdd(&wg_cnt, __popcll(mask));
   }
   __syncthreads();
   if (tid == 0) { wg_base = wg_cnt ? atomicAdd(bin_cursor + n_bins, wg_cnt) : 0; wg_cnt = 0; }
-  __syncthreads();
-  for (int li = tid; li < ne; li += BINRED_TPB) {
-    const unsigned fp = mn[li];
-    if (fp != 0xffffffffu) {
-      const int j = wg_base + atomicAdd(&wg_cnt, 1);
-      if (j < cap_c) { touched_key[j] = ((unsigned long long)fp << 32) | (((unsigned)li << log2_bins) | (unsigned)b); touched_sum[j] = sm[li]; }
-      atomicOr(bitmap + (fp >> 5), 1u << (fp & 31u));
+  if (FUSED) {
+    hist_flush(lh, hist);
+  } else {
+    __syncthreads();
+    for (int li = tid; li < ne; li += BINRED_TPB) {
+      const unsigned fp = mn[li];
+      if (fp != 0xffffffffu) {
+        const int j = wg_base + atomicAdd(&wg_cnt, 1);
+        if (j < cap_c) { touched_key[j] = ((unsigned long long)fp << 32) | (((unsigned)li << log2_bins) | (unsigned)b); touched_sum[j] = sm[li]; }
+        atomicOr(bitmap + (fp >> 5), 1u << (fp & 31u));
+      }
     }
   }
   if (bad) atomicOr(&cnt->err, bad);
+}
+
+__device__ __forceinline__ double block_sum_f64(double v, double* shd) {
+  for (int d = 32; d >= 1; d >>= 1) {
+    long long b = __double_as_longlong(v);
+    int lo = __shfl_down((int)(b & 0xffffffffll), d), hi = __shfl_down((int)(b >> 32), d);
+    v += __longlong_as_double(((long long)hi << 32) | (unsigned)lo);
+  }
+  __syncthreads();
+  if (lane_id() == 0) shd[threadIdx.x >> 6] = v;
+  __syncthreads();
+  double t = 0;
+  for (int i = 0; i < (int)(blockDim.x >> 6); ++i) t += shd[i];
+  return t;
+}
+
+template <bool COHERENT>
+__device__ __forceinline__ void poisson_scale_body(int* hist, LayerCounts* cnt, int C, int num, double eps, const int* lh, double* shd) {
+  int n[HIST_BINS / 1024];
+  bool any = false;
+#pragma unroll
+  for (int i = 0; i < HIST_BINS / 1024; ++i) {
+    const int b = i * 1024 + threadIdx.x;
+    n[i] = COHERENT ? __hip_atomic_load(hist + b, __ATOMIC_RELAXED, __HIP_MEMORY_SCOPE_AGENT) : hist[b];
+  }
+#pragma unroll
+  for (int i = 0; i < HIST_BINS / 1024; ++i) {
+    const int b = i * 1024 + threadIdx.x;
+    if (n[i]) {
+      if (COHERENT) __hip_atomic_store(hist + b, 0, __ATOMIC_RELAXED, __HIP_MEMORY_SCOPE_AGENT); else hist[b] = 0;
+    }
+    if (lh) {
+      if ((unsigned)(b - HWIN_LO) < (unsigned)HWIN_N) n[i] += lh[b - HWIN_LO];
+      else if (b == 0) n[i] += lh[HWIN_N];
+    }
+    if (n[i]) any = true;
+  }
+  if (C <= num) {
+    if (threadIdx.x == 0) { cnt->c = 1.0; cnt->all_one = 1; cnt->iters = 0; }
+    return;
+  }
+  double c = 1.0;
+  int it = 0;
+  for (; it < 50; ++it) {
+    const float c32 = (float)c;
+    double loc = 0;
+    if (any) {
+#pragma unroll
+      for (int i = 0; i < HIST_BINS / 1024; ++i) {
+        if (n[i]) {
+          float v = rbf(bf2f((bf16_t)(i * 1024 + threadIdx.x)) * c32);
+          v = v < 1.0f ? v : (v != v ? v : 1.0f);
+          loc += (double)n[i] * (double)v;
+        }
+      }
+    }
+    double Ssum = block_sum_f64(loc, shd);
+    double lo = Ssum < (double)num ? Ssum : (double)num, hi = Ssum < (double)num ? (double)num : Ssum;
+    if (lo / hi >= eps) { ++it; break; }
+    c *= (double)num / Ssum;
+  }
+  if (threadIdx.x == 0) { cnt->c = c; cnt->all_one = 0; cnt->iters = it > 50 ? 50 : it; }
+}
+
+__global__ void __launch_bounds__(1024) k_poisson_scale(int* hist, LayerCounts* cnt, int num, double eps, int* rng_ctl,
+                                                        int* layer_off, int is_last, int rng_cap_total, int* __restrict__ sel_state) {
+  __shared__ double shd[16];
+  const int C = cnt->C;
+  for (int i = threadIdx.x; i < (C + CHUNK - 1) / CHUNK + 2; i += 1024) sel_state[i] = 0;
+  if (rng_ctl && threadIdx.x == 1023) rng_stream_acquire(rng_ctl, C, layer_off, is_last, rng_cap_total);
+  poisson_scale_body<false>(hist, cnt, C, num, eps, nullptr, shd);
 }
 
 #define BTILE_W 4
 #define BTILE (1024 * BTILE_W)
 #define MAX_TILES 2048
+#define SEL_WORDS TPB
+static_assert(BTILE % SEL_WORDS == 0, "a chunk of k_cand_select lies inside one bitmap tile");
+__device__ __forceinline__ int sel_chunks(int E) {
+  const int n = (((E + 31) >> 5) + SEL_WORDS - 1) / SEL_WORDS;
+  return n > 0 ? n : 1;
+}
+
+struct ScaleTask {
+  int* hist; const int* seeds; const unsigned long long* seed_p2; const int* n_new; int* cand_nid; bf16_t* p;
+  int cap_c, uniform_nodes, num; double eps; int* rng_ctl; int* layer_off; int is_last, rng_cap_total; int* sel_state;
+};
+__device__ __forceinline__ void scale_workgroup(const ScaleTask& sc, LayerCounts* cnt, int* lh, double* shd) {
+  const int tid = threadIdx.x, S = cnt->S;
+  int C = S + *sc.n_new;
+  if (C > sc.cap_c) { C = sc.cap_c; if (tid == 0) atomicOr(&cnt->err, BLISS_ERR_CAP_CAND); }
+  if (tid == 0) cnt->C = C;
+  for (int i = tid; i < HWIN_N + 4; i += 1024) lh[i] = 0;
+  for (int i = tid; i < sel_chunks(cnt->E) + 2; i += 1024) sc.sel_state[i] = 0;
+  __syncthreads();
+  int bad = 0;
+  if (tid >= 1024 - 64) {
+    if (sc.rng_ctl && tid == 1023) rng_stream_acquire(sc.rng_ctl, C, sc.layer_off, sc.is_last, sc.rng_cap_total);
+  } else {
+    for (int i = tid; i < min(S, C); i += 1024 - 64) {
+      sc.cand_nid[i] = sc.seeds[i];
+      const bf16_t pj = cand_importance(sc.seed_p2[i], sc.uniform_nodes, &bad);
+      sc.p[i] = pj;
+      hist_count(pj, lh, sc.hist, &bad);
+    }
+  }
+  if (bad) atomicOr(&cnt->err, bad);
+  asm volatile("s_waitcnt vmcnt(0)" ::: "memory");
+  __syncthreads();
+  poisson_scale_body<true>(sc.hist, cnt, C, sc.num, sc.eps, lh, shd);
+}
+
 __global__ void __launch_bounds__(1024) k_bitmap_tiles(const unsigned* __restrict__ bitmap, int* __restrict__ word_prefix,
-                                                       int* __restrict__ tile_sum, LayerCounts* cnt) {
+                                                       int* __restrict__ tile_sum, LayerCounts* cnt, const ScaleTask sc) {
   __shared__ int sh[17];
+  __shared__ int lh[HWIN_N + 4];
+  __shared__ double shd[16];
+  int n_tile_wgs = gridDim.x;
+  if (sc.hist) {
+    --n_tile_wgs;
+    if ((int)blockIdx.x == n_tile_wgs) { scale_workgroup(sc, cnt, lh, shd); return; }
+  }
   const int nw = (cnt->E + 31) >> 5;
   const int ntiles = (nw + BTILE - 1) / BTILE;
-  for (int tile = blockIdx.x; tile < ntiles; tile += gridDim.x) {
+  for (int tile = blockIdx.x; tile < ntiles; tile += n_tile_wgs) {
     const int i = tile * BTILE + threadIdx.x * BTILE_W;
     uint4 v = make_uint4(0, 0, 0, 0);
     if (i < nw) v = *reinterpret_cast<const uint4*>(bitmap + i);
@@ -678,82 +833,13 @@
   }
 }
 
-__device__ __forceinline__ double block_sum_f64(double v, double* shd) {
-  for (int d = 32; d >= 1; d >>= 1) {
-    long long b = __double_as_longlong(v);
-    int lo = __shfl_down((int)(b & 0xffffffffll), d), hi = __shfl_down((int)(b >> 32), d);
-    v += __longlong_as_double(((long long)hi << 32) | (unsigned)lo);
-  }
-  __syncthreads();
-  if (lane_id() == 0) shd[threadIdx.x >> 6] = v;
-  __syncthreads();
-  double t = 0;
-  for (int i = 0; i < (int)(blockDim.x >> 6); ++i) t += shd[i];
-  return t;
-}
-
-template <bool COHERENT>
-__device__ __forceinline__ void poisson_scale_body(int* hist, LayerCounts* cnt, int C, int num, double eps, int* rng_ctl,
-                                                   int* layer_off, int is_last, int rng_cap_total, int* __restrict__ sel_state,
-                                                   double* shd) {
-  for (int i = threadIdx.x; i < (C + CHUNK - 1) / CHUNK + 2; i += 1024) sel_state[i] = 0;
-  if (rng_ctl && threadIdx.x == 1023) rng_stream_acquire(rng_ctl, C, layer_off, is_last, rng_cap_total);
-  int n[HIST_BINS / 1024];
-  bool any = false;
-#pragma unroll
-  for (int i = 0; i < HIST_BINS / 1024; ++i) {
-    const int b = i * 1024 + threadIdx.x;
-    n[i] = COHERENT ? __hip_atomic_load(hist + b, __ATOMIC_RELAXED, __HIP_MEMORY_SCOPE_AGENT) : hist[b];
-  }
-#pragma unroll
-  for (int i = 0; i < HIST_BINS / 1024; ++i) {
-    const int b = i * 1024 + threadIdx.x;
-    if (n[i]) {
-      if (COHERENT) __hip_atomic_store(hist + b, 0, __ATOMIC_RELAXED, __HIP_MEMORY_SCOPE_AGENT); else hist[b] = 0;
-      any = true;
-    }
-  }
-  if (C <= num) {
-    if (threadIdx.x == 0) { cnt->c = 1.0; cnt->all_one = 1; cnt->iters = 0; }
-    return;
-  }
-  double c = 1.0;
-  int it = 0;
-  for (; it < 50; ++it) {
-    const float c32 = (float)c;
-    double loc = 0;
-    if (any) {
-#pragma unroll
-      for (int i = 0; i < HIST_BINS / 1024; ++i) {
-        if (n[i]) {
-          float v = rbf(bf2f((bf16_t)(i * 1024 + threadIdx.x)) * c32);
-          v = v < 1.0f ? v : (v != v ? v : 1.0f);
-          loc += (double)n[i] * (double)v;
-        }
-      }
-    }
-    double Ssum = block_sum_f64(loc, shd);
-    double lo = Ssum < (double)num ? Ssum : (double)num, hi = Ssum < (double)num ? (double)num : Ssum;
-    if (lo / hi >= eps) { ++it; break; }
-    c *= (double)num / Ssum;
-  }
-  if (threadIdx.x == 0) { cnt->c = c; cnt->all_one = 0; cnt->iters = it > 50 ? 50 : it; }
-}
-
-__global__ void __launch_bounds__(1024) k_poisson_scale(int* hist, LayerCounts* cnt, int num, double eps, int* rng_ctl,
-                                                        int* layer_off, int is_last, int rng_cap_total, int* __restrict__ sel_state) {
-  __shared__ double shd[16];
-  poisson_scale_body<false>(hist, cnt, cnt->C, num, eps, rng_ctl, layer_off, is_last, rng_cap_total, sel_state, shd);
-}
-
-struct FusedScale { int* ticket; int num; double eps; int* rng_ctl; int* layer_off; int is_last; int rng_cap_total; int* sel_state; };
 __global__ void __launch_bounds__(FIN_TPB) k_cand_number(const int* __restrict__ seeds, LayerCounts* cnt, int* __restrict__ cand_nid,
                                                          int* local_id, const unsigned long long* __restrict__ seed_p2,
                                                          const unsigned long long* __restrict__ touched_key,
                                                          const unsigned long long* __restrict__ touched_sum,
                                                          const unsigned* __restrict__ bitmap, const int* __restrict__ word_prefix,
                                                          const int* __restrict__ tile_sum, bf16_t* __restrict__ p, int* hist,
-                                                         int cap_c, int uniform_nodes, const FusedScale fs) {
+                                                         int cap_c, int uniform_nodes) {
   __shared__ int lh[HWIN_N + 4];
   __shared__ int tile_off[MAX_TILES];
   __shared__ int sh[17];
@@ -790,57 +876,53 @@
       if (id >= cap_c) continue;
       local_id[g] = id; cand_nid[id] = (int)g;
     }
-    bf16_t pj;
-    if (uniform_nodes) pj = raw ? (bf16_t)0x3f80 : (bf16_t)0;
-    else pj = f2bf(sqrtf(bf2f(fixed_to_bf((int64_t)raw, FRAC_SRC, &bad))));
+    const bf16_t pj = cand_importance(raw, uniform_nodes, &bad);
     p[id] = pj;
-    if (pj >= HIST_BINS) bad |= BLISS_ERR_NONFINITE;
-    else if ((unsigned)(pj - HWIN_LO) < (unsigned)HWIN_N) atomicAdd(&lh[pj - HWIN_LO], 1);
-    else if (pj == 0) atomicAdd(&lh[HWIN_N], 1);
-    else atomicAdd(hist + pj, 1);
-  }
-  __syncthreads();
-  {
-    const int4* lh4 = reinterpret_cast<const int4*>(lh);
-    for (int b = threadIdx.x; b < HWIN_N / 4; b += FIN_TPB) {
-      const int4 v = lh4[b];
-      if (v.x | v.y | v.z | v.w) {
-        if (v.x) atomicAdd(hist + HWIN_LO + 4 * b, v.x);
-        if (v.y) atomicAdd(hist + HWIN_LO + 4 * b + 1, v.y);
-        if (v.z) atomicAdd(hist + HWIN_LO + 4 * b + 2, v.z);
-        if (v.w) atomicAdd(hist + HWIN_LO + 4 * b + 3, v.w);
-      }
-    }
-    if (threadIdx.x == 0 && lh[HWIN_N]) atomicAdd(hist, lh[HWIN_N]);
-  }
+    hist_count(pj, lh, hist, &bad);
+  }
+  __syncthreads();
+  hist_flush(lh, hist);
   if (bad) atomicOr(&cnt->err, bad);
-  if (fs.ticket) {
-    static_assert(FIN_TPB == 1024, "the fused Poisson scale runs in a 1024-thread workgroup");
-    __shared__ int sh_is_last;
-    __shared__ double shd[16];
-    int active = (C + FIN_TPB - 1) / FIN_TPB;
-    if (active > (int)gridDim.x) active = (int)gridDim.x;
-    if (active < 1) active = 1;
-    asm volatile("s_waitcnt vmcnt(0)" ::: "memory");
-    __syncthreads();
-    if (threadIdx.x == 0) {
-      sh_is_last = atomicAdd(fs.ticket, 1) == active - 1;
-      if (sh_is_last) __hip_atomic_store(fs.ticket, 0, __ATOMIC_RELAXED, __HIP_MEMORY_SCOPE_AGENT);
-    }
-    __syncthreads();
-    if (sh_is_last)
-      poisson_scale_body<true>(hist, cnt, C, fs.num, fs.eps, fs.rng_ctl, fs.layer_off, fs.is_last, fs.rng_cap_total, fs.sel_state, shd);
-  }
-}
-
+}
+
+__device__ __forceinline__ bf16_t incl_prob_of(bf16_t pj, int all_one, float c32) {
+  if (all_one) return 0x3f80;
+  float v = rbf(bf2f(pj) * c32);
+  return (v < 1.0f || v != v) ? f2bf(v) : (bf16_t)0x3f80;
+}
 __device__ __forceinline__ bf16_t incl_prob(const bf16_t* __restrict__ p, int j, int S, int all_one, float c32) {
   if (all_one || j < S) return 0x3f80;
-  float v = rbf(bf2f(p[j]) * c32);
-  return (v < 1.0f || v != v) ? f2bf(v) : (bf16_t)0x3f80;
+  return incl_prob_of(p[j], all_one, c32);
 }
 
 #define SEL_AGG 1
 #define SEL_PFX 2
+__device__ __forceinline__ int sel_lookback(int* state, int chunk, int tot, int* bad) {
+  const int lane = lane_id();
+  int excl = 0;
+  if (chunk > 0) {
+    if (lane == 0) __hip_atomic_store(state + 1 + chunk, (tot << 2) | SEL_AGG, __ATOMIC_RELAXED, __HIP_MEMORY_SCOPE_AGENT);
+    long long spins = 0;
+    for (int top = chunk - 1; top >= 0;) {
+      const int j = top - lane;
+      const int v = j >= 0 ? __hip_atomic_load(state + 1 + j, __ATOMIC_RELAXED, __HIP_MEMORY_SCOPE_AGENT) : SEL_PFX;
+      const unsigned long long ready = __ballot((v & 3) != 0), pfx = __ballot((v & 3) == SEL_PFX);
+      const int stop = pfx ? __ffsll((long long)pfx) - 1 : 63;
+      const unsigned long long need = stop == 63 ? ~0ull : ((1ull << (stop + 1)) - 1ull);
+      if ((ready & need) != need) {
+        __builtin_amdgcn_s_sleep(1);
+        if (++spins > (1ll << 22)) { *bad |= BLISS_ERR_CAP_KEPT; break; }
+        continue;
+      }
+      excl += wave_total_i32(lane <= stop && j >= 0 ? (v >> 2) : 0);
+      if (pfx) break;
+      top -= 64;
+    }
+  }
+  if (lane == 0) __hip_atomic_store(state + 1 + chunk, ((excl + tot) << 2) | SEL_PFX, __ATOMIC_RELAXED, __HIP_MEMORY_SCOPE_AGENT);
+  return excl;
+}
+
 __global__ void __launch_bounds__(TPB) k_select_fused(const bf16_t* __restrict__ p, const float* __restrict__ uniforms_base,
                                                       const int* __restrict__ u_off, LayerCounts* cnt, bf16_t* __restrict__ P,
                                                       int* state, const int* __restrict__ cand_nid, int* __restrict__ new_id,
@@ -875,29 +957,9 @@
   int tot;
   const int woff = chunk_wave_offset(wave_total, sh4, &tot);
   if (threadIdx.x < 64) {
-    const int lane = lane_id();
-    int excl = 0, bad = 0;
-    if (chunk > 0) {
-      if (lane == 0) __hip_atomic_store(state + 1 + chunk, (tot << 2) | SEL_AGG, __ATOMIC_RELAXED, __HIP_MEMORY_SCOPE_AGENT);
-      long long spins = 0;
-      for (int top = chunk - 1; top >= 0;) {
-        const int j = top - lane;
-        const int v = j >= 0 ? __hip_atomic_load(state + 1 + j, __ATOMIC_RELAXED, __HIP_MEMORY_SCOPE_AGENT) : SEL_PFX;
-        const unsigned long long ready = __ballot((v & 3) != 0), pfx = __ballot((v & 3) == SEL_PFX);
-        const int stop = pfx ? __ffsll((long long)pfx) - 1 : 63;
-        const unsigned long long need = stop == 63 ? ~0ull : ((1ull << (stop + 1)) - 1ull);
-        if ((ready & need) != need) {
-          __builtin_amdgcn_s_sleep(1);
-          if (++spins > (1ll << 22)) { bad = BLISS_ERR_CAP_KEPT; break; }
-          continue;
-        }
-        excl += wave_total_i32(lane <= stop && j >= 0 ? (v >> 2) : 0);
-        if (pfx) break;
-        top -= 64;
-      }
-    }
-    if (lane == 0) {
-      __hip_atomic_store(state + 1 + chunk, ((excl + tot) << 2) | SEL_PFX, __ATOMIC_RELAXED, __HIP_MEMORY_SCOPE_AGENT);
+    int bad = 0;
+    const int excl = sel_lookback(state, chunk, tot, &bad);
+    if (lane_id() == 0) {
       sh_base = excl;
       if (chunk == nchunks - 1) {
         int K = excl + tot;
@@ -926,6 +988,91 @@
   }
   if (chunk == nchunks - 1)
     for (int r = sh_K + threadIdx.x; r < cap_k; r += TPB) { kept_nid[r] = 0; node_prob[r] = 0x3f80; }
+}
+
+__global__ void __launch_bounds__(TPB) k_cand_select(const unsigned* __restrict__ bitmap, const int* __restrict__ word_prefix,
+                                                     const int* __restrict__ tile_sum,
+                                                     const unsigned long long* __restrict__ cand_rec,
+                                                     const float* __restrict__ uniforms_base, const int* __restrict__ u_off,
+                                                     LayerCounts* cnt, int* state, int* __restrict__ local_id, int* cand_nid,
+                                                     bf16_t* __restrict__ p, bf16_t* __restrict__ P, int* __restrict__ new_id,
+                                                     int* __restrict__ kept_nid, bf16_t* __restrict__ node_prob, int cap_c, int cap_k,
+                                                     int* __restrict__ kept_map) {
+  __shared__ int sh[17];
+  __shared__ int sh_chunk, sh_base, sh_K;
+  const float* __restrict__ uniforms = uniforms_base + (u_off ? *u_off : 0);
+  const int E = cnt->E, C = min(cnt->C, cap_c), all_one = cnt->all_one, tid = threadIdx.x;
+  const int S = min(cnt->S, C);
+  const float c32 = (float)cnt->c;
+  const int nw = (E + 31) >> 5, nchunks = sel_chunks(E);
+  for (;;) {
+    __syncthreads();
+    if (tid == 0) sh_chunk = atomicAdd(state, 1);
+    __syncthreads();
+    const int chunk = sh_chunk;
+    if (chunk >= nchunks) return;
+    for (int i = chunk * TPB + tid; i < S; i += nchunks * TPB) {
+      P[i] = 0x3f80;
+      if (i < cap_k) {
+        const int g = cand_nid[i];
+        kept_nid[i] = g; node_prob[i] = 0x3f80; new_id[i] = i;
+        if (kept_map) kept_map[g] = i;
+      } else new_id[i] = -1;
+    }
+    const int tile = chunk * SEL_WORDS / BTILE;
+    int tile_off = 0;
+    if (tile > 0) {
+      int part = 0;
+      for (int t = tid; t < tile; t += TPB) part += tile_sum[t];
+      block_excl_scan(part, sh, &tile_off);
+    }
+    const int w = chunk * SEL_WORDS + tid;
+    const unsigned word = w < nw ? bitmap[w] : 0u;
+    const int id0 = word ? S + tile_off + word_prefix[w] : 0;
+    unsigned keep = 0;
+    {
+      int id = id0;
+      for (unsigned m = word; m && id < C; m &= m - 1, ++id) {
+        const int bit = __ffs((int)m) - 1;
+        const unsigned long long rec = cand_rec[((size_t)w << 5) | (unsigned)bit];
+        const int g = (int)(unsigned)rec;
+        const bf16_t pj = (bf16_t)(rec >> 32), Pv = incl_prob_of(pj, all_one, c32);
+        local_id[g] = id; cand_nid[id] = g; p[id] = pj; P[id] = Pv;
+        if (__hip_atomic_load(uniforms + id, __ATOMIC_RELAXED, __HIP_MEMORY_SCOPE_AGENT) < bf2f(Pv)) keep |= 1u << bit;
+        else new_id[id] = -1;
+      }
+    }
+    int tot;
+    const int ex = block_excl_scan(__popc(keep), sh, &tot);
+    if (tid < 64) {
+      int bad = 0;
+      const int excl = sel_lookback(state, chunk, tot, &bad);
+      if (lane_id() == 0) {
+        sh_base = excl;
+        if (chunk == nchunks - 1) {
+          int K = S + excl + tot;
+          if (K > cap_k) { bad |= BLISS_ERR_CAP_KEPT; K = cap_k; }
+          cnt->K = K;
+          sh_K = K;
+        }
+        if (bad) atomicOr(&cnt->err, bad);
+      }
+    }
+    __syncthreads();
+    int r = S + sh_base + ex;
+    for (unsigned m = keep; m; m &= m - 1, ++r) {
+      const int bit = __ffs((int)m) - 1;
+      const int id = id0 + __popc(word & ((1u << bit) - 1u));
+      if (r < cap_k) {
+        const unsigned long long rec = cand_rec[((size_t)w << 5) | (unsigned)bit];
+        const int g = (int)(unsigned)rec;
+        kept_nid[r] = g; node_prob[r] = incl_prob_of((bf16_t)(rec >> 32), all_one, c32); new_id[id] = r;
+        if (kept_map) kept_map[g] = r;
+      } else new_id[id] = -1;
+    }
+    if (chunk == nchunks - 1)
+      for (int k = sh_K + tid; k < cap_k; k += TPB) { kept_nid[k] = 0; node_prob[k] = 0x3f80; }
+  }
 }
 
 __global__ void __launch_bounds__(TPB) k_mn_prepare(LayerCounts* cnt, const bf16_t* __restrict__ p, bf16_t* __restrict__ P,
@@ -1306,12 +1453,15 @@
   if (frontier_bound < 1) frontier_bound = 1;
   const int ge = grid_for(frontier_bound, TPB), gc = grid_for(frontier_bound, CHUNK);
   const bool binned = ws->n_bins > 0;
+  const bool fused = binned && !partials_only && ws->fs_ticket;
+  if (fused && (!ws->cand_rec || ws->fs_local_id != m->local_id || ws->fs_fanout < 0 || !ws->chunk_cnt)) return BLISS_EINVAL;
   int log2_bins = 0, slots = 0;
   if (binned) {
     while ((1 << log2_bins) < ws->n_bins) ++log2_bins;
     slots = (g->num_nodes + ws->n_bins - 1) >> log2_bins;
     if ((1 << log2_bins) != ws->n_bins || ws->n_bins > MAX_BINS || (size_t)slots * 12 > 64 * 1024 || ws->bin_cap <= 0 ||
-        g->num_edges > (long long)MAX_TILES * BTILE * 32 || !ws->bin_cursor || !ws->bin_rec || !ws->bitmap || !ws->word_prefix || !ws->touched_key || !ws->touched_sum)
+        g->num_edges > (long long)MAX_TILES * BTILE * 32 || !ws->bin_cursor || !ws->bin_rec || !ws->bitmap || !ws->word_prefix ||
+        (!fused && (!ws->touched_key || !ws->touched_sum)))
       return BLISS_EINVAL;
   }
   const long long fcap = (long long)(g->num_edges < 0x7fffffffll ? g->num_edges : 0x7fffffffll);
@@ -1333,20 +1483,29 @@
       PROF_LAUNCH(BK_BIN_SCATTER, st, k_bin_scatter<true><<<gb, BIN_TPB, 0, st>>>(g->indptr, g->indices, w, seeds, ws->seg_ptr, col_base, ws->span_seg, cnt, acc_w, acc_q, eta_f, one_minus_eta_f, uniform_nodes, ws->n_bins, log2_bins, ws->bin_cap, ws->bin_cursor, bin_rec, ws->bitmap, seed_coef));
     else
       PROF_LAUNCH(BK_BIN_SCATTER, st, k_bin_scatter<false><<<gb, BIN_TPB, 0, st>>>(g->indptr, g->indices, w, seeds, ws->seg_ptr, col_base, ws->span_seg, cnt, acc_w, acc_q, eta_f, one_minus_eta_f, uniform_nodes, ws->n_bins, log2_bins, ws->bin_cap, ws->bin_cursor, bin_rec, ws->bitmap, seed_coef));
-    PROF_LAUNCH(BK_BIN_REDUCE, st, k_bin_reduce<<<ws->n_bins, BINRED_TPB, (size_t)slots * 12, st>>>(
-        cnt, ws->n_bins, log2_bins, ws->bin_cap, ws->bin_cursor, bin_rec, g->num_nodes, slots, m->local_id, seed_p2,
-        (unsigned long long*)ws->touched_key, (unsigned long long*)ws->touched_sum, ws->bitmap, ws->cap_c));
-    if (partials_only) return (int)hipGetLastError();
+    const int n_tile_wgs = grid_for(frontier_bound, (int64_t)BTILE * 32, MAX_TILES);
     int* tile_sum = ws->word_prefix;
     int* word_prefix = ws->word_prefix + MAX_TILES;
-    PROF_LAUNCH(BK_BITMAP_SCAN, st, k_bitmap_tiles<<<grid_for(frontier_bound, (int64_t)BTILE * 32, MAX_TILES), 1024, 0, st>>>(ws->bitmap, word_prefix, tile_sum, cnt));
+    if (fused) {
+      PROF_LAUNCH(BK_BIN_REDUCE, st, k_bin_reduce<true><<<ws->n_bins, BINRED_TPB, (size_t)slots * 12, st>>>(
+          cnt, ws->n_bins, log2_bins, ws->bin_cap, ws->bin_cursor, bin_rec, g->num_nodes, slots, m->local_id, seed_p2,
+          nullptr, nullptr, ws->bitmap, ws->cap_c, (unsigned long long*)ws->cand_rec, ws->hist, uniform_nodes));
+      const ScaleTask sc{ws->hist, seeds, seed_p2, ws->bin_cursor + ws->n_bins, ws->cand_nid, (bf16_t*)ws->p, ws->cap_c, uniform_nodes,
+                         ws->fs_fanout, ws->fs_eps, ws->fs_rng_ctl, ws->fs_layer_off, ws->fs_is_last, ws->fs_rng_cap, ws->chunk_cnt};
+      PROF_LAUNCH(BK_BITMAP_SCAN, st, k_bitmap_tiles<<<n_tile_wgs + 1, 1024, 0, st>>>(ws->bitmap, word_prefix, tile_sum, cnt, sc));
+      return (int)hipGetLastError();
+    }
+    PROF_LAUNCH(BK_BIN_REDUCE, st, k_bin_reduce<false><<<ws->n_bins, BINRED_TPB, (size_t)slots * 12, st>>>(
+        cnt, ws->n_bins, log2_bins, ws->bin_cap, ws->bin_cursor, bin_rec, g->num_nodes, slots, m->local_id, seed_p2,
+        (unsigned long long*)ws->touched_key, (unsigned long long*)ws->touched_sum, ws->bitmap, ws->cap_c, nullptr, nullptr, uniform_nodes));
+    if (partials_only) return (int)hipGetLastError();
+    PROF_LAUNCH(BK_BITMAP_SCAN, st, k_bitmap_tiles<<<n_tile_wgs, 1024, 0, st>>>(ws->bitmap, word_prefix, tile_sum, cnt, ScaleTask{}));
     int gf = (ws->cap_c + FIN_TPB - 1) / FIN_TPB;
     if (gf < 1) gf = 1;
     if (gf > 512) gf = 512;
     PROF_LAUNCH(BK_CAND_NUMBER, st, k_cand_number<<<gf, FIN_TPB, 0, st>>>(
         seeds, cnt, ws->cand_nid, m->local_id, seed_p2, (const unsigned long long*)ws->touched_key,
-        (const unsigned long long*)ws->touched_sum, ws->bitmap, word_prefix, tile_sum, (bf16_t*)ws->p, ws->hist, ws->cap_c, uniform_nodes,
-        FusedScale{ws->fs_ticket, ws->fs_fanout, ws->fs_eps, ws->fs_rng_ctl, ws->fs_layer_off, ws->fs_is_last, ws->fs_rng_cap, ws->chunk_cnt}));
+        (const unsigned long long*)ws->touched_sum, ws->bitmap, word_prefix, tile_sum, (bf16_t*)ws->p, ws->hist, ws->cap_c, uniform_nodes));
     return (int)hipGetLastError();
   }
   if (mode == BLISS_MODE_BANDIT) {
@@ -1379,8 +1538,15 @@
   LayerCounts* cnt = (LayerCounts*)ws->counts;
   if (cand_bound < 1) cand_bound = 1;
   if (cand_bound > ws->cap_c) cand_bound = ws->cap_c;
-  if (!ws->fs_ticket)
-    PROF_LAUNCH(BK_POISSON_SCALE, st, k_poisson_scale<<<1, 1024, 0, st>>>(ws->hist, cnt, fanout, eps, rng_ctl, uniforms_offset_dev, is_last, rng_cap_total, ws->chunk_cnt));
+  if (ws->fs_ticket) {
+    if (!ws->n_bins || !ws->bitmap || !ws->word_prefix || !ws->cand_rec || !ws->fs_local_id) return BLISS_EINVAL;
+    PROF_LAUNCH(BK_CAND_SELECT, st, k_cand_select<<<grid_for(cand_bound, SEL_WORDS, 2048), TPB, 0, st>>>(
+        ws->bitmap, ws->word_prefix + MAX_TILES, ws->word_prefix, (const unsigned long long*)ws->cand_rec, uniforms, uniforms_offset_dev,
+        cnt, ws->chunk_cnt, ws->fs_local_id, ws->cand_nid, (bf16_t*)ws->p, (bf16_t*)ws->P, ws->new_id, ws->kept_nid,
+        (bf16_t*)ws->node_prob, ws->cap_c, ws->cap_k, ws->kept_map));
+    return (int)hipGetLastError();
+  }
+  PROF_LAUNCH(BK_POISSON_SCALE, st, k_poisson_scale<<<1, 1024, 0, st>>>(ws->hist, cnt, fanout, eps, rng_ctl, uniforms_offset_dev, is_last, rng_cap_total, ws->chunk_cnt));
   PROF_LAUNCH(BK_SELECT2, st, k_select_fused<<<grid_for(cand_bound, CHUNK, 1 << 20), TPB, 0, st>>>(
       (const bf16_t*)ws->p, uniforms, uniforms_offset_dev, cnt, (bf16_t*)ws->P, ws->chunk_cnt, ws->cand_nid, ws->new_id, ws->kept_nid,
       (bf16_t*)ws->node_prob, ws->cap_c, ws->cap_k, ws->kept_map));
diff --git a/bliss_gnn_amd/roofline.py b/bliss_gnn_amd/roofline.py
--- a/bliss_gnn_amd/roofline.py
+++ b/bliss_gnn_amd/roofline.py
@@ -21,6 +21,7 @@
         "k_bin_scatter": 6 * E + 16 * S,
         "k_bin_reduce": 12 * Cn,
         "k_cand_number": 14 * Cn,
+        "k_cand_select": 26 * Cn + 6 * K,
         "k_block_pass1": 6 * E + 16 * S + 6 * Cn,
         "k_block_pass2": 6 * E + 16 * S + 6 * Cn + 20 * B,
         "k_cand_finalize": 14 * Cn,
diff --git a/include/bliss_gnn.h b/include/bliss_gnn.h
--- a/include/bliss_gnn.h
+++ b/include/bliss_gnn.h
@@ -66,6 +66,8 @@
   int32_t* kept_map;
   int32_t* entry_flag;
   int32_t* fs_ticket; int32_t fs_fanout, fs_is_last, fs_rng_cap, fs_reserved; double fs_eps; int32_t* fs_rng_ctl; int32_t* fs_layer_off;
+  uint64_t* cand_rec;
+  int32_t* fs_local_id;
   int32_t* block_ready_flag;
 } bliss_layer_ws_t;
 
```

Result: slower. 1087 (-25.7%).
